# BadgerTechnologies/navigation

Measured on AMD Instinct MI355X. Metric: scored trajectories/sec (whole node) + costmap inflation cells/sec, 400x400 map, higher is better.
Workload: dtype f64

## Files before the change

### navigation_amd/csrc/costmap_kernels.hip

```cpp
#include "navgpu_device.h"

namespace navgpu {

__global__ void k_fill_u8(uint8_t* dst, uint8_t v, size_t n) {
  size_t i = (size_t)blockIdx.x * blockDim.x + threadIdx.x;
  size_t stride = (size_t)gridDim.x * blockDim.x;
  uint32_t w = v * 0x01010101u;
  uint4 q = make_uint4(w, w, w, w);
  size_t n16 = n / 16;
  for (size_t k = i; k < n16; k += stride) reinterpret_cast<uint4*>(dst)[k] = q;
  for (size_t k = n16 * 16 + i; k < n; k += stride) dst[k] = v;
}
__global__ void k_fill_u32(uint32_t* dst, uint32_t v, size_t n) {
  size_t i = (size_t)blockIdx.x * blockDim.x + threadIdx.x;
  size_t stride = (size_t)gridDim.x * blockDim.x;
  for (size_t k = i; k < n; k += stride) dst[k] = v;
}
void launch_fill_u8(uint8_t* dst, uint8_t v, size_t n, hipStream_t s) {
  if (!n) return;
  size_t blocks = (n / 16 + 255) / 256;
  if (blocks < 1) blocks = 1;
  if (blocks > 4096) blocks = 4096;
  hipLaunchKernelGGL(k_fill_u8, dim3((unsigned)blocks), dim3(256), 0, s, dst, v, n);
}
// ... 301 lines not shown
            double full = hyp2(dx, dy);
            double scale = fmin(1.0, obs.raytrace_range / full);
            b.touch(ox + dx * scale, oy + dy * scale);
          }
        } else {
          if (obs.n_points == 0) continue;
          const double ox = obs.ox, oy = obs.oy, oz = obs.oz;
          if (ox < g.ox || oy < g.oy || oz < cm.origin_z) continue;
          const double sensor_x = (ox - g.ox) / g.res, sensor_y = (oy - g.oy) / g.res, sensor_z = (oz - cm.origin_z) / cm.z_resolution;
          if (!(sensor_x < g.nx && sensor_y < g.ny && sensor_z < size_z)) continue;
          const double map_end_x = g.ox + (g.nx - 1 + 0.5) * g.res;
          const double map_end_y = g.oy + (g.ny - 1 + 0.5) * g.res;
          const uint32_t cell_range = cellDistance(obs.raytrace_range, g.res);
          for (uint32_t p = tid; p < obs.n_points; p += blockDim.x) {
            double wpx = pts[3 * p], wpy = pts[3 * p + 1], wpz = pts[3 * p + 2];
            double distance = sqrt((ox - wpx) * (ox - wpx) + (oy - wpy) * (oy - wpy) + (oz - wpz) * (oz - wpz));
            double scaling_fact = fmax(fmin(1.0, (distance - 2 * g.res) / distance), 0.0);
            wpx = scaling_fact * (wpx - ox) + ox;
            wpy = scaling_fact * (wpy - oy) + oy;
            wpz = scaling_fact * (wpz - oz) + oz;
            double a = wpx - ox, bb = wpy - oy, c = wpz - oz, t = 1.0;
            if (wpz > cm.max_obstacle_height)
              t = fmax(0.0, fmin(t, (cm.max_obstacle_height - 0.01 - oz) / c));
            else if (wpz < cm.origin_z)
              t = fmin(t, (cm.origin_z - oz) / c);
            if (wpx < g.ox) t = fmin(t, (g.ox - ox) / a);
            if (wpy < g.oy) t = fmin(t, (g.oy - oy) / bb);
            if (wpx > map_end_x) t = fmin(t, (map_end_x - ox) / a);
            if (wpy > map_end_y) t = fmin(t, (map_end_y - oy) / bb);
            wpx = ox + a * t;
            wpy = oy + bb * t;
            wpz = oz + c * t;
            if (wpx < g.ox || wpy < g.oy || wpz < cm.origin_z) continue;
            double px = (wpx - g.ox) / g.res, py = (wpy - g.oy) / g.res, pz = (wpz - cm.origin_z) / cm.z_resolution;
            if (!(px < g.nx && py < g.ny && pz < size_z)) continue;
            if (pass == 0) {
              raytrace3d(g.nx, sensor_x, sensor_y, sensor_z, px, py, pz, cell_range,
                         [&](uint32_t off, uint32_t zm) { atomicAnd(&vox[off], ~zm); });
              double dx = wpx - ox, dy = wpy - oy;
              double full = hyp2(dx, dy);
              double scale = fmin(1.0, obs.raytrace_range / full);
              b.touch(ox + dx * scale, oy + dy * scale);
            } else {
              raytrace3d(g.nx, sensor_x, sensor_y, sensor_z, px, py, pz, cell_range, [&](uint32_t off, uint32_t) {
                uint32_t col = vox[off];
                uint32_t unknown_bits = (uint16_t)(col >> 16) ^ (uint16_t)col;
                uint32_t marked_bits = col >> 16;
                if (bitsBelowThreshold(marked_bits, mark_thr))
                  layer[off] = bitsBelowThreshold(unknown_bits, unknown_thr) ? kFree : kNoInfo;
              });
            }
          }
        }
      }
      __syncthreads();
    }
    if (VOXEL && mark_thr > 0) {
      uint2* seq = cm.mark_seq + (size_t)inst * cm.max_points;
      uint32_t n_seq = 0;
      for (uint32_t o = ob; o < oe; ++o) n_seq = max(n_seq, cm.obs[o].first_point + cm.obs[o].n_points);
      for (uint32_t s = tid; s < n_seq; s += blockDim.x) seq[s] = make_uint2(0u, 0u);
      __syncthreads();
      for (uint32_t o = ob; o < oe; ++o) {
        const ObsCsr obs = cm.obs[o];
        if (!(obs.flags & NAVGPU_OBS_MARKING)) continue;
        const float* pts = inst_points + (size_t)obs.first_point * 3;
        const double sq_obstacle_range = obs.obstacle_range * obs.obstacle_range;
        for (uint32_t p = tid; p < obs.n_points; p += blockDim.x) {
          const float fx = pts[3 * p], fy = pts[3 * p + 1], fz = pts[3 * p + 2];
          double px = fx, py = fy, pz = fz;
          if (pz > cm.max_obstacle_height) continue;
          double sq_dist = (px - obs.ox) * (px - obs.ox) + (py - obs.oy) * (py - obs.oy) + (pz - obs.oz) * (pz - obs.oz);
          if (sq_dist >= sq_obstacle_range) continue;
          double wz = (pz < cm.origin_z) ? cm.origin_z : pz;
          if (px < g.ox || py < g.oy || wz < cm.origin_z) continue;
          double fxm = (px - g.ox) / g.res, fym = (py - g.oy) / g.res, fzm = (wz - cm.origin_z) / cm.z_resolution;
          if (!(fxm < 2147483648.0) || !(fym < 2147483648.0) || !(fzm < 2147483648.0)) continue;
          uint32_t mx = (uint32_t)(int)fxm, my = (uint32_t)(int)fym, mz = (uint32_t)(int)fzm;
          if (!(mx < g.nx && my < g.ny && mz < (uint32_t)cm.z_voxels)) continue;
          if (mz >= size_z) continue;
          const uint32_t cell = my * g.nx + mx;
          seq[obs.first_point + p] = make_uint2(cell, 0x80000000u | ((vox[cell] >> 16) << 8) | mz);
        }
      }
      __syncthreads();
      for (uint32_t s = tid; s < n_seq; s += blockDim.x) {
        const uint2 e = seq[s];
        if (!(e.y & 0x80000000u)) continue;
        const uint32_t mz = e.y & 0xFFu;
        uint32_t acc = ((e.y >> 8) & 0xFFFFu) | (1u << mz);
        for (uint32_t q = 0; q < s; ++q) {
          const uint2 f = seq[q];
          if ((f.y & 0x80000000u) && f.x == e.x) acc |= 1u << (f.y & 0xFFu);
        }
        atomicOr(&vox[e.x], ((uint32_t)1 << mz << 16) | (1u << mz));
        if (!bitsBelowThreshold(acc, mark_thr)) {
          layer[e.x] = kLethal;
          const float* pt = inst_points + (size_t)s * 3;
          b.touch((double)pt[0], (double)pt[1]);
        }
      }
    } else
    for (uint32_t o = ob; o < oe; ++o) {
      const ObsCsr obs = cm.obs[o];
      if (!(obs.flags & NAVGPU_OBS_MARKING)) continue;
      const float* pts = inst_points + (size_t)obs.first_point * 3;
      const double sq_obstacle_range = obs.obstacle_range * obs.obstacle_range;
      for (uint32_t p = tid; p < obs.n_points; p += blockDim.x) {
        const float fx = pts[3 * p], fy = pts[3 * p + 1], fz = pts[3 * p + 2];
        double px = fx, py = fy, pz = fz;
        if (pz > cm.max_obstacle_height) continue;
        double sq_dist = (px - obs.ox) * (px - obs.ox) + (py - obs.oy) * (py - obs.oy) + (pz - obs.oz) * (pz - obs.oz);
        if (sq_dist >= sq_obstacle_range) continue;
        if (!VOXEL) {
          uint32_t mx, my;
          if (!worldToMap(g, px, py, mx, my)) continue;
          layer[my * g.nx + mx] = kLethal;
          b.touch(px, py);
        } else {
          double wz = (pz < cm.origin_z) ? cm.origin_z : pz;
          if (px < g.ox || py < g.oy || wz < cm.origin_z) continue;
          double fxm = (px - g.ox) / g.res, fym = (py - g.oy) / g.res, fzm = (wz - cm.origin_z) / cm.z_resolution;
          if (!(fxm < 2147483648.0) || !(fym < 2147483648.0) || !(fzm < 2147483648.0)) continue;
          uint32_t mx = (uint32_t)(int)fxm, my = (uint32_t)(int)fym, mz = (uint32_t)(int)fzm;
          if (!(mx < g.nx && my < g.ny && mz < (uint32_t)cm.z_voxels)) continue;
          if (mz >= size_z) continue;
          uint32_t full_mask = ((uint32_t)1 << mz << 16) | (1u << mz);
          uint32_t old = atomicOr(&vox[my * g.nx + mx], full_mask);
          uint32_t marked_bits = (old | full_mask) >> 16;
          if (!bitsBelowThreshold(marked_bits, mark_thr)) {
            layer[my * g.nx + mx] = kLethal;
            b.touch(px, py);
          }
        }
      }
    }
    if (cm.footprint_clearing) {
      uint32_t nfp = cm.fp_n[inst];
      if (tid < nfp) b.touch(cm.fp_world[((size_t)inst * kMaxFootprint + tid) * 2], cm.fp_world[((size_t)inst * kMaxFootprint + tid) * 2 + 1]);
    }
  }

  for (int off = 32; off > 0; off >>= 1) {
    double o0 = __shfl_down(b.min_x, off), o1 = __shfl_down(b.min_y, off), o2 = __shfl_down(b.max_x, off), o3 = __shfl_down(b.max_y, off);
    b.min_x = (o0 < b.min_x) ? o0 : b.min_x;
    b.min_y = (o1 < b.min_y) ? o1 : b.min_y;
    b.max_x = (b.max_x < o2) ? o2 : b.max_x;
    b.max_y = (b.max_y < o3) ? o3 : b.max_y;
  }
  if ((tid & 63) == 0) {
    red[tid >> 6][0] = b.min_x;
    red[tid >> 6][1] = b.min_y;
    red[tid >> 6][2] = b.max_x;
    red[tid >> 6][3] = b.max_y;
  }
  __syncthreads();
  if (tid == 0) {
    for (int w = 1; w < 4; ++w) {
      b.min_x = (red[w][0] < b.min_x) ? red[w][0] : b.min_x;
      b.min_y = (red[w][1] < b.min_y) ? red[w][1] : b.min_y;
      b.max_x = (b.max_x < red[w][2]) ? red[w][2] : b.max_x;
      b.max_y = (b.max_y < red[w][3]) ? red[w][3] : b.max_y;
    }
    if (only_bounds) {
      bounds_io_out[4 * blockIdx.x + 0] = b.min_x;
      bounds_io_out[4 * blockIdx.x + 1] = b.min_y;
      bounds_io_out[4 * blockIdx.x + 2] = b.max_x;
      bounds_io_out[4 * blockIdx.x + 3] = b.max_y;
      s_box_valid = 1;
    } else {
      if (cm.layers & NAVGPU_LAYER_INFLATION) {
        if (st->need_reinflation) {
          st->last_min_x = b.min_x;
          st->last_min_y = b.min_y;
          st->last_max_x = b.max_x;
          st->last_max_y = b.max_y;
          b.min_x = -3.4028234663852886e38;
          b.min_y = -3.4028234663852886e38;
          b.max_x = 3.4028234663852886e38;
          b.max_y = 3.4028234663852886e38;
          st->need_reinflation = 0;
        } else {
          double tminx = st->last_min_x, tminy = st->last_min_y, tmaxx = st->last_max_x, tmaxy = st->last_max_y;
          st->last_min_x = b.min_x;
          st->last_min_y = b.min_y;
          st->last_max_x = b.max_x;
          st->last_max_y = b.max_y;
          b.min_x = ((b.min_x < tminx) ? b.min_x : tminx) - cm.inflation_radius;
          b.min_y = ((b.min_y < tminy) ? b.min_y : tminy) - cm.inflation_radius;
          b.max_x = ((tmaxx < b.max_x) ? b.max_x : tmaxx) + cm.inflation_radius;
          b.max_y = ((tmaxy < b.max_y) ? b.max_y : tmaxy) + cm.inflation_radius;
        }
      }
      st->bounds[0] = b.min_x;
      st->bounds[1] = b.min_y;
      st->bounds[2] = b.max_x;
      st->bounds[3] = b.max_y;
      int x0, xn, y0, yn;
      enforceBounds(g, b.min_x, b.min_y, x0, y0);
      enforceBounds(g, b.max_x, b.max_y, xn, yn);
      x0 = x0 > 0 ? x0 : 0;
      xn = ((int)g.nx < xn + 1) ? (int)g.nx : xn + 1;
      y0 = y0 > 0 ? y0 : 0;
      yn = ((int)g.ny < yn + 1) ? (int)g.ny : yn + 1;
      st->box[0] = x0;
      st->box[1] = xn;
      st->box[2] = y0;
      st->box[3] = yn;
      st->box_valid = !(xn < x0 || yn < y0);
      s_box_valid = st->box_valid;
    }
  }
  __syncthreads();

  if (has_obs_layer && cm.footprint_clearing && s_box_valid) {
    const uint32_t nfp = cm.fp_n[inst];
    if (tid == 0) s_poly_ok = nfp >= 3;
    __syncthreads();
    if (tid < nfp) {
      uint32_t mx, my;
      bool ok = worldToMap(g, cm.fp_world[((size_t)inst * kMaxFootprint + tid) * 2], cm.fp_world[((size_t)inst * kMaxFootprint + tid) * 2 + 1], mx, my);
      s_vx[tid] = mx;
      s_vy[tid] = my;
      if (!ok) atomicAnd(&s_poly_ok, 0);
    }
    __syncthreads();
    if (s_poly_ok) {
      uint32_t minx = 0xFFFFFFFFu, maxx = 0;
      for (uint32_t i = 0; i < nfp; ++i) {
        minx = s_vx[i] < minx ? s_vx[i] : minx;
        maxx = s_vx[i] > maxx ? s_vx[i] : maxx;
      }
      const uint32_t span = maxx - minx + 1;
      if (span <= 1024) {
        for (uint32_t c = tid; c < span; c += blockDim.x) {
          colmin[c] = 0xFFFFFFFFu;
          colmax[c] = 0;
        }
        __syncthreads();
        if (tid < nfp) {
          uint32_t e1 = (tid + 1 == nfp) ? 0 : tid + 1;
          raytrace2d(g.nx, s_vx[tid], s_vy[tid], s_vx[e1], s_vy[e1], 0xFFFFFFFFu, [&](uint32_t off) {
            uint32_t y = off / g.nx, x = off - y * g.nx;
            atomicMin(&colmin[x - minx], y);
            atomicMax(&colmax[x - minx], y);
          });
        }
        __syncthreads();
        for (uint32_t c = tid >> 4; c < span; c += blockDim.x >> 4) {
          uint32_t lo = colmin[c], hi = colmax[c];
          if (lo == 0xFFFFFFFFu) continue;
          for (uint32_t y = lo + (tid & 15); y <= hi; y += 16) layer[y * g.nx + minx + c] = kFree;
        }
      }
    }
  }
}

__global__ __launch_bounds__(256) void k_reset_bounding_box(CostmapDev cm, uint32_t first, const double* boxes_world) {
  const uint32_t inst = first + blockIdx.x;
  const Geom g{cm.origin[2 * inst], cm.origin[2 * inst + 1], cm.res, cm.nx, cm.ny};
  const double* bw = boxes_world + 4 * blockIdx.x;
  int x0, y0, xn, yn;
  enforceBounds(g, bw[0], bw[1], x0, y0);
  enforceBounds(g, bw[2], bw[3], xn, yn);
  uint8_t* layer = cm.obst + (size_t)inst * cm.cells_padded;
  if (xn > x0 && yn > y0) {
    const uint32_t w = (uint32_t)(xn - x0), n = w * (uint32_t)(yn - y0);
    for (uint32_t i = threadIdx.x; i < n; i += blockDim.x) layer[(uint32_t)(y0 + i / w) * g.nx + (uint32_t)x0 + i % w] = cm.obstacle_default;
  }
  if (threadIdx.x == 0) {
    InstCostmapState* st = cm.state + inst;
    if (!st->has_extra_bounds) {
      st->extra[0] = st->extra[1] = 1e6;
      st->extra[2] = st->extra[3] = -1e6;
    }
    st->extra[0] = (bw[0] < st->extra[0]) ? bw[0] : st->extra[0];
    st->extra[1] = (bw[1] < st->extra[1]) ? bw[1] : st->extra[1];
    st->extra[2] = (st->extra[2] < bw[2]) ? bw[2] : st->extra[2];
    st->extra[3] = (st->extra[3] < bw[3]) ? bw[3] : st->extra[3];
    st->has_extra_bounds = 1;
  }
}
__global__ __launch_bounds__(256) void k_reset_window(uint8_t* grid, size_t stride, uint32_t nx, uint32_t x0, uint32_t y0, uint32_t xn, uint32_t yn, uint8_t value) {
  uint8_t* gp = grid + (size_t)blockIdx.x * stride;
  const uint32_t w = xn - x0, n = w * (yn - y0);
  for (uint32_t i = threadIdx.x; i < n; i += blockDim.x) gp[(y0 + i / w) * nx + x0 + i % w] = value;
}
void launch_reset_window(uint8_t* grid, size_t stride, uint32_t count, uint32_t nx, uint32_t x0, uint32_t y0, uint32_t xn, uint32_t yn, uint8_t value, hipStream_t s) {
  hipLaunchKernelGGL(k_reset_window, dim3(count), dim3(256), 0, s, grid, stride, nx, x0, y0, xn, yn, value);
}
void launch_reset_bounding_box(const CostmapDev& cm, uint32_t first, uint32_t count, const double* boxes_world, hipStream_t s) {
  hipLaunchKernelGGL(k_reset_bounding_box, dim3(count), dim3(256), 0, s, cm, first, boxes_world);
}

void launch_obstacle(const CostmapDev& cm, uint32_t first, uint32_t count, const double* bounds_in, int only_bounds, hipStream_t s) {
  double* bounds_out = const_cast<double*>(bounds_in);
  if (cm.layers & NAVGPU_LAYER_VOXEL)
    hipLaunchKernelGGL(k_obstacle<true>, dim3(count), dim3(256), 0, s, cm, first, bounds_in, bounds_out, only_bounds);
  else
    hipLaunchKernelGGL(k_obstacle<false>, dim3(count), dim3(256), 0, s, cm, first, bounds_in, bounds_out, only_bounds);
}

__global__ __launch_bounds__(256) void k_merge(CostmapDev cm, uint32_t first, const int32_t* boxes, int static_received, int layer_only) {
  const uint32_t inst = first + blockIdx.y;
  int x0, xn, y0, yn;
  if (boxes) {
    x0 = boxes[4 * blockIdx.y + 0];
    y0 = boxes[4 * blockIdx.y + 1];
    xn = boxes[4 * blockIdx.y + 2];
    yn = boxes[4 * blockIdx.y + 3];
  } else {
    const InstCostmapState* st = cm.state + inst;
    if (!st->box_valid) return;
    x0 = st->box[0];
    xn = st->box[1];
    y0 = st->box[2];
    yn = st->box[3];
  }
  const uint32_t q = blockIdx.x * blockDim.x + threadIdx.x;
  const uint32_t base = q * 16;
  if (base >= cm.cells) return;
  const int row_first = base / cm.nx, row_last = (min(base + 15, cm.cells - 1)) / cm.nx;
  if (row_last < y0 || row_first >= yn) return;
  bool inside = false;
  if (row_first == row_last) {
    const int gx = base - row_first * cm.nx;
    if (gx + 15 < x0 || gx >= xn) return;
    inside = gx >= x0 && gx + 15 < xn && base + 15 < cm.cells && !layer_only;
  }
  const size_t off = (size_t)inst * cm.cells_padded + base;
  uint4 mv = make_uint4(0, 0, 0, 0);
  if (!inside) mv = *reinterpret_cast<const uint4*>(cm.master + off);
  const bool has_static = (cm.layers & NAVGPU_LAYER_STATIC) && static_received && !layer_only && !cm.stat_roll && cm.stat;
  const bool roll_static = cm.stat_roll != nullptr && !layer_only;
  double tfm[8] = {1, 0, 0, 0, 0, 1, 0, 0};
  double m_ox = 0, m_oy = 0;
  if (roll_static) {
    const double* T = cm.stat_tf + (size_t)inst * 12;
    tfm[0] = T[0]; tfm[1] = T[1]; tfm[2] = T[2]; tfm[3] = T[9];
    tfm[4] = T[3]; tfm[5] = T[4]; tfm[6] = T[5]; tfm[7] = T[10];
    m_ox = cm.origin[2 * inst];
    m_oy = cm.origin[2 * inst + 1];
  }
  const bool has_obst = (cm.layers & (NAVGPU_LAYER_OBSTACLE | NAVGPU_LAYER_VOXEL)) && cm.obs_enabled;
  uint4 sv = has_static ? *reinterpret_cast<const uint4*>(cm.stat + off) : make_uint4(0, 0, 0, 0);
  uint4 lv = has_obst ? *reinterpret_cast<const uint4*>(cm.obst + off) : make_uint4(0, 0, 0, 0);
  uint32_t mw[4] = {mv.x, mv.y, mv.z, mv.w}, sw[4] = {sv.x, sv.y, sv.z, sv.w}, lw[4] = {lv.x, lv.y, lv.z, lv.w};
  int y = row_first;
  int x = base - row_first * cm.nx;
  bool changed = false;
#pragma unroll
  for (int k = 0; k < 16; ++k) {
    if (base + k < cm.cells && x >= x0 && x < xn && y >= y0 && y < yn) {
      const int sh = (k & 3) * 8;
      uint8_t m = layer_only ? (uint8_t)((mw[k >> 2] >> sh) & 0xFF) : cm.master_default;
      if (has_static) {
        uint8_t sc = (sw[k >> 2] >> sh) & 0xFF;
        if (!cm.static_use_maximum)
          m = sc;
        else if (sc != kNoInfo && (m == kNoInfo || m < sc))
          m = sc;
      }
      if (roll_static) {
        const double wx = m_ox + (x + 0.5) * cm.res, wy = m_oy + (y + 0.5) * cm.res;
        const double px = tfm[0] * wx + tfm[1] * wy + tfm[2] * 0.0 + tfm[3];
        const double py = tfm[4] * wx + tfm[5] * wy + tfm[6] * 0.0 + tfm[7];
        if (!(px < cm.stat_ox || py < cm.stat_oy)) {
          const uint32_t smx = (uint32_t)(int)((px - cm.stat_ox) / cm.stat_res), smy = (uint32_t)(int)((py - cm.stat_oy) / cm.stat_res);
          if (smx < cm.stat_nx && smy < cm.stat_ny) {
            const uint8_t sc = cm.stat_roll[(size_t)smy * cm.stat_nx + smx];
            m = cm.static_use_maximum ? (sc > m ? sc : m) : sc;
          }
        }
      }
      if (has_obst) {
        uint8_t lc = (lw[k >> 2] >> sh) & 0xFF;
        if (lc != kNoInfo) {
          if (cm.combination_method == 0)
            m = lc;
          else if (cm.combination_method == 1 && (m == kNoInfo || m < lc))
            m = lc;
        }
      }
      mw[k >> 2] = (mw[k >> 2] & ~(0xFFu << sh)) | ((uint32_t)m << sh);
      changed = true;
    }
    if (++x == (int)cm.nx) {
      x = 0;
      ++y;
    }
  }
  if (changed) *reinterpret_cast<uint4*>(cm.master + off) = make_uint4(mw[0], mw[1], mw[2], mw[3]);
}

void launch_merge(const CostmapDev& cm, uint32_t first, uint32_t count, const int32_t* boxes, hipStream_t s, bool layer_only) {
  uint32_t groups = (cm.cells + 15) / 16;
  dim3 grid((groups + 255) / 256, count);
  hipLaunchKernelGGL(k_merge, grid, dim3(256), 0, s, cm, first, boxes, cm.static_received, layer_only ? 1 : 0);
}

constexpr int kTile = 64;
__global__ __launch_bounds__(256) void k_inflate(CostmapDev cm, uint32_t first, const int32_t* boxes) {
  extern __shared__ __align__(16) uint8_t lds[];
  const uint32_t inst = first + blockIdx.z;
  const int R = (int)cm.R;
  int min_i, min_j, max_i, max_j;
  if (boxes) {
    min_i = boxes[4 * blockIdx.z + 0];
    min_j = boxes[4 * blockIdx.z + 1];
    max_i = boxes[4 * blockIdx.z + 2];
    max_j = boxes[4 * blockIdx.z + 3];
  } else {
    const InstCostmapState* st = cm.state + inst;
    if (!st->box_valid) return;
    min_i = st->box[0];
    max_i = st->box[1];
    min_j = st->box[2];
    max_j = st->box[3];
  }
  min_i = max(0, min_i - R);
  min_j = max(0, min_j - R);
  max_i = min((int)cm.nx, max_i + R);
  max_j = min((int)cm.ny, max_j + R);
  const int tx0 = blockIdx.x * kTile, ty0 = blockIdx.y * kTile;
  if (tx0 - R >= max_i || tx0 + kTile + R <= min_i || ty0 - R >= max_j || ty0 + kTile + R <= min_j) return;

  const int W = kTile + 2 * R;
  const int WS = (W + 3) & ~3;
  uint8_t* seed = lds;
  uint8_t* hd = seed + W * WS;
  uint8_t* lut = hd + W * kTile;
  __shared__ int s_any;
  const uint32_t tid = threadIdx.x;
  uint8_t* master = cm.master + (size_t)inst * cm.cells_padded;
  if (tid == 0) s_any = 0;
  for (int i = tid; i < (R + 2) * (R + 2); i += blockDim.x) lut[i] = cm.lut[i];
  __syncthreads();
  int any = 0;
  for (int i = tid; i < W * W; i += blockDim.x) {
    int ly = i / W, lx = i - ly * W;
    int gx = tx0 - R + lx, gy = ty0 - R + ly;
    uint8_t f = 0;
    if (gx >= min_i && gx < max_i && gy >= min_j && gy < max_j) f = master[gy * cm.nx + gx] == kLethal;
    seed[ly * WS + lx] = f;
    any |= f;
  }
  if (any) s_any = 1;
  __syncthreads();
  if (!s_any) return;
  for (int i = tid; i < W * kTile; i += blockDim.x) {
    int ly = i / kTile, c = i - ly * kTile;
    const uint8_t* row = seed + ly * WS + c + R;
    uint8_t best = 255;
    for (int d = 0; d <= R; ++d) {
      if (row[d] | row[-d]) {
        best = (uint8_t)d;
        break;
      }
    }
    hd[i] = best;
  }
  __syncthreads();
  const int n = R + 2;
  for (int i = tid; i < kTile * kTile; i += blockDim.x) {
    int ry = i / kTile, c = i - ry * kTile;
    int gx = tx0 + c, gy = ty0 + ry;
    if (gx >= (int)cm.nx || gy >= (int)cm.ny) continue;
    uint8_t cost = 0;
    for (int dy = -R; dy <= R; ++dy) {
      uint8_t h = hd[(ry + R + dy) * kTile + c];
      if (h != 255) {
        int ady = dy < 0 ? -dy : dy;
        uint8_t cc = lut[h * n + ady];
        cost = cc > cost ? cc : cost;
      }
    }
    if (cost == 0) continue;
    uint8_t old = master[gy * cm.nx + gx];
    uint8_t nv = (old == kNoInfo && cost >= kInscribed) ? cost : (old > cost ? old : cost);
    if (nv != old) master[gy * cm.nx + gx] = nv;
  }
}

constexpr int kBX = 64, kBY = 32;
template <int RT>
__global__ __launch_bounds__(256) void k_inflate_bits(CostmapDev cm, uint32_t first, uint32_t count, const int32_t* boxes) {
  const uint32_t tbx = blockIdx.x >> 3, tby = blockIdx.y, rz = blockIdx.z * 8u + (blockIdx.x & 7u);
  if (rz >= count) return;
  const uint32_t inst = first + rz;
  const int R = RT > 0 ? RT : (int)cm.R;
  int min_i, min_j, max_i, max_j;
  if (boxes) {
    min_i = boxes[4 * rz + 0];
    min_j = boxes[4 * rz + 1];
    max_i = boxes[4 * rz + 2];
    max_j = boxes[4 * rz + 3];
  } else {
    const InstCostmapState* st = cm.state + inst;
    if (!st->box_valid) return;
    min_i = st->box[0];
    max_i = st->box[1];
    min_j = st->box[2];
    max_j = st->box[3];
  }
  min_i = max(0, min_i - R);
  min_j = max(0, min_j - R);
  max_i = min((int)cm.nx, max_i + R);
  max_j = min((int)cm.ny, max_j + R);
  const int tx0 = (int)tbx * kBX, ty0 = (int)tby * kBY;
  if (tx0 - R >= max_i || tx0 + kBX + R <= min_i || ty0 - R >= max_j || ty0 + kBY + R <= min_j) return;

  constexpr int kMaxHR = kBY + 2 * 14;
  constexpr int kOct = (kMaxHR + 7) / 8;
  __shared__ uint32_t s_rows[kMaxHR][4];
  __shared__ uint32_t s_hd[kOct + 1][kBX];
  __shared__ uint8_t s_lut2[256];
  __shared__ int s_any;
  __shared__ uint32_t s_rowany[2];
  const uint32_t tid = threadIdx.x, lane = tid & 63, wave = tid >> 6;
  const int HR = kBY + 2 * R;
  uint8_t* master = cm.master + (size_t)inst * cm.cells_padded;
  if (tid == 0) s_any = 0;
  if (tid < 2) s_rowany[tid] = 0;
  s_lut2[tid] = cm.lut2[tid];
  __syncthreads();
  int any = 0;
  uint32_t rows_lo = 0, rows_hi = 0;
  constexpr int kSeedIt = (kMaxHR + 3) / 4;
  uint8_t cell[kSeedIt][2];
  const int gxa = tx0 - 32 + (int)lane, gxb = gxa + 64;
  const int lo_x = max(min_i, tx0 - R), lo_y = max(min_j, ty0 - R);
  const int hi_x = max(lo_x, min(max_i, tx0 + kBX + R) - 1), hi_y = max(lo_y, min(max_j, ty0 + kBY + R) - 1);
  const int cxa = min(min(max(gxa, lo_x), hi_x), (int)cm.nx - 1), cxb = min(min(max(gxb, lo_x), hi_x), (int)cm.nx - 1);
  const bool xa_ok = gxa >= min_i && gxa < max_i && gxa >= tx0 - R && gxa < tx0 + kBX + R;
  const bool xb_ok = gxb >= min_i && gxb < max_i && gxb >= tx0 - R && gxb < tx0 + kBX + R;
#pragma unroll
  for (int it = 0; it < kSeedIt; ++it) {
    const int gy = ty0 - R + (int)wave + 4 * it;
    const int cy = min(min(max(gy, lo_y), hi_y), (int)cm.ny - 1);
    cell[it][0] = master[cy * cm.nx + cxa];
    cell[it][1] = master[cy * cm.nx + cxb];
  }
#pragma unroll
  for (int it = 0; it < kSeedIt; ++it) {
    const int r = (int)wave + 4 * it, gy = ty0 - R + r;
    if (r < HR) {
      const bool row_ok = gy >= min_j && gy < max_j;
#pragma unroll
      for (int half = 0; half < 2; ++half) {
        const unsigned long long m = __ballot(row_ok && (half ? xb_ok : xa_ok) && cell[it][half] == kLethal);
        if (lane == 0) {
          s_rows[r][2 * half] = (uint32_t)m;
          s_rows[r][2 * half + 1] = (uint32_t)(m >> 32);
        }
        any |= m != 0ull;
        if (m != 0ull) {
          if (r < 32)
            rows_lo |= 1u << r;
          else
            rows_hi |= 1u << (r - 32);
        }
      }
    }
  }
  if (any && lane == 0) {
    s_any = 1;
    if (rows_lo) atomicOr(&s_rowany[0], rows_lo);
    if (rows_hi) atomicOr(&s_rowany[1], rows_hi);
  }
  __syncthreads();
  if (!s_any) return;
  const uint32_t lowmask = (1u << R) - 1u;
  for (int o = wave; o * 8 < HR; o += 4) {
    uint32_t packed = 0;
#pragma unroll
    for (int k = 0; k < 8; ++k) {
      const int r = o * 8 + k;
      uint32_t h = 15;
      if (r < HR && (s_rows[r][0] | s_rows[r][1] | s_rows[r][2] | s_rows[r][3]) != 0u) {
        const uint32_t sft = 32u + lane - (uint32_t)R;
        const uint32_t wi = sft >> 5, bs = sft & 31u;
        const unsigned long long two = ((unsigned long long)s_rows[r][wi + 1 < 4 ? wi + 1 : 3] << 32) | s_rows[r][wi];
        const uint32_t q = (uint32_t)(two >> bs);
        const uint32_t qr = q >> R;
        const uint32_t ql = q & lowmask;
        uint32_t dr = 15, dl = 15;
        if (qr & ((2u << R) - 1u)) dr = (uint32_t)__builtin_ctz(qr & ((2u << R) - 1u));
        if (ql) dl = (uint32_t)R - (31u - (uint32_t)__builtin_clz(ql));
        h = dr < dl ? dr : dl;
      }
      packed |= h << (4 * k);
    }
    s_hd[o][lane] = packed;
  }
  __syncthreads();
  uint32_t hw[5];
#pragma unroll
  for (int k = 0; k < 5; ++k) hw[k] = (wave + k) * 8 < (uint32_t)HR ? s_hd[wave + k][lane] : 0xFFFFFFFFu;
  if (__ballot((hw[0] & hw[1] & hw[2] & hw[3] & hw[4]) != 0xFFFFFFFFu) == 0ull) return;
  const int gx = tx0 + (int)lane;
  const int R2 = R * R;
  uint32_t bestr[8] = {0xFFFFu, 0xFFFFu, 0xFFFFu, 0xFFFFu, 0xFFFFu, 0xFFFFu, 0xFFFFu, 0xFFFFu};
  if (RT > 0) {
    const unsigned long long rowany = (((unsigned long long)s_rowany[1] << 32) | s_rowany[0]) >> (8u * wave);
    const uint32_t ra_lo = __builtin_amdgcn_readfirstlane((uint32_t)rowany), ra_hi = __builtin_amdgcn_readfirstlane((uint32_t)(rowany >> 32));
#pragma unroll
    for (int p = 0; p < 8 + 2 * RT; ++p) {
      if (((p < 32 ? ra_lo >> (p & 31) : ra_hi >> (p & 31)) & 1u) != 0u) {
        const uint32_t h = (hw[p >> 3] >> (4 * (p & 7))) & 15u;
        const uint32_t hh = h * h;
#pragma unroll
        for (int j = 0; j < 8; ++j) {
          const int dy = p - RT - j;
          if (dy >= -RT && dy <= RT) {
            const uint32_t d2 = hh + (uint32_t)(dy * dy);
            bestr[j] = d2 < bestr[j] ? d2 : bestr[j];
          }
        }
      }
    }
  }
#pragma unroll
  for (int j = 0; j < 8; ++j) {
    const int gy = ty0 + (int)wave * 8 + j;
    uint32_t best = bestr[j];
    if (RT == 0) {
      for (int dy = -R; dy <= R; ++dy) {
        const int p = j + R + dy;
        const uint32_t wsel = p >> 3;
        const uint32_t word = wsel == 0 ? hw[0] : (wsel == 1 ? hw[1] : (wsel == 2 ? hw[2] : (wsel == 3 ? hw[3] : hw[4])));
        const uint32_t h = (word >> (4 * (p & 7))) & 15u;
        const uint32_t d2 = h * h + (uint32_t)(dy * dy);
        best = d2 < best ? d2 : best;
      }
    }
    if (best > (uint32_t)R2 || gx >= (int)cm.nx || gy >= (int)cm.ny) continue;
    const uint8_t cost = s_lut2[best];
    if (cost == 0) continue;
    const uint8_t old = master[gy * cm.nx + gx];
    const uint8_t nv = (old == kNoInfo && cost >= kInscribed) ? cost : (old > cost ? old : cost);
    if (nv != old) master[gy * cm.nx + gx] = nv;
  }
}

constexpr uint32_t kPqSeenWords = 5120, kPqWinBytes = 65536;
constexpr size_t kPqLdsBytes = 150 * 1024;
constexpr uint32_t kPqTabEntries = 66 * 66;
__global__ __launch_bounds__(64) void k_inflate_pq(CostmapDev cm, uint32_t first, const int32_t* boxes) {
  extern __shared__ __align__(16) uint8_t pq_sm[];
  const uint32_t inst = first + blockIdx.x;
  const uint32_t tid = threadIdx.x;
  int min_i, min_j, max_i, max_j;
  if (boxes) {
    min_i = boxes[4 * blockIdx.x + 0];
    min_j = boxes[4 * blockIdx.x + 1];
    max_i = boxes[4 * blockIdx.x + 2];
    max_j = boxes[4 * blockIdx.x + 3];
  } else {
    const InstCostmapState* st = cm.state + inst;
    if (!st->box_valid) return;
    min_i = st->box[0];
    max_i = st->box[1];
    min_j = st->box[2];
    max_j = st->box[3];
  }
  uint8_t* master = cm.master + (size_t)inst * cm.cells_padded;
  uint8_t* seen_g = cm.pq_seen + (size_t)inst * cm.cells_padded;
  PqCell* heap_g = cm.pq_heap + (size_t)inst * cm.pq_cap;
  const uint32_t size_x = cm.nx, size_y = cm.ny;
  const int R = (int)cm.R;
  const uint32_t n = cm.R + 2;
  min_i = max(0, min_i - R);
  min_j = max(0, min_j - R);
  max_i = min((int)size_x, max_i + R);
  max_j = min((int)size_y, max_j + R);
  if (max_i <= min_i || max_j <= min_j) return;
  const int wx0 = max(0, min_i - R - 1), wy0 = max(0, min_j - R - 1), wx1 = min((int)size_x, max_i + R + 1), wy1 = min((int)size_y, max_j + R + 1);
  const uint32_t ww = (uint32_t)(wx1 - wx0), wh = (uint32_t)(wy1 - wy0), wcells = ww * wh;
  const bool seen_lds = wcells <= kPqSeenWords * 32u, win_lds = wcells <= kPqWinBytes;
  uint16_t* rank = reinterpret_cast<uint16_t*>(pq_sm);
  uint8_t* lut_l = pq_sm + kPqTabEntries * 2;
  const uint32_t seen_off = (kPqTabEntries * 3 + 15u) & ~15u;
  uint32_t* seen_l = reinterpret_cast<uint32_t*>(pq_sm + seen_off);
  const uint32_t win_off = seen_off + (seen_lds ? (((wcells + 31) / 32 * 4 + 15u) & ~15u) : 0u);
  uint8_t* win_l = pq_sm + win_off;
  const uint32_t heap_off = win_off + (win_lds ? ((wcells + 15u) & ~15u) : 0u);
  PqCell* heap_l = reinterpret_cast<PqCell*>(pq_sm + heap_off);
  const long heap_lds = (long)((kPqLdsBytes - heap_off) / sizeof(PqCell));
  for (uint32_t i = tid; i < n * n; i += 64) {
    rank[i] = reinterpret_cast<const uint16_t*>(cm.dist_lut)[i];
    lut_l[i] = cm.lut[i];
  }
  if (seen_lds) {
    for (uint32_t i = tid; i < (wcells + 31) / 32; i += 64) seen_l[i] = 0;
  } else {
    for (uint32_t i = tid * 16; i < cm.cells_padded; i += 64 * 16) *reinterpret_cast<uint4*>(seen_g + i) = make_uint4(0, 0, 0, 0);
  }
  if (win_lds)
    for (uint32_t i = tid; i < wcells; i += 64) {
      const uint32_t y = i / ww, x = i - y * ww;
      win_l[i] = master[(uint32_t)(wy0 + (int)y) * size_x + (uint32_t)(wx0 + (int)x)];
    }
  __syncthreads();
  if (tid == 0) {
    long len = 0;
    auto hget = [&](long i) -> PqCell { return i < heap_lds ? heap_l[i] : heap_g[i]; };
    auto hset = [&](long i, const PqCell& v) {
      if (i < heap_lds)
        heap_l[i] = v;
      else
        heap_g[i] = v;
    };
    auto widx = [&](uint32_t mx, uint32_t my) { return (my - (uint32_t)wy0) * ww + (mx - (uint32_t)wx0); };
    auto seenGet = [&](uint32_t index, uint32_t mx, uint32_t my) -> bool {
      if (seen_lds) {
        const uint32_t w = widx(mx, my);
        return (seen_l[w >> 5] >> (w & 31)) & 1u;
      }
      return seen_g[index] != 0;
    };
    auto seenSet = [&](uint32_t index, uint32_t mx, uint32_t my) {
      if (seen_lds) {
        const uint32_t w = widx(mx, my);
        seen_l[w >> 5] |= 1u << (w & 31);
      } else {
        seen_g[index] = 1;
      }
    };
    auto pushHeap = [&](long hole, const PqCell& value) {
      long parent = (hole - 1) / 2;
      while (hole > 0) {
        const PqCell pv = hget(parent);
        if (!(pv.rank > value.rank)) break;
        hset(hole, pv);
        hole = parent;
        parent = (hole - 1) / 2;
      }
      hset(hole, value);
    };
    auto probe = [&](bool in_map, uint32_t index, uint32_t mx, uint32_t my, uint32_t sx, uint32_t sy) -> uint32_t {
      if (!in_map) return 0xFFFFu;
      const uint32_t dx = mx > sx ? mx - sx : sx - mx, dy = my > sy ? my - sy : sy - my;
      const uint32_t r = rank[dx * n + dy];
      return seenGet(index, mx, my) ? 0xFFFFu : r;
    };
    auto push = [&](uint32_t r, uint32_t index, uint32_t mx, uint32_t my, uint32_t sx, uint32_t sy) {
      if (r == 0xFFFFu) return;
      if ((uint64_t)len >= cm.pq_cap) return;
      PqCell c;
      c.index = index;
      c.rank = (uint16_t)r;
      c.sdx = (int8_t)((int)sx - (int)mx);
      c.sdy = (int8_t)((int)sy - (int)my);
      pushHeap(len++, c);
    };
    auto enqueue = [&](uint32_t index, uint32_t mx, uint32_t my, uint32_t sx, uint32_t sy) { push(probe(true, index, mx, my, sx, sy), index, mx, my, sx, sy); };
    for (int j = min_j; j < max_j; j++)
      for (int i = min_i; i < max_i; i++) {
        const uint32_t index = (uint32_t)j * size_x + (uint32_t)i;
        const uint8_t c0 = win_lds ? win_l[widx((uint32_t)i, (uint32_t)j)] : master[index];
        if (c0 == kLethal) enqueue(index, i, j, i, j);
      }
    while (len > 0) {
      const PqCell cur = hget(0);
      if (len > 1) {
        const PqCell value = hget(len - 1);
        const long l = len - 1;
        long hole = 0, child = 0;
        while (child < (l - 1) / 2) {
          child = 2 * (child + 1);
          const PqCell a = hget(child), b = hget(child - 1);
          if (a.rank > b.rank) {
            child--;
            hset(hole, b);
          } else {
            hset(hole, a);
          }
          hole = child;
        }
        if ((l & 1) == 0 && child == (l - 2) / 2) {
          child = 2 * (child + 1);
          hset(hole, hget(child - 1));
          hole = child - 1;
        }
        pushHeap(hole, value);
      }
      --len;
      const uint32_t index = cur.index;
      const uint32_t my = index / size_x, mx = index - my * size_x;
      if (seenGet(index, mx, my)) continue;
      seenSet(index, mx, my);
      const uint32_t sx = (uint32_t)((int)mx + cur.sdx), sy = (uint32_t)((int)my + cur.sdy);
      const uint32_t dx = mx > sx ? mx - sx : sx - mx, dy = my > sy ? my - sy : sy - my;
      const uint8_t cost = lut_l[dx * n + dy];
      uint8_t* cellp = win_lds ? &win_l[widx(mx, my)] : &master[index];
      const uint8_t old_cost = *cellp;
      if (old_cost == kNoInfo && cost >= kInscribed)
        *cellp = cost;
      else
        *cellp = old_cost > cost ? old_cost : cost;
      const uint32_t r0 = probe(mx > 0, index - 1, mx - 1, my, sx, sy), r1 = probe(my > 0, index - size_x, mx, my - 1, sx, sy),
                     r2 = probe(mx < size_x - 1, index + 1, mx + 1, my, sx, sy), r3 = probe(my < size_y - 1, index + size_x, mx, my + 1, sx, sy);
      push(r0, index - 1, mx - 1, my, sx, sy);
      push(r1, index - size_x, mx, my - 1, sx, sy);
      push(r2, index + 1, mx + 1, my, sx, sy);
      push(r3, index + size_x, mx, my + 1, sx, sy);
    }
  }
  __syncthreads();
  if (win_lds)
    for (uint32_t i = tid; i < wcells; i += 64) {
      const uint32_t y = i / ww, x = i - y * ww;
      master[(uint32_t)(wy0 + (int)y) * size_x + (uint32_t)(wx0 + (int)x)] = win_l[i];
    }
}

void launch_inflate(const CostmapDev& cm, uint32_t first, uint32_t count, const int32_t* boxes, hipStream_t s) {
  if (!cm.infl_enabled) return;
  const int R = (int)cm.R;
  if (cm.infl_pq) {
    if (!cm.pq_heap || !cm.pq_seen || !cm.dist_lut) return;
    hipFuncSetAttribute((const void*)k_inflate_pq, hipFuncAttributeMaxDynamicSharedMemorySize, (int)kPqLdsBytes);
    hipLaunchKernelGGL(k_inflate_pq, dim3(count), dim3(64), kPqLdsBytes, s, cm, first, boxes);
    return;
  }
  if (cm.lut2_ok && R >= 1 && R <= 14) {
    dim3 grid(8u * ((cm.nx + kBX - 1) / kBX), (cm.ny + kBY - 1) / kBY, (count + 7u) / 8u);
    if (R == 11)
      hipLaunchKernelGGL(k_inflate_bits<11>, grid, dim3(256), 0, s, cm, first, count, boxes);
    else
      hipLaunchKernelGGL(k_inflate_bits<0>, grid, dim3(256), 0, s, cm, first, count, boxes);
    return;
  }
  const int W = kTile + 2 * R, WS = (W + 3) & ~3;
  size_t lds = (size_t)W * WS + (size_t)W * kTile + (size_t)(R + 2) * (R + 2);
  dim3 grid((cm.nx + kTile - 1) / kTile, (cm.ny + kTile - 1) / kTile, count);
  hipLaunchKernelGGL(k_inflate, grid, dim3(256), lds, s, cm, first, boxes);
}

}
```

### navigation_amd/csrc/navgpu_device.h

```cpp
#pragma once
#include <hip/hip_runtime.h>
#include <stdint.h>

#include "../../include/navgpu.h"

namespace navgpu {

constexpr uint8_t kNoInfo = 255, kLethal = 254, kInscribed = 253, kFree = 0;
constexpr int kMaxFootprint = 32;
constexpr int kCareRows = 128, kCareWords = 4;
#ifndef NAVGPU_SCORE_TAB_THREADS
#define NAVGPU_SCORE_TAB_THREADS 256
#endif
#ifndef NAVGPU_SCORE_TAB_LDS_KB
#define NAVGPU_SCORE_TAB_LDS_KB 14
#endif
#ifndef NAVGPU_SCORE_PREP_THREADS
#define NAVGPU_SCORE_PREP_THREADS 256
#endif
#ifndef NAVGPU_SCORE_THREADS
#define NAVGPU_SCORE_THREADS 256
#endif
#ifdef NAVGPU_DEBUG_SWITCHES
#define NAVGPU_DEBUG_ENV(name) getenv(name)
#else
#define NAVGPU_DEBUG_ENV(name) ((const char*)nullptr)
#endif
constexpr int kScoreThreads = NAVGPU_SCORE_THREADS;

struct InstCostmapState {
  double last_min_x, last_min_y, last_max_x, last_max_y;
  int32_t need_reinflation;
  int32_t static_has_updated_data;
  int32_t box[4];
  int32_t box_valid;
  int32_t pad;
  double bounds[4];
  double extra[4];
  int32_t has_extra_bounds, pad2;
};

struct ObsCsr {
  uint32_t first_point, n_points, flags, pad;
  double ox, oy, oz;
  double obstacle_range, raytrace_range;
};

struct PqCell {
  uint32_t index;
  uint16_t rank;
  int8_t sdx, sdy;
};
static_assert(sizeof(PqCell) == 8, "heap entry");
struct CostmapDev {
  uint32_t nx, ny, cells, cells_padded;
  double res;
  int32_t layers, track_unknown;
  uint8_t master_default, obstacle_default;
  int32_t obs_enabled, footprint_clearing, combination_method, static_use_maximum, static_received;
  double max_obstacle_height;
  int32_t z_voxels, unknown_threshold, mark_threshold;
  double origin_z, z_resolution;
  int32_t infl_enabled;
  uint32_t R;
  double inflation_radius;
  double* origin;
  uint8_t *master, *stat, *obst;
  uint32_t* voxel;
  uint8_t* lut;
  uint8_t* lut2;
  int32_t lut2_ok;
  int32_t infl_pq;
  double* dist_lut;
  uint8_t* pq_seen;
  PqCell* pq_heap;
  uint64_t pq_cap;
  uint8_t* stat_roll;
  uint32_t stat_nx, stat_ny;
  double stat_res, stat_ox, stat_oy;
  double* stat_tf;
  InstCostmapState* state;
  double* pose;
  double* fp_world;
  uint32_t* fp_n;
  ObsCsr* obs;
  uint32_t* obs_count;
  float* points;
  uint32_t max_obs, max_points;
  int32_t* shift;
  uint8_t *master_alt, *obst_alt;
  uint32_t* voxel_alt;
  uint2* mark_seq;
};

struct PlannerDev {
  uint32_t nx, ny, cells;
  double res, inv_res;
  double* origin;
  const uint8_t* master;
  uint32_t cells_padded;
  navgpu_dwa_config cfg;
  double scale_path, scale_goal, scale_obstacle;
  uint32_t max_plan, max_sim_steps, max_axis;
  uint32_t max_samples, score_blocks;
  navgpu_robot_state* state;
  double* plan;
  uint32_t* plan_count;
  double* front_last;
  int32_t* align_on;
  double* fp_spec;
  uint32_t* fp_n;
  float* axis_samples;
  int32_t* axis_count;
  uint32_t *path, *goal, *goal_front;
  uint32_t* bfs_scratch;
  int32_t* bfs_box;
  uint32_t* bfs_care;
  uint32_t* bfs_reach;
  uint32_t bfs_bounded;
  unsigned long long* bfs_trace;
  uint32_t* bfs_next_item;
  uint32_t* bfs_free;
  uint32_t* bfs_levels;
  uint32_t* bfs_order;
  uint32_t bfs_grids;
  uint32_t* within;
  uint32_t win;
  uint32_t fp_rcells;
  uint8_t fp_halfw[32];
  uint32_t fp_chunk;
  uint32_t use_tables, tab_steps, tab_nfp, tab_nth;
  int32_t mg_agg[4];
  double mg_yshift[4];
  int32_t mg_generic;
  uint32_t tab_rows;
  uint32_t tab_bytes;
  double tab_dt;
  uint8_t* prep;
  uint32_t prep_stride, prep_bytes;
  double* sample_cost;
  int32_t* sample_status;
  double* part_cost;
  int32_t* part_index;
  int32_t* counters;
  uint32_t* osc_flags;
  float* osc_prev;
  navgpu_plan_result* result;
  double* traj;
};

struct TpOut {
  double cost;
  double ex, ey, eth;
  double ahead;
  int32_t n_points;
  int32_t ahead_ok;
};
struct TpDev {
  navgpu_tp_config cfg;
  uint32_t max_samples;
  double* samples;
  uint32_t* n_samples;
  double* start;
  TpOut* out;
  int32_t* winner;
  double* points;
  uint32_t* within_cells;
  uint32_t* within_count;
  uint32_t max_within;
  uint32_t* within_bits;
};
void launch_tp_within(const PlannerDev& pl, const TpDev& tp, uint32_t first, uint32_t count, hipStream_t s);
void launch_tp_rollout(const PlannerDev& pl, const TpDev& tp, uint32_t first, uint32_t count, int store_points, hipStream_t s);

void launch_obstacle(const CostmapDev& cm, uint32_t first, uint32_t count, const double* bounds_in, int only_bounds,
                     hipStream_t s);
void launch_reset_window(uint8_t* grid, size_t stride, uint32_t count, uint32_t nx, uint32_t x0, uint32_t y0, uint32_t xn, uint32_t yn, uint8_t value, hipStream_t s);
void launch_reset_bounding_box(const CostmapDev& cm, uint32_t first, uint32_t count, const double* boxes_world, hipStream_t s);
void launch_merge(const CostmapDev& cm, uint32_t first, uint32_t count, const int32_t* boxes, hipStream_t s, bool layer_only = false);
void launch_inflate(const CostmapDev& cm, uint32_t first, uint32_t count, const int32_t* boxes, hipStream_t s);
void launch_static_interpret(uint8_t* dst, const int8_t* occ, uint32_t cells, uint32_t cells_padded, uint32_t count,
                             int track_unknown_space, int trinary, int lethal_threshold, int unknown_cost_value, hipStream_t s);
void launch_export_window(const uint8_t* master, uint32_t nx, uint32_t x0, uint32_t y0, uint32_t w, uint32_t h, int8_t* out, hipStream_t s);
void launch_fill_u8(uint8_t* dst, uint8_t v, size_t n, hipStream_t s);
void launch_fill_u32(uint32_t* dst, uint32_t v, size_t n, hipStream_t s);
void launch_shift_u8(const uint8_t* src, uint8_t* dst, const CostmapDev& cm, uint32_t first, uint32_t count, uint8_t fill, hipStream_t s);
void launch_shift_u32(const uint32_t* src, uint32_t* dst, const CostmapDev& cm, uint32_t first, uint32_t count, uint32_t fill, hipStream_t s);

void launch_cell_costs(const PlannerDev& pl, uint32_t inst, float4* out, hipStream_t s);
void launch_samples(const PlannerDev& pl, uint32_t first, uint32_t count, hipStream_t s);
void launch_bfs(const PlannerDev& pl, uint32_t first, uint32_t count, hipStream_t s, const uint32_t* order = nullptr, bool free_ready = false);
uint32_t launch_score(const PlannerDev& pl, uint32_t first, uint32_t count, const float* explicit_sample, hipStream_t s);
void launch_select(const PlannerDev& pl, uint32_t first, uint32_t count, uint32_t n_blocks, hipStream_t s);
constexpr uint32_t kPoseChunk = 64;
struct PoseChunk {
  navgpu_robot_state* state;
  double* front_last;
  int32_t* align_on;
  uint32_t* bfs_reach;
  uint32_t first, count;
  navgpu_robot_state st[kPoseChunk];
  double front[2 * kPoseChunk];
  int32_t align[kPoseChunk];
  uint32_t reach[kPoseChunk];
};
static_assert(sizeof(PoseChunk) <= 4096, "kernel arguments are limited to 4 KB");
void launch_stage_poses(const PoseChunk& c, hipStream_t s);
void launch_sincos(const double* th, uint32_t n, double* sn, double* cs, hipStream_t s);
size_t score_table_bytes(const PlannerDev& pl);
size_t score_window_bytes(uint32_t win);
size_t score_prep_bytes(const PlannerDev& pl);
size_t score_prep_slot_bytes(const PlannerDev& pl);
size_t bfs_scratch_words(uint32_t nx, uint32_t ny);
uint32_t score_table_rows(const PlannerDev& pl, uint32_t win);

struct Geom {
  double ox, oy, res;
  uint32_t nx, ny;
};

__device__ __forceinline__ bool worldToMap(const Geom& g, double wx, double wy, uint32_t& mx, uint32_t& my) {
  if (wx < g.ox || wy < g.oy) return false;
  double fx = (wx - g.ox) / g.res;
  double fy = (wy - g.oy) / g.res;
  if (!(fx < 2147483648.0) || !(fy < 2147483648.0)) return false;
  mx = (uint32_t)(int)fx;
  my = (uint32_t)(int)fy;
  return mx < g.nx && my < g.ny;
}

__device__ __forceinline__ double hyp2(double x, double y) {
  double a = x * x, b = y * y;
  double s = a + b;
  double h = sqrt(s);
  if (h == 0.0) return 0.0;
  double bb = s - a;
  double e = (a - (s - bb)) + (b - bb);
  double r = __builtin_fma(-h, h, s);
  return h + (r + e) / (2.0 * h);
}

struct NavfnDev {
  int nx, ny, ns;
  uint32_t ns_padded, path_cap;
  uint8_t *costarr, *pending;
  float *potarr, *gradx, *grady;
  int* pb;
  float* path;
  navgpu_navfn_result* results;
  float* potalt;
  uint32_t* wf_act;
  uint32_t *wf_nchg, *wf_min;
  struct NavfnWfStatus* wf_status;
  int wf_tiles_x, wf_tiles_y, wf_max_rounds;
};
struct NavfnWfStatus {
  int32_t done, final_array, rounds, pad;
};
struct NavfnWfRule {
  int32_t global_planner, quadratic, outline, allow_unknown;
  int32_t lethal_cost, neutral_cost;
  float cost_factor;
  int32_t max_sweeps;
};
void launch_navfn_wf_init(const NavfnDev& nv, uint32_t first, uint32_t count, const NavfnWfRule& rule, const int32_t* seed_cells, const float* seed_vals,
                          hipStream_t s);
void launch_navfn_wf_round(const NavfnDev& nv, uint32_t first, uint32_t count, const NavfnWfRule& rule, const int32_t* stop_cells, int at_start, int round,
                           hipStream_t s);
void launch_gp_wf_finish(const NavfnDev& nv, uint32_t first, uint32_t count, const navgpu_global_planner_params& gp, const double* starts,
                         const double* goals, const int32_t* goal_cells, hipStream_t s);
void launch_navfn_wf_path(const NavfnDev& nv, uint32_t first, uint32_t count, const int32_t* goals, const int32_t* starts, hipStream_t s);
void launch_navfn_costmap(const NavfnDev& nv, uint32_t first, uint32_t count, const uint8_t* cmap, size_t stride, int cost_mode, int allow_unknown,
                          hipStream_t s);
void launch_gp_plan(const NavfnDev& nv, uint32_t first, uint32_t count, const navgpu_global_planner_params& gp, const double* starts,
                    const double* goals, const int32_t* goal_cells, void* heaps, hipStream_t s);
void launch_navfn_plan(const NavfnDev& nv, uint32_t first, uint32_t count, const int32_t* goals, const int32_t* starts, int astar, int at_start,
                       hipStream_t s);

}
```

### navigation_amd/csrc/navgpu_fleet.h

```cpp
#pragma once
#include <algorithm>
#include <cfloat>
#include <cmath>
#include <cstdio>
#include <cstdlib>
#include <cstring>
#include <ctime>
#include <mutex>
#include <string>
#include <vector>

#include "navgpu_device.h"

using namespace navgpu;

namespace navgpu {
extern thread_local std::string g_last_error;

#define HIP_TRY(expr)                                                                              \
  do {                                                                                             \
    hipError_t e_ = (expr);                                                                        \
    if (e_ != hipSuccess) {                                                                        \
      g_last_error = std::string(#expr) + ": " + hipGetErrorString(e_);                            \
      return NAVGPU_ERR_HIP;                                                                       \
    }                                                                                              \
  } while (0)

inline hipError_t waitStream(hipStream_t s) { return hipStreamSynchronize(s); }

struct EventPair {
  int kernel;
  hipEvent_t a, b;
};
int ensureCompleteGrids(navgpu_fleet* f, uint32_t first, uint32_t count);
}

struct navgpu_fleet {
  navgpu_fleet_desc desc{};
  std::recursive_mutex mu;
  hipStream_t stream = nullptr;
  CostmapDev cm{};
  PlannerDev pl{};
  bool planner_configured = false, inflation_configured = false, planner_staged = false;
  bool shift_pending = false;
  uint32_t shift_first = 0, shift_count = 0;
  std::vector<void*> allocs;
  std::vector<double> h_origin;
  std::vector<double> h_fp_spec;
  std::vector<uint32_t> h_fp_n;
  navgpu_inflation_params infl{};
  navgpu_obstacle_params obsp{};
  double fp_radius = 0.0;
  std::vector<void*> pinned;
  ObsCsr* hp_obs = nullptr;
  uint32_t *hp_cnt = nullptr, *hp_used = nullptr, *hp_plan_cnt = nullptr;
  float* hp_pts = nullptr;
  double *hp_fpw = nullptr, *hp_pose = nullptr, *hp_plan = nullptr, *hp_front = nullptr;
  int32_t *hp_shift = nullptr, *hp_align = nullptr;
  uint32_t *hp_reach = nullptr, *hp_fpn = nullptr;
  uint8_t *cm_stage_dev = nullptr, *cm_stage_host = nullptr, *pl_stage_dev = nullptr, *pl_stage_host = nullptr;
  size_t cm_stage_bytes = 0, pl_stage_bytes = 0;
  bool bounded_grids = true;
  std::vector<uint8_t> grid_partial;
  std::vector<int32_t> h_box;
  std::vector<uint64_t> inputs_gen, cycle_gen;
  void touchInputs(uint32_t first, uint32_t count) {
    for (uint32_t i = first; i < first + count && i < inputs_gen.size(); ++i) ++inputs_gen[i];
  }
  navgpu_robot_state* hp_state = nullptr;
  navgpu_plan_result* hp_result = nullptr;
  bool hp_dma_pending = false;
  int cycles_in_flight = 1;
  int res_slot = 0;
  hipEvent_t ev_cycle[2] = {nullptr, nullptr}, ev_cm_h2d = nullptr, ev_pl_h2d = nullptr;
  bool ev_cycle_set[2] = {false, false}, ev_cm_set = false, ev_pl_set = false;
  hipError_t waitMirrors(hipEvent_t ev, bool set) {
    if (cycles_in_flight < 2) return navgpu::waitStream(stream);
    return set ? hipEventSynchronize(ev) : hipSuccess;
  }
  struct LocalPlannerState {
    std::vector<double> plan;
    double T[3] = {0, 0, 0};
    bool has_T = false, have_plan = false;
    bool xy_tolerance_latch = false, rotating_to_goal = false;
  };
  std::vector<LocalPlannerState> lp;
  navgpu_local_limits lp_limits{};
  bool lp_configured = false;
  struct TpHost {
    std::vector<double> plan;
    double final_goal_x = 0, final_goal_y = 0;
    bool final_goal_position_valid = false;
    navgpu_tp_state st{};
    std::vector<navgpu_tp_sample> made;
    int n_points = 0;
  };
  TpDev tp{};
  bool tp_configured = false;
  std::vector<TpHost> tph;
  std::vector<double> tp_h_samples, tp_h_start;
  std::vector<TpOut> tp_h_out;
  std::vector<uint32_t> tp_h_nsamples, tp_h_within, tp_h_within_count;
  std::vector<int32_t> tp_h_winner;
  double* d_bounds_tmp = nullptr;
  int32_t* d_boxes_tmp = nullptr;
  float* d_explicit = nullptr;
  int8_t* d_occ = nullptr;
  float4* d_cell_costs = nullptr;
  size_t alloc_limit = 0;
  bool profiling = false;
  uint32_t prof_mask = ~0u;
  std::vector<EventPair> events;
  std::vector<EventPair> free_events;
  double prof_ms[NAVGPU_K_COUNT] = {0};
  uint64_t prof_n[NAVGPU_K_COUNT] = {0};

  template <class T>
  int alloc(T** p, size_t count) {
    void* q = nullptr;
    size_t bytes = std::max<size_t>(count * sizeof(T), 16);
    if (alloc_limit && bytes > alloc_limit) {
      g_last_error = "hipMalloc: refused by navgpu_fleet_set_alloc_limit";
      return NAVGPU_ERR_HIP;
    }
    hipError_t e = hipMalloc(&q, bytes);
    if (e != hipSuccess) {
      g_last_error = std::string("hipMalloc: ") + hipGetErrorString(e);
      return NAVGPU_ERR_HIP;
    }
    e = hipMemsetAsync(q, 0, bytes, stream);
    if (e != hipSuccess) {
      g_last_error = std::string("hipMemsetAsync: ") + hipGetErrorString(e);
      return NAVGPU_ERR_HIP;
    }
    allocs.push_back(q);
    *p = static_cast<T*>(q);
    return NAVGPU_OK;
  }
  template <class T>
  int allocPinned(T** p, size_t count) {
    void* q = nullptr;
    hipError_t e = hipHostMalloc(&q, std::max<size_t>(count * sizeof(T), 16), hipHostMallocDefault);
    if (e != hipSuccess) {
      g_last_error = std::string("hipHostMalloc: ") + hipGetErrorString(e);
      return NAVGPU_ERR_HIP;
    }
    memset(q, 0, std::max<size_t>(count * sizeof(T), 16));
    pinned.push_back(q);
    *p = static_cast<T*>(q);
    return NAVGPU_OK;
  }
  void release(void* q) {
    if (!q) return;
    auto it = std::find(allocs.begin(), allocs.end(), q);
    if (it != allocs.end()) allocs.erase(it);
    hipFree(q);
  }
  bool rangeOk(uint32_t first, uint32_t count) const { return count > 0 && first < desc.n_instances && count <= desc.n_instances - first; }

  int beginKernel(int k, EventPair* ep) {
    if (!profiling || !((prof_mask >> k) & 1u)) return NAVGPU_OK;
    if (free_events.empty()) {
      EventPair n{};
      HIP_TRY(hipEventCreate(&n.a));
      HIP_TRY(hipEventCreate(&n.b));
      free_events.push_back(n);
    }
    *ep = free_events.back();
    free_events.pop_back();
    ep->kernel = k;
    HIP_TRY(hipEventRecord(ep->a, stream));
    return NAVGPU_OK;
  }
  int endKernel(EventPair* ep) {
    if (!profiling || !ep->a) return NAVGPU_OK;
    HIP_TRY(hipEventRecord(ep->b, stream));
    events.push_back(*ep);
    if (events.size() > 8192) return foldEvents();
    return NAVGPU_OK;
  }
  int foldEvents() {
    if (events.empty()) return NAVGPU_OK;
    HIP_TRY(waitStream(stream));
    for (auto& e : events) {
      float ms = 0;
      HIP_TRY(hipEventElapsedTime(&ms, e.a, e.b));
      prof_ms[e.kernel] += ms;
      prof_n[e.kernel] += 1;
      free_events.push_back(e);
    }
    events.clear();
    return NAVGPU_OK;
  }
};

#ifndef NAVGPU_TEST_NO_FLEET_LOCK
struct FleetGuard {
  std::lock_guard<std::recursive_mutex> lk;
  explicit FleetGuard(navgpu_fleet* f) : lk(f->mu) { (void)hipSetDevice(f->desc.device); }
};
#else
struct FleetGuard {
  explicit FleetGuard(navgpu_fleet* f) { (void)hipSetDevice(f->desc.device); }
};
#endif

#define PROFILED(fleet, kid, launch_expr)            \
  do {                                               \
    EventPair ep_{};                                 \
    int rc_ = (fleet)->beginKernel((kid), &ep_);     \
    if (rc_) return rc_;                             \
    launch_expr;                                     \
    rc_ = (fleet)->endKernel(&ep_);                  \
    if (rc_) return rc_;                             \
  } while (0)

inline int checkLaunch() {
  hipError_t e = hipGetLastError();
  if (e != hipSuccess) {
    g_last_error = std::string("kernel launch: ") + hipGetErrorString(e);
    return NAVGPU_ERR_HIP;
  }
  return NAVGPU_OK;
}
```

### navigation_amd/csrc/navgpu_host.cpp

```cpp
#include "navgpu_fleet.h"

namespace navgpu {
thread_local std::string g_last_error;
}

extern "C" {

const char* navgpu_version(void) { return "navgpu 0.1 (gfx950)"; }
const char* navgpu_strerror(int status) {
  switch (status) {
    case NAVGPU_OK: return "ok";
    case NAVGPU_ERR_INVALID: return "invalid argument";
    case NAVGPU_ERR_NO_DEVICE: return "no usable HIP device (this library has no CPU fallback)";
    case NAVGPU_ERR_HIP: return "HIP runtime error";
    case NAVGPU_ERR_CAPACITY: return "input exceeds a capacity given at fleet creation";
    case NAVGPU_ERR_STATE: return "call sequence violated";
    default: return "unknown status";
  }
}
const char* navgpu_last_error(void) { return g_last_error.c_str(); }
int navgpu_device_count(void) {
  int n = 0;
  if (hipGetDeviceCount(&n) != hipSuccess) return 0;
  return n;
}
const char* navgpu_kernel_name(int32_t k) {
  static const char* names[NAVGPU_K_COUNT] = {"k_obstacle", "k_merge", "k_inflate", "k_bfs", "k_score", "k_select"};
  return (k >= 0 && k < NAVGPU_K_COUNT) ? names[k] : "?";
}

int navgpu_fleet_create(const navgpu_fleet_desc* d, navgpu_fleet** out) {
  if (!d || !out || d->n_instances == 0 || d->size_x == 0 || d->size_y == 0 || !(d->resolution > 0)) return NAVGPU_ERR_INVALID;
  if ((uint64_t)((d->size_x + 127) / 128) * ((d->size_y + 15) / 16) > 8192) {
    g_last_error = "navgpu_fleet_create: costmap larger than 16.7 M cells";
    return NAVGPU_ERR_CAPACITY;
  }
  if (d->max_footprint > (uint32_t)kMaxFootprint) return NAVGPU_ERR_CAPACITY;
  if ((uint64_t)d->size_x * d->size_y > (1ull << 30) || d->size_x > 65535 || d->size_y > 65535) return NAVGPU_ERR_CAPACITY;
  int ndev = 0;
  if (hipGetDeviceCount(&ndev) != hipSuccess || ndev <= 0 || d->device < 0 || d->device >= ndev) {
    g_last_error = "no HIP device";
    return NAVGPU_ERR_NO_DEVICE;
  }
  HIP_TRY(hipSetDevice(d->device));
  auto* f = new navgpu_fleet();
  f->desc = *d;
  if (f->desc.max_observations == 0) f->desc.max_observations = 1;
  if (f->desc.max_points == 0) f->desc.max_points = 1;
  if (f->desc.max_plan == 0) f->desc.max_plan = 1;
  if (f->desc.max_sim_steps == 0) f->desc.max_sim_steps = 64;
  const uint32_t n = d->n_instances;
  if (hipStreamCreateWithFlags(&f->stream, hipStreamNonBlocking) != hipSuccess) {
    g_last_error = "hipStreamCreate failed";
    delete f;
    return NAVGPU_ERR_NO_DEVICE;
  }
  CostmapDev& cm = f->cm;
  cm.nx = d->size_x;
  cm.ny = d->size_y;
  cm.cells = d->size_x * d->size_y;
  cm.cells_padded = (cm.cells + 63) & ~63u;
  cm.res = d->resolution;
  cm.layers = d->layers;
  cm.track_unknown = d->track_unknown;
  cm.master_default = d->track_unknown ? kNoInfo : kFree;
  cm.obstacle_default = d->track_unknown ? kNoInfo : kFree;
  cm.obs_enabled = 1;
  cm.footprint_clearing = 1;
  cm.combination_method = 1;
  cm.max_obstacle_height = 2.0;
  cm.z_voxels = 10;
  cm.unknown_threshold = 15;
  cm.mark_threshold = 0;
  cm.origin_z = 0.0;
  cm.z_resolution = 0.2;
  cm.max_obs = f->desc.max_observations;
  cm.max_points = f->desc.max_points;
  int rc = 0;
#define A(ptr, cnt)                        \
  if ((rc = f->alloc(&(ptr), (cnt))) != 0) { \
    navgpu_fleet_destroy(f);               \
    return rc;                             \
  }
  A(cm.origin, (size_t)n * 2);
  A(cm.master, (size_t)n * cm.cells_padded);
  if ((d->layers & NAVGPU_LAYER_STATIC) && !d->rolling_window) A(cm.stat, (size_t)n * cm.cells_padded);
  if (d->layers & (NAVGPU_LAYER_OBSTACLE | NAVGPU_LAYER_VOXEL)) A(cm.obst, (size_t)n * cm.cells_padded);
  if (d->layers & NAVGPU_LAYER_VOXEL) A(cm.voxel, (size_t)n * cm.cells_padded);
  A(cm.lut, 66 * 66);
  A(cm.lut2, 256);
  A(cm.state, n);
  A(cm.shift, (size_t)n * 2);
  {
    size_t off = 0;
    auto take = [&](size_t bytes) {
      const size_t at = off;
      off = (off + bytes + 255) & ~(size_t)255;
      return at;
    };
    const size_t o_pose = take(sizeof(double) * 3 * n), o_fpw = take(sizeof(double) * 2 * kMaxFootprint * n), o_fpn = take(sizeof(uint32_t) * n),
                 o_obs = take(sizeof(ObsCsr) * (size_t)n * cm.max_obs), o_cnt = take(sizeof(uint32_t) * n),
                 o_pts = take(sizeof(float) * 3 * (size_t)n * cm.max_points);
    f->cm_stage_bytes = off;
    uint8_t *d = nullptr, *h = nullptr;
    A(d, off);
    if ((rc = f->allocPinned(&h, off)) != 0) {
      navgpu_fleet_destroy(f);
      return rc;
    }
    f->cm_stage_dev = d;
    f->cm_stage_host = h;
    cm.pose = reinterpret_cast<double*>(d + o_pose);
    cm.fp_world = reinterpret_cast<double*>(d + o_fpw);
    cm.fp_n = reinterpret_cast<uint32_t*>(d + o_fpn);
    cm.obs = reinterpret_cast<ObsCsr*>(d + o_obs);
    cm.obs_count = reinterpret_cast<uint32_t*>(d + o_cnt);
    cm.points = reinterpret_cast<float*>(d + o_pts);
    f->hp_pose = reinterpret_cast<double*>(h + o_pose);
    f->hp_fpw = reinterpret_cast<double*>(h + o_fpw);
    f->hp_fpn = reinterpret_cast<uint32_t*>(h + o_fpn);
    f->hp_obs = reinterpret_cast<ObsCsr*>(h + o_obs);
    f->hp_cnt = reinterpret_cast<uint32_t*>(h + o_cnt);
    f->hp_pts = reinterpret_cast<float*>(h + o_pts);
  }
  if (d->rolling_window) {
    if (d->layers & NAVGPU_LAYER_STATIC) {
      A(cm.stat_tf, (size_t)n * 12);
      std::vector<double> ident((size_t)n * 12, 0.0);
      for (uint32_t i = 0; i < n; ++i) ident[(size_t)i * 12 + 0] = ident[(size_t)i * 12 + 4] = ident[(size_t)i * 12 + 8] = 1.0;
      if (hipMemcpy(cm.stat_tf, ident.data(), sizeof(double) * ident.size(), hipMemcpyHostToDevice) != hipSuccess) {
        navgpu_fleet_destroy(f);
        return NAVGPU_ERR_HIP;
      }
    }
    A(cm.master_alt, (size_t)n * cm.cells_padded);
    if (cm.obst) A(cm.obst_alt, (size_t)n * cm.cells_padded);
    if (cm.voxel) A(cm.voxel_alt, (size_t)n * cm.cells_padded);
  }
  if (cm.voxel) A(cm.mark_seq, (size_t)n * cm.max_points);
#define AP(ptr, cnt)                              \
  if ((rc = f->allocPinned(&(ptr), (cnt))) != 0) { \
    navgpu_fleet_destroy(f);                       \
    return rc;                                     \
  }
  AP(f->hp_used, n);
  AP(f->hp_shift, (size_t)n * 2);
  AP(f->hp_result, (size_t)n * 2);
  f->pl.result = f->hp_result;
#undef AP
  A(f->d_bounds_tmp, (size_t)n * 4);
  A(f->d_boxes_tmp, (size_t)n * 4);
  A(f->d_explicit, 4);
  PlannerDev& pl = f->pl;
  pl.nx = cm.nx;
  pl.ny = cm.ny;
  pl.cells = cm.cells;
  pl.cells_padded = cm.cells_padded;
  pl.res = cm.res;
  pl.inv_res = 1.0 / cm.res;
  pl.origin = cm.origin;
  pl.master = cm.master;
  pl.max_plan = f->desc.max_plan;
  pl.max_sim_steps = f->desc.max_sim_steps;
  {
    size_t off = 0;
    auto take = [&](size_t bytes) {
      const size_t at = off;
      off = (off + bytes + 255) & ~(size_t)255;
      return at;
    };
    const size_t o_state = take(sizeof(navgpu_robot_state) * n), o_front = take(sizeof(double) * 2 * n), o_align = take(sizeof(int32_t) * n),
                 o_reach = take(sizeof(uint32_t) * n), o_pcnt = take(sizeof(uint32_t) * n), o_plan = take(sizeof(double) * 2 * (size_t)n * pl.max_plan);
    f->pl_stage_bytes = off;
    uint8_t *d = nullptr, *h = nullptr;
    A(d, off);
    if ((rc = f->allocPinned(&h, off)) != 0) {
      navgpu_fleet_destroy(f);
      return rc;
    }
    f->pl_stage_dev = d;
    f->pl_stage_host = h;
    pl.state = reinterpret_cast<navgpu_robot_state*>(d + o_state);
    pl.front_last = reinterpret_cast<double*>(d + o_front);
    pl.align_on = reinterpret_cast<int32_t*>(d + o_align);
    pl.bfs_reach = reinterpret_cast<uint32_t*>(d + o_reach);
    pl.plan_count = reinterpret_cast<uint32_t*>(d + o_pcnt);
    pl.plan = reinterpret_cast<double*>(d + o_plan);
    f->hp_state = reinterpret_cast<navgpu_robot_state*>(h + o_state);
    f->hp_front = reinterpret_cast<double*>(h + o_front);
    f->hp_align = reinterpret_cast<int32_t*>(h + o_align);
    f->hp_reach = reinterpret_cast<uint32_t*>(h + o_reach);
    f->hp_plan_cnt = reinterpret_cast<uint32_t*>(h + o_pcnt);
    f->hp_plan = reinterpret_cast<double*>(h + o_plan);
  }
  A(pl.fp_spec, (size_t)n * kMaxFootprint * 2);
  A(pl.fp_n, n);
  A(pl.axis_count, (size_t)n * 4);
  A(pl.path, (size_t)n * pl.cells);
  A(pl.goal, (size_t)n * pl.cells);
  A(pl.goal_front, (size_t)n * pl.cells);
  if (bfs_scratch_words(cm.nx, cm.ny)) A(pl.bfs_scratch, (size_t)n * bfs_scratch_words(cm.nx, cm.ny));
  pl.bfs_grids = 3;
  pl.within = nullptr;
  A(pl.bfs_box, (size_t)n * 8);
  A(pl.bfs_care, (size_t)n * kCareRows * kCareWords);
  A(pl.bfs_next_item, 4);
  A(pl.bfs_free, (size_t)n * cm.ny * ((cm.nx + 31) / 32));
  A(pl.bfs_levels, (size_t)n * 3);
  A(pl.bfs_order, (size_t)n * 3);
  pl.bfs_bounded = 0;
  A(pl.counters, (size_t)n * 2);
  A(pl.osc_flags, n);
  A(pl.osc_prev, (size_t)n * 3);
  A(pl.traj, (size_t)n * pl.max_sim_steps * 3);
#undef A
  f->h_origin.assign((size_t)n * 2, 0.0);
  f->h_fp_spec.assign((size_t)n * kMaxFootprint * 2, 0.0);
  f->h_fp_n.assign(n, 0);
  f->grid_partial.assign(n, 0);
  f->bounded_grids = true;
  f->h_box.assign((size_t)n * 4, 0);
  f->inputs_gen.assign(n, 0);
  f->cycle_gen.assign(n, 0);
  launch_fill_u8(cm.master, cm.master_default, (size_t)n * cm.cells_padded, f->stream);
  if (cm.obst) launch_fill_u8(cm.obst, cm.obstacle_default, (size_t)n * cm.cells_padded, f->stream);
  if (cm.voxel) launch_fill_u32(cm.voxel, 0x0000FFFFu, (size_t)n * cm.cells_padded, f->stream);
  std::vector<InstCostmapState> st(n);
  for (auto& s : st) {
    memset(&s, 0, sizeof(s));
    s.last_min_x = -FLT_MAX;
    s.last_min_y = -FLT_MAX;
    s.last_max_x = FLT_MAX;
    s.last_max_y = FLT_MAX;
  }
  hipError_t e = hipMemcpyAsync(cm.state, st.data(), sizeof(InstCostmapState) * n, hipMemcpyHostToDevice, f->stream);
  if (e == hipSuccess) e = hipMemsetAsync(pl.bfs_reach, 0, sizeof(uint32_t) * n, f->stream);
  if (e == hipSuccess) e = hipMemsetAsync(pl.bfs_levels, 0, sizeof(uint32_t) * 3 * n, f->stream);
  if (e == hipSuccess) e = waitStream(f->stream);
  if (e != hipSuccess || checkLaunch() != NAVGPU_OK) {
    if (e != hipSuccess) g_last_error = std::string("fleet init: ") + hipGetErrorString(e);
    navgpu_fleet_destroy(f);
    return NAVGPU_ERR_NO_DEVICE;
  }
  *out = f;
  return NAVGPU_OK;
}

int navgpu_fleet_destroy(navgpu_fleet* f) {
  if (!f) return NAVGPU_ERR_INVALID;
  if (f->stream) waitStream(f->stream);
  for (auto& e : f->events) {
    hipEventDestroy(e.a);
    hipEventDestroy(e.b);
  }
  for (auto& e : f->free_events) {
    hipEventDestroy(e.a);
    hipEventDestroy(e.b);
  }
  for (hipEvent_t e : {f->ev_cycle[0], f->ev_cycle[1], f->ev_cm_h2d, f->ev_pl_h2d})
    if (e) hipEventDestroy(e);
  for (void* p : f->allocs) hipFree(p);
  for (void* p : f->pinned) hipHostFree(p);
  if (f->stream) hipStreamDestroy(f->stream);
  delete f;
  return NAVGPU_OK;
}
int navgpu_sync(navgpu_fleet* f) {
  if (!f) return NAVGPU_ERR_INVALID;
  FleetGuard guard_(f);
  HIP_TRY(waitStream(f->stream));
  return NAVGPU_OK;
}
void* navgpu_stream(navgpu_fleet* f) { return f ? (void*)f->stream : nullptr; }
int navgpu_fleet_set_alloc_limit(navgpu_fleet* f, uint64_t max_bytes) {
  if (!f) return NAVGPU_ERR_INVALID;
  FleetGuard guard_(f);
  f->alloc_limit = (size_t)max_bytes;
  return NAVGPU_OK;
}

int navgpu_fleet_set_origin(navgpu_fleet* f, uint32_t first, uint32_t count, const double* xy) {
  if (!f || !xy || !f->rangeOk(first, count)) return NAVGPU_ERR_INVALID;
  FleetGuard guard_(f);
  f->touchInputs(first, count);
  memcpy(&f->h_origin[(size_t)first * 2], xy, sizeof(double) * 2 * count);
  HIP_TRY(hipMemcpyAsync(f->cm.origin + (size_t)first * 2, xy, sizeof(double) * 2 * count, hipMemcpyHostToDevice, f->stream));
  HIP_TRY(waitStream(f->stream));
  return NAVGPU_OK;
}

int navgpu_fleet_get_origin(navgpu_fleet* f, uint32_t first, uint32_t count, double* xy) {
  if (!f || !xy || !f->rangeOk(first, count)) return NAVGPU_ERR_INVALID;
  FleetGuard guard_(f);
  memcpy(xy, &f->h_origin[(size_t)first * 2], sizeof(double) * 2 * count);
  return NAVGPU_OK;
}

static int gridInfo(navgpu_fleet* f, int grid, void** base, size_t* elem, size_t* stride_elems, size_t* used_elems) {
  CostmapDev& cm = f->cm;
  PlannerDev& pl = f->pl;
  switch (grid) {
    case NAVGPU_GRID_MASTER: *base = cm.master; *elem = 1; *stride_elems = cm.cells_padded; break;
    case NAVGPU_GRID_STATIC: *base = cm.stat; *elem = 1; *stride_elems = cm.cells_padded; break;
    case NAVGPU_GRID_OBSTACLE: *base = cm.obst; *elem = 1; *stride_elems = cm.cells_padded; break;
    case NAVGPU_GRID_VOXEL: *base = cm.voxel; *elem = 4; *stride_elems = cm.cells_padded; break;
    case NAVGPU_GRID_PATH: *base = pl.path; *elem = 4; *stride_elems = pl.cells; break;
    case NAVGPU_GRID_GOAL: *base = pl.goal; *elem = 4; *stride_elems = pl.cells; break;
    case NAVGPU_GRID_GOAL_FRONT: *base = pl.goal_front; *elem = 4; *stride_elems = pl.cells; break;
    default: return NAVGPU_ERR_INVALID;
  }
  *used_elems = cm.cells;
  if (!*base) return NAVGPU_ERR_STATE;
  return NAVGPU_OK;
}
int navgpu_grid_upload(navgpu_fleet* f, int grid, uint32_t first, uint32_t count, const void* host) {
  if (!f || !host || !f->rangeOk(first, count)) return NAVGPU_ERR_INVALID;
  FleetGuard guard_(f);
  f->touchInputs(first, count);
  void* base;
  size_t elem, stride, used;
  int rc = gridInfo(f, grid, &base, &elem, &stride, &used);
  if (rc) return rc;
  if (grid >= NAVGPU_GRID_PATH)
    for (uint32_t i = first; i < first + count; ++i) f->grid_partial[i] = 0;
  HIP_TRY(hipMemcpy2DAsync((char*)base + (size_t)first * stride * elem, stride * elem, host, used * elem, used * elem, count,
                           hipMemcpyHostToDevice, f->stream));
  HIP_TRY(waitStream(f->stream));
  return NAVGPU_OK;
}
int navgpu_grid_download(navgpu_fleet* f, int grid, uint32_t first, uint32_t count, void* host) {
  if (!f || !host || !f->rangeOk(first, count)) return NAVGPU_ERR_INVALID;
  FleetGuard guard_(f);
  void* base;
  size_t elem, stride, used;
  int rc = gridInfo(f, grid, &base, &elem, &stride, &used);
  if (rc) return rc;
  if (grid >= NAVGPU_GRID_PATH && (rc = ensureCompleteGrids(f, first, count))) return rc;
  HIP_TRY(hipMemcpy2DAsync(host, used * elem, (char*)base + (size_t)first * stride * elem, stride * elem, used * elem, count,
                           hipMemcpyDeviceToHost, f->stream));
  HIP_TRY(waitStream(f->stream));
  return NAVGPU_OK;
}
int navgpu_grid_device(navgpu_fleet* f, int grid, void** ptr, size_t* stride_bytes) {
  if (!f || !ptr) return NAVGPU_ERR_INVALID;
  FleetGuard guard_(f);
  void* base;
  size_t elem, stride, used;
  int rc = gridInfo(f, grid, &base, &elem, &stride, &used);
  if (rc) return rc;
  if (grid >= NAVGPU_GRID_PATH && (rc = ensureCompleteGrids(f, 0, f->desc.n_instances))) return rc;
  *ptr = base;
  if (stride_bytes) *stride_bytes = stride * elem;
  return NAVGPU_OK;
}
int navgpu_grid_reset(navgpu_fleet* f, int grid, uint32_t first, uint32_t count) {
  if (!f || !f->rangeOk(first, count)) return NAVGPU_ERR_INVALID;
  FleetGuard guard_(f);
  f->touchInputs(first, count);
  CostmapDev& cm = f->cm;
  switch (grid) {
    case NAVGPU_GRID_MASTER: launch_fill_u8(cm.master + (size_t)first * cm.cells_padded, cm.master_default, (size_t)count * cm.cells_padded, f->stream); break;
    case NAVGPU_GRID_OBSTACLE:
      if (!cm.obst) return NAVGPU_ERR_STATE;
      launch_fill_u8(cm.obst + (size_t)first * cm.cells_padded, cm.obstacle_default, (size_t)count * cm.cells_padded, f->stream);
      if (cm.voxel) launch_fill_u32(cm.voxel + (size_t)first * cm.cells_padded, 0x0000FFFFu, (size_t)count * cm.cells_padded, f->stream);
      break;
    case NAVGPU_GRID_VOXEL:
      if (!cm.voxel) return NAVGPU_ERR_STATE;
      launch_fill_u32(cm.voxel + (size_t)first * cm.cells_padded, 0x0000FFFFu, (size_t)count * cm.cells_padded, f->stream);
      break;
    default: return NAVGPU_ERR_INVALID;
  }
  return checkLaunch();
}

static int applyPendingShift(navgpu_fleet* f, uint32_t first, uint32_t count);
int navgpu_grid_reset_window(navgpu_fleet* f, int grid, uint32_t first, uint32_t count, uint32_t x0, uint32_t y0, uint32_t xn, uint32_t yn) {
  if (!f || !f->rangeOk(first, count)) return NAVGPU_ERR_INVALID;
  FleetGuard guard_(f);
  CostmapDev& cm = f->cm;
  if (xn > cm.nx || yn > cm.ny || x0 > xn || y0 > yn) return NAVGPU_ERR_INVALID;
  uint8_t* base = nullptr;
  uint8_t value = 0;
  switch (grid) {
    case NAVGPU_GRID_MASTER: base = cm.master; value = cm.master_default; break;
    case NAVGPU_GRID_OBSTACLE: base = cm.obst; value = cm.obstacle_default; break;
    default: return NAVGPU_ERR_INVALID;
  }
  if (!base) return NAVGPU_ERR_STATE;
  f->touchInputs(first, count);
  if (xn > x0 && yn > y0) launch_reset_window(base + (size_t)first * cm.cells_padded, cm.cells_padded, count, cm.nx, x0, y0, xn, yn, value, f->stream);
  return checkLaunch();
}
int navgpu_layer_reset_bounding_box(navgpu_fleet* f, uint32_t first, uint32_t count, const double* boxes) {
  if (!f || !boxes || !f->rangeOk(first, count)) return NAVGPU_ERR_INVALID;
  FleetGuard guard_(f);
  CostmapDev& cm = f->cm;
  if (!cm.obst) return NAVGPU_ERR_STATE;
  for (uint32_t i = 0; i < count; ++i)
    if (!(boxes[4 * i] <= boxes[4 * i + 2]) || !(boxes[4 * i + 1] <= boxes[4 * i + 3])) return NAVGPU_ERR_INVALID;
  {
    int rc = applyPendingShift(f, first, count);
    if (rc) return rc;
  }
  f->touchInputs(first, count);
  HIP_TRY(hipMemcpyAsync(f->d_bounds_tmp, boxes, sizeof(double) * 4 * count, hipMemcpyHostToDevice, f->stream));
  launch_reset_bounding_box(cm, first, count, f->d_bounds_tmp, f->stream);
  HIP_TRY(waitStream(f->stream));
  return checkLaunch();
}

static double fpDistance(double x0, double y0, double x1, double y1) { return hypot(x1 - x0, y1 - y0); }
static double fpDistanceToLine(double pX, double pY, double x0, double y0, double x1, double y1) {
  const double A = pX - x0, B = pY - y0, C = x1 - x0, D = y1 - y0;
  const double dot = A * C + B * D, len_sq = C * C + D * D;
  const double param = dot / len_sq;
  double xx, yy;
  if (param < 0) {
    xx = x0;
    yy = y0;
  } else if (param > 1) {
    xx = x1;
    yy = y1;
  } else {
    xx = x0 + param * C;
    yy = y0 + param * D;
  }
  return fpDistance(pX, pY, xx, yy);
}
int navgpu_footprint_radii(const double* xy, uint32_t n, double* inscribed, double* circumscribed) {
  if ((n && !xy) || !inscribed || !circumscribed) return NAVGPU_ERR_INVALID;
  double min_dist = DBL_MAX, max_dist = 0.0;
  if (n > 2) {
    for (uint32_t i = 0; i < n; ++i) {
      const uint32_t j = (i + 1 == n) ? 0 : i + 1;
      const double vertex_dist = fpDistance(0.0, 0.0, xy[2 * i], xy[2 * i + 1]);
      const double edge_dist = fpDistanceToLine(0.0, 0.0, xy[2 * i], xy[2 * i + 1], xy[2 * j], xy[2 * j + 1]);
      min_dist = std::min(min_dist, std::min(vertex_dist, edge_dist));
      max_dist = std::max(max_dist, std::max(vertex_dist, edge_dist));
    }
  }
  *inscribed = min_dist;
  *circumscribed = max_dist;
  return NAVGPU_OK;
}
int navgpu_footprint_pad(double* xy, uint32_t n, double padding) {
  if (n && !xy) return NAVGPU_ERR_INVALID;
  auto sign0 = [](double x) { return x < 0.0 ? -1.0 : (x > 0.0 ? 1.0 : 0.0); };
  for (uint32_t i = 0; i < 2 * n; ++i) xy[i] += sign0(xy[i]) * padding;
  return NAVGPU_OK;
}
int navgpu_footprint_from_radius(double radius, double* xy16) {
  if (!xy16) return NAVGPU_ERR_INVALID;
  const int N = 16;
  for (int i = 0; i < N; ++i) {
    const double angle = i * 2 * M_PI / N;
    xy16[2 * i] = cos(angle) * radius;
    xy16[2 * i + 1] = sin(angle) * radius;
  }
  return NAVGPU_OK;
}

int navgpu_device_sincos(int32_t device, const double* theta, uint32_t n, double* sin_out, double* cos_out) {
  if (!theta || !sin_out || !cos_out) return NAVGPU_ERR_INVALID;
  if (n == 0) return NAVGPU_OK;
  HIP_TRY(hipSetDevice(device));
  double* d = nullptr;
  HIP_TRY(hipMalloc(&d, (size_t)3 * n * sizeof(double)));
  int rc = NAVGPU_OK;
  if (hipMemcpy(d, theta, (size_t)n * sizeof(double), hipMemcpyHostToDevice) != hipSuccess) rc = NAVGPU_ERR_HIP;
  if (rc == NAVGPU_OK) {
    launch_sincos(d, n, d + n, d + 2 * (size_t)n, nullptr);
    if (hipMemcpy(sin_out, d + n, (size_t)n * sizeof(double), hipMemcpyDeviceToHost) != hipSuccess ||
        hipMemcpy(cos_out, d + 2 * (size_t)n, (size_t)n * sizeof(double), hipMemcpyDeviceToHost) != hipSuccess)
      rc = NAVGPU_ERR_HIP;
  }
  hipFree(d);
  return rc;
}

int navgpu_costmap_export(navgpu_fleet* f, uint32_t instance, uint32_t x0, uint32_t y0, uint32_t xn, uint32_t yn, int8_t* out) {
  if (!f || !out || instance >= f->desc.n_instances) return NAVGPU_ERR_INVALID;
  FleetGuard guard_(f);
  const CostmapDev& cm = f->cm;
  if (x0 >= xn || y0 >= yn || xn > cm.nx || yn > cm.ny) return NAVGPU_ERR_INVALID;
  if (!f->d_occ) {
    int rc = f->alloc(&f->d_occ, cm.cells);
    if (rc) return rc;
  }
  const uint32_t w = xn - x0, h = yn - y0;
  launch_export_window(cm.master + (size_t)instance * cm.cells_padded, cm.nx, x0, y0, w, h, f->d_occ, f->stream);
  HIP_TRY(hipMemcpyAsync(out, f->d_occ, (size_t)w * h, hipMemcpyDeviceToHost, f->stream));
  HIP_TRY(waitStream(f->stream));
  return checkLaunch();
}

int navgpu_static_set_map(navgpu_fleet* f, uint32_t first, uint32_t count, const int8_t* occ, int32_t track_unknown_space,
                          int32_t use_maximum, int32_t trinary, int32_t lethal_cost_threshold, int32_t unknown_cost_value) {
  if (!f || !occ || !f->rangeOk(first, count)) return NAVGPU_ERR_INVALID;
  FleetGuard guard_(f);
  CostmapDev& cm = f->cm;
  if (!cm.stat) return NAVGPU_ERR_STATE;
  if (!f->d_occ) {
    int rc = f->alloc(&f->d_occ, cm.cells);
    if (rc) return rc;
  }
  HIP_TRY(hipMemcpyAsync(f->d_occ, occ, cm.cells, hipMemcpyHostToDevice, f->stream));
  int lethal = std::max(std::min(lethal_cost_threshold, 100), 0);
  launch_static_interpret(cm.stat + (size_t)first * cm.cells_padded, f->d_occ, cm.cells, cm.cells_padded, count, track_unknown_space,
                          trinary, lethal, unknown_cost_value, f->stream);
  cm.static_use_maximum = use_maximum;
  cm.static_received = 1;
  std::vector<InstCostmapState> st(count);
  HIP_TRY(hipMemcpyAsync(st.data(), cm.state + first, sizeof(InstCostmapState) * count, hipMemcpyDeviceToHost, f->stream));
  HIP_TRY(waitStream(f->stream));
  for (auto& s : st) s.static_has_updated_data = 1;
  HIP_TRY(hipMemcpyAsync(cm.state + first, st.data(), sizeof(InstCostmapState) * count, hipMemcpyHostToDevice, f->stream));
  HIP_TRY(waitStream(f->stream));
  return checkLaunch();
}

int navgpu_static_set_rolling_map(navgpu_fleet* f, const int8_t* occ, uint32_t size_x, uint32_t size_y, double resolution, double origin_x,
                                  double origin_y, int32_t track_unknown_space, int32_t use_maximum, int32_t trinary, int32_t lethal_cost_threshold,
                                  int32_t unknown_cost_value) {
  if (!f || !occ || size_x == 0 || size_y == 0 || !(resolution > 0)) return NAVGPU_ERR_INVALID;
  FleetGuard guard_(f);
  CostmapDev& cm = f->cm;
  if (!f->desc.rolling_window || !(cm.layers & NAVGPU_LAYER_STATIC) || !cm.stat_tf) {
    g_last_error = "navgpu_static_set_rolling_map needs a rolling_window fleet with NAVGPU_LAYER_STATIC (else: navgpu_static_set_map)";
    return NAVGPU_ERR_STATE;
  }
  const size_t cells = (size_t)size_x * size_y;
  if (cells > 0xFFFFFFFFull) return NAVGPU_ERR_CAPACITY;
  HIP_TRY(waitStream(f->stream));
  int8_t* d_in = nullptr;
  uint8_t* d_map = nullptr;
  int rc = f->alloc(&d_in, cells);
  if (rc) return rc;
  if ((rc = f->alloc(&d_map, cells))) {
    f->release(d_in);
    return rc;
  }
  const int lethal = std::max(std::min(lethal_cost_threshold, 100), 0);
  hipError_t e = hipMemcpyAsync(d_in, occ, cells, hipMemcpyHostToDevice, f->stream);
  if (e == hipSuccess) {
    launch_static_interpret(d_map, d_in, (uint32_t)cells, (uint32_t)cells, 1, track_unknown_space, trinary, lethal, unknown_cost_value, f->stream);
    e = waitStream(f->stream);
  }
  f->release(d_in);
  if (e != hipSuccess) {
    f->release(d_map);
    g_last_error = std::string("navgpu_static_set_rolling_map: ") + hipGetErrorString(e);
    return NAVGPU_ERR_HIP;
  }
  if (cm.stat_roll) f->release(cm.stat_roll);
  cm.stat_roll = d_map;
  cm.stat_nx = size_x;
  cm.stat_ny = size_y;
  cm.stat_res = resolution;
  cm.stat_ox = origin_x;
  cm.stat_oy = origin_y;
  cm.static_use_maximum = use_maximum;
  cm.static_received = 1;
  f->touchInputs(0, f->desc.n_instances);
  return checkLaunch();
}

int navgpu_static_set_transform(navgpu_fleet* f, uint32_t first, uint32_t count, const double* m) {
  if (!f || !m || !f->rangeOk(first, count)) return NAVGPU_ERR_INVALID;
  FleetGuard guard_(f);
  if (!f->cm.stat_tf) return NAVGPU_ERR_STATE;
  HIP_TRY(hipMemcpyAsync(f->cm.stat_tf + (size_t)first * 12, m, sizeof(double) * 12 * count, hipMemcpyHostToDevice, f->stream));
  HIP_TRY(waitStream(f->stream));
  f->touchInputs(first, count);
  return NAVGPU_OK;
}

int navgpu_obstacle_configure(navgpu_fleet* f, const navgpu_obstacle_params* p) {
  if (!f || !p) return NAVGPU_ERR_INVALID;
  FleetGuard guard_(f);
  if (p->z_voxels < 0 || p->z_voxels > 16) return NAVGPU_ERR_INVALID;
  CostmapDev& cm = f->cm;
  f->obsp = *p;
  cm.obs_enabled = p->enabled;
  cm.footprint_clearing = p->footprint_clearing_enabled;
  cm.combination_method = p->combination_method;
  cm.max_obstacle_height = p->max_obstacle_height;
  if (cm.layers & NAVGPU_LAYER_VOXEL) {
    cm.z_voxels = p->z_voxels;
    cm.origin_z = p->origin_z;
    cm.z_resolution = p->z_resolution;
    cm.unknown_threshold = p->unknown_threshold;
    cm.mark_threshold = p->mark_threshold;
  }
  return NAVGPU_OK;
}

int navgpu_inflation_configure(navgpu_fleet* f, const navgpu_inflation_params* p) {
  if (!f || !p) return NAVGPU_ERR_INVALID;
  FleetGuard guard_(f);
  CostmapDev& cm = f->cm;
  if (p->cost_scaling_factor < 0) {
    g_last_error = "cost_scaling_factor < 0 is not supported";
    return NAVGPU_ERR_INVALID;
  }
  double cells_dist = std::max(0.0, ceil(p->inflation_radius / cm.res));
  if (cells_dist > 64) return NAVGPU_ERR_CAPACITY;
  const uint32_t R = (uint32_t)cells_dist;
  const uint32_t n = R + 2;
  std::vector<uint8_t> lut((size_t)n * n);
  for (uint32_t i = 0; i < n; ++i)
    for (uint32_t j = 0; j < n; ++j) {
      double distance = hypot(i, j);
      uint8_t cost = 0;
      if (distance == 0)
        cost = kLethal;
      else if (distance * cm.res <= p->inscribed_radius)
        cost = kInscribed;
      else {
        double euclidean_distance = distance * cm.res;
        double factor = exp(-1.0 * p->cost_scaling_factor * (euclidean_distance - p->inscribed_radius));
        cost = (uint8_t)((kInscribed - 1) * factor);
      }
      if (distance > R) cost = 0;
      lut[(size_t)i * n + j] = cost;
    }
  std::vector<uint16_t> dist_lut((size_t)n * n);
  const int want_pq = p->priority_queue_order ? 1 : 0;
  if (want_pq) {
    std::vector<double> d((size_t)n * n);
    for (uint32_t i = 0; i < n; ++i)
      for (uint32_t j = 0; j < n; ++j) d[(size_t)i * n + j] = hypot(i, j);
    std::vector<double> uniq(d);
    std::sort(uniq.begin(), uniq.end());
    uniq.erase(std::unique(uniq.begin(), uniq.end()), uniq.end());
    for (size_t k = 0; k < d.size(); ++k)
      dist_lut[k] = d[k] > (double)R ? (uint16_t)0xFFFFu : (uint16_t)(std::lower_bound(uniq.begin(), uniq.end(), d[k]) - uniq.begin());
    if (cm.nx > 65535 || cm.ny > 65535) return NAVGPU_ERR_CAPACITY;
    int rc;
    if (!cm.dist_lut && (rc = f->alloc(&cm.dist_lut, (size_t)66 * 66))) return rc;
    if (!cm.pq_seen && (rc = f->alloc(&cm.pq_seen, (size_t)f->desc.n_instances * cm.cells_padded))) return rc;
    if (!cm.pq_heap) {
      const uint64_t cap = (uint64_t)5 * cm.cells;
      if ((rc = f->alloc(&cm.pq_heap, (size_t)f->desc.n_instances * cap))) return rc;
      cm.pq_cap = cap;
    }
  }
  std::vector<uint8_t> lut2(256, 0);
  bool lut2_ok = R <= 14;
  if (lut2_ok) {
    for (uint32_t i = 0; i <= R; ++i)
      for (uint32_t j = 0; j <= R; ++j) {
        const uint32_t d2 = i * i + j * j;
        if (d2 < 256) lut2[d2] = std::max(lut2[d2], lut[(size_t)i * n + j]);
      }
    uint8_t prev = 255;
    for (uint32_t d2 = 0; d2 <= R * R; ++d2) {
      bool reachable = false;
      for (uint32_t i = 0; i * i <= d2 && !reachable; ++i) {
        const uint32_t rem = d2 - i * i, j = (uint32_t)llround(sqrt((double)rem));
        reachable = j * j == rem;
      }
      if (!reachable) continue;
      if (lut2[d2] > prev) lut2_ok = false;
      prev = lut2[d2];
    }
  }
  HIP_TRY(waitStream(f->stream));
  HIP_TRY(hipMemcpyAsync(cm.lut, lut.data(), lut.size(), hipMemcpyHostToDevice, f->stream));
  HIP_TRY(hipMemcpyAsync(cm.lut2, lut2.data(), lut2.size(), hipMemcpyHostToDevice, f->stream));
  if (want_pq) HIP_TRY(hipMemcpyAsync(cm.dist_lut, dist_lut.data(), sizeof(uint16_t) * dist_lut.size(), hipMemcpyHostToDevice, f->stream));
  HIP_TRY(waitStream(f->stream));
  cm.infl_pq = want_pq;
  cm.lut2_ok = lut2_ok ? 1 : 0;
  const bool changed = !f->inflation_configured || f->infl.inflation_radius != p->inflation_radius ||
                       f->infl.cost_scaling_factor != p->cost_scaling_factor || f->infl.inscribed_radius != p->inscribed_radius ||
                       f->infl.enabled != p->enabled || f->infl.priority_queue_order != p->priority_queue_order;
  f->infl = *p;
  f->inflation_configured = true;
  cm.R = R;
  cm.inflation_radius = p->inflation_radius;
  cm.infl_enabled = p->enabled;
  if (changed) {
    const uint32_t nI = f->desc.n_instances;
    std::vector<InstCostmapState> st(nI);
    HIP_TRY(hipMemcpyAsync(st.data(), cm.state, sizeof(InstCostmapState) * nI, hipMemcpyDeviceToHost, f->stream));
    HIP_TRY(waitStream(f->stream));
    for (auto& s : st) s.need_reinflation = 1;
    HIP_TRY(hipMemcpyAsync(cm.state, st.data(), sizeof(InstCostmapState) * nI, hipMemcpyHostToDevice, f->stream));
    HIP_TRY(waitStream(f->stream));
  }
  return NAVGPU_OK;
}

static void planWindow(const navgpu_fleet* f, PlannerDev& pl, const std::vector<uint32_t>& fp_n, const std::vector<double>& fp_spec, double fp_radius) {
  const navgpu_dwa_config& c = pl.cfg;
  double vmax;
  if (c.max_trans_vel >= 0)
    vmax = c.max_trans_vel + 1e-4;
  else
    vmax = hypot(std::max(fabs(c.min_vel_x), fabs(c.max_vel_x)), std::max(fabs(c.min_vel_y), fabs(c.max_vel_y)));
  double reach = vmax * c.sim_time + std::max(fp_radius, fabs(c.forward_point_distance));
  double cells = ceil(reach / pl.res) + 2;
  uint32_t win = (uint32_t)std::min(cells * 2 + 1, 240.0);
  pl.win = win;
  pl.fp_rcells = (uint32_t)ceil(fp_radius / pl.res) + 1;
  {
    const double rho = fp_radius / pl.res + 1.803 + 0.01;
    for (uint32_t d = 0; d < 32; ++d) {
      pl.fp_halfw[d] = 0xFF;
      if (d <= pl.fp_rcells && (double)d <= rho) pl.fp_halfw[d] = (uint8_t)std::min<double>(pl.fp_rcells, floor(sqrt(rho * rho - (double)d * d)));
    }
  }
  {
    double max_edge = 0.0;
    for (uint32_t i = 0; i < f->desc.n_instances; ++i) {
      const uint32_t nv = fp_n[i];
      const double* q = &fp_spec[(size_t)i * kMaxFootprint * 2];
      for (uint32_t a = 0; a < nv; ++a) {
        const uint32_t b = (a + 1) % nv;
        max_edge = std::max(max_edge, std::max(fabs(q[2 * a] - q[2 * b]), fabs(q[2 * a + 1] - q[2 * b + 1])));
        max_edge = std::max(max_edge, hypot(q[2 * a] - q[2 * b], q[2 * a + 1] - q[2 * b + 1]));
      }
    }
    pl.fp_chunk = (uint32_t)ceil(max_edge / pl.res) + 1;
  }
  uint32_t max_nfp = 0;
  for (uint32_t v : fp_n) max_nfp = std::max(max_nfp, v);
  pl.use_tables = 0;
  if (c.use_dwa && c.discretize_by_time && max_nfp <= 8) {
    pl.tab_steps = (uint32_t)ceil(c.sim_time / c.sim_granularity);
    pl.tab_dt = c.sim_time / (int)pl.tab_steps;
    pl.tab_nfp = max_nfp;
    pl.tab_nth = (uint32_t)std::max(c.vth_samples, 2) + 1;
    pl.tab_rows = pl.tab_steps >= 1 && pl.tab_steps <= pl.max_sim_steps && pl.tab_steps <= 127 ? score_table_rows(pl, win) : 0;
    if (pl.tab_rows >= 1) pl.use_tables = 1;
  }
}

static int allocPrep(navgpu_fleet* f, const PlannerDev& pl, uint8_t** fresh, uint32_t* stride) {
  PlannerDev tmp = pl;
  tmp.use_tables = 1;
  const size_t need = (score_prep_slot_bytes(tmp) + 255) & ~(size_t)255;
  *fresh = nullptr;
  *stride = f->pl.prep_stride;
  if (f->pl.prep && need <= f->pl.prep_stride) return NAVGPU_OK;
  int rc = f->alloc(fresh, (size_t)f->desc.n_instances * need);
  if (rc != NAVGPU_OK) return rc;
  *stride = (uint32_t)need;
  return NAVGPU_OK;
}

int navgpu_set_footprint(navgpu_fleet* f, uint32_t first, uint32_t count, const double* xy, uint32_t nv) {
  if (!f || !f->rangeOk(first, count) || (nv && !xy)) return NAVGPU_ERR_INVALID;
  FleetGuard guard_(f);
  if (nv > f->desc.max_footprint || nv > (uint32_t)kMaxFootprint) return NAVGPU_ERR_CAPACITY;
  std::vector<uint32_t> fp_n = f->h_fp_n;
  std::vector<double> fp_spec = f->h_fp_spec;
  double fp_radius = f->fp_radius;
  for (uint32_t i = first; i < first + count; ++i) {
    fp_n[i] = nv;
    for (uint32_t k = 0; k < nv * 2; ++k) fp_spec[(size_t)i * kMaxFootprint * 2 + k] = xy[k];
  }
  for (uint32_t k = 0; k < nv; ++k) fp_radius = std::max(fp_radius, hypot(xy[2 * k], xy[2 * k + 1]));
  if (fp_radius / f->cm.res > 500) return NAVGPU_ERR_CAPACITY;
  PlannerDev np = f->pl;
  uint8_t* fresh_prep = nullptr;
  uint32_t stride = f->pl.prep_stride;
  if (f->planner_configured) {
    planWindow(f, np, fp_n, fp_spec, fp_radius);
    int rc = allocPrep(f, np, &fresh_prep, &stride);
    if (rc != NAVGPU_OK) return rc;
  }
  hipError_t e = waitStream(f->stream);
  if (e == hipSuccess)
    e = hipMemcpyAsync(f->pl.fp_spec + (size_t)first * kMaxFootprint * 2, &fp_spec[(size_t)first * kMaxFootprint * 2], sizeof(double) * kMaxFootprint * 2 * count,
                       hipMemcpyHostToDevice, f->stream);
  if (e == hipSuccess) e = hipMemcpyAsync(f->pl.fp_n + first, &fp_n[first], sizeof(uint32_t) * count, hipMemcpyHostToDevice, f->stream);
  if (e == hipSuccess) e = waitStream(f->stream);
  if (e != hipSuccess) {
    if (fresh_prep) f->release(fresh_prep);
    g_last_error = std::string("navgpu_set_footprint: ") + hipGetErrorString(e);
    return NAVGPU_ERR_HIP;
  }
  f->h_fp_n.swap(fp_n);
  f->h_fp_spec.swap(fp_spec);
  f->fp_radius = fp_radius;
  if (f->planner_configured) {
    uint8_t* keep = fresh_prep ? fresh_prep : f->pl.prep;
    if (fresh_prep) f->release(f->pl.prep);
    f->pl = np;
    f->pl.prep = keep;
    f->pl.prep_stride = stride;
  }
  return NAVGPU_OK;
}

int navgpu_costmap_stage(navgpu_fleet* f, uint32_t first, uint32_t count, const double* poses, const navgpu_observation* obs,
                         uint32_t n_obs, const float* points, uint32_t n_points_total) {
  if (!f || !poses || !f->rangeOk(first, count) || (n_obs && (!obs || (!points && n_points_total)))) return NAVGPU_ERR_INVALID;
  FleetGuard guard_(f);
  CostmapDev& cm = f->cm;
  if (f->desc.rolling_window && f->shift_pending) return NAVGPU_ERR_STATE;
  if (f->desc.rolling_window) f->touchInputs(first, count);
  HIP_TRY(f->waitMirrors(f->ev_cm_h2d, f->ev_cm_set));
  for (uint32_t li = 0; li < count; ++li) f->hp_cnt[first + li] = f->hp_used[first + li] = 0;
  for (uint32_t k = 0; k < n_obs; ++k) {
    const navgpu_observation& o = obs[k];
    if (o.instance < first || o.instance >= first + count) return NAVGPU_ERR_INVALID;
    const uint32_t i = o.instance;
    if (f->hp_cnt[i] >= cm.max_obs || f->hp_used[i] + o.n_points > cm.max_points) return NAVGPU_ERR_CAPACITY;
    if ((uint64_t)o.first_point + o.n_points > n_points_total) return NAVGPU_ERR_INVALID;
    ObsCsr& d = f->hp_obs[(size_t)i * cm.max_obs + f->hp_cnt[i]++];
    d.first_point = f->hp_used[i];
    d.n_points = o.n_points;
    d.flags = o.flags;
    d.pad = 0;
    d.ox = o.origin_x;
    d.oy = o.origin_y;
    d.oz = o.origin_z;
    d.obstacle_range = o.obstacle_range;
    d.raytrace_range = o.raytrace_range;
    if (o.n_points)
      memcpy(&f->hp_pts[((size_t)i * cm.max_points + f->hp_used[i]) * 3], points + (size_t)o.first_point * 3, sizeof(float) * 3 * o.n_points);
    f->hp_used[i] += o.n_points;
  }
  if (f->desc.rolling_window) {
    const double size_m_x = (cm.nx - 1 + 0.5) * cm.res, size_m_y = (cm.ny - 1 + 0.5) * cm.res;
    for (uint32_t li = 0; li < count; ++li) {
      double& ox = f->h_origin[(size_t)(first + li) * 2];
      double& oy = f->h_origin[(size_t)(first + li) * 2 + 1];
      const double new_origin_x = poses[3 * li] - size_m_x / 2, new_origin_y = poses[3 * li + 1] - size_m_y / 2;
      const int cell_ox = int((new_origin_x - ox) / cm.res), cell_oy = int((new_origin_y - oy) / cm.res);
      ox = ox + cell_ox * cm.res;
      oy = oy + cell_oy * cm.res;
      f->hp_shift[2 * (first + li)] = cell_ox;
      f->hp_shift[2 * (first + li) + 1] = cell_oy;
    }
    HIP_TRY(hipMemcpyAsync(cm.shift + (size_t)first * 2, f->hp_shift + (size_t)first * 2, sizeof(int32_t) * 2 * count, hipMemcpyHostToDevice, f->stream));
    HIP_TRY(hipMemcpyAsync(cm.origin + (size_t)first * 2, &f->h_origin[(size_t)first * 2], sizeof(double) * 2 * count, hipMemcpyHostToDevice, f->stream));
    f->shift_pending = true;
    f->shift_first = first;
    f->shift_count = count;
  }
  for (uint32_t li = 0; li < count; ++li) {
    const uint32_t i = first + li;
    const double x = poses[3 * li], y = poses[3 * li + 1], th = poses[3 * li + 2];
    f->hp_pose[3 * i] = x;
    f->hp_pose[3 * i + 1] = y;
    f->hp_pose[3 * i + 2] = th;
    const double cos_th = cos(th), sin_th = sin(th);
    for (uint32_t v = 0; v < f->h_fp_n[i]; ++v) {
      const double sx = f->h_fp_spec[((size_t)i * kMaxFootprint + v) * 2], sy = f->h_fp_spec[((size_t)i * kMaxFootprint + v) * 2 + 1];
      f->hp_fpw[((size_t)i * kMaxFootprint + v) * 2] = x + (sx * cos_th - sy * sin_th);
      f->hp_fpw[((size_t)i * kMaxFootprint + v) * 2 + 1] = y + (sx * sin_th + sy * cos_th);
    }
  }
  memcpy(f->hp_fpn + first, &f->h_fp_n[first], sizeof(uint32_t) * count);
  if (first == 0 && count == f->desc.n_instances) {
    HIP_TRY(hipMemcpyAsync(f->cm_stage_dev, f->cm_stage_host, f->cm_stage_bytes, hipMemcpyHostToDevice, f->stream));
  } else {
    HIP_TRY(hipMemcpyAsync(cm.pose + (size_t)first * 3, f->hp_pose + (size_t)first * 3, sizeof(double) * 3 * count, hipMemcpyHostToDevice, f->stream));
    HIP_TRY(hipMemcpyAsync(cm.obs + (size_t)first * cm.max_obs, f->hp_obs + (size_t)first * cm.max_obs, sizeof(ObsCsr) * (size_t)count * cm.max_obs, hipMemcpyHostToDevice, f->stream));
    HIP_TRY(hipMemcpyAsync(cm.obs_count + first, f->hp_cnt + first, sizeof(uint32_t) * count, hipMemcpyHostToDevice, f->stream));
    HIP_TRY(hipMemcpyAsync(cm.points + (size_t)first * cm.max_points * 3, f->hp_pts + (size_t)first * cm.max_points * 3, sizeof(float) * 3 * (size_t)count * cm.max_points, hipMemcpyHostToDevice, f->stream));
    HIP_TRY(hipMemcpyAsync(cm.fp_world + (size_t)first * kMaxFootprint * 2, f->hp_fpw + (size_t)first * kMaxFootprint * 2, sizeof(double) * 2 * kMaxFootprint * (size_t)count, hipMemcpyHostToDevice, f->stream));
    HIP_TRY(hipMemcpyAsync(cm.fp_n + first, f->hp_fpn + first, sizeof(uint32_t) * count, hipMemcpyHostToDevice, f->stream));
  }
  if (f->cycles_in_flight > 1) {
    HIP_TRY(hipEventRecord(f->ev_cm_h2d, f->stream));
    f->ev_cm_set = true;
  }
  return NAVGPU_OK;
}

static int applyPendingShift(navgpu_fleet* f, uint32_t first, uint32_t count) {
  CostmapDev& cm = f->cm;
  if (!(f->desc.rolling_window && f->shift_pending)) return NAVGPU_OK;
  if (first != f->shift_first || count != f->shift_count) return NAVGPU_ERR_STATE;
  if (first != 0 || count != f->desc.n_instances) return NAVGPU_ERR_INVALID;
  launch_shift_u8(cm.master, cm.master_alt, cm, first, count, cm.master_default, f->stream);
  std::swap(cm.master, cm.master_alt);
  f->pl.master = cm.master;
  if (cm.obst) {
    launch_shift_u8(cm.obst, cm.obst_alt, cm, first, count, cm.obstacle_default, f->stream);
    std::swap(cm.obst, cm.obst_alt);
  }
  if (cm.voxel) {
    launch_shift_u32(cm.voxel, cm.voxel_alt, cm, first, count, 0x0000FFFFu, f->stream);
    std::swap(cm.voxel, cm.voxel_alt);
  }
  f->shift_pending = false;
  return NAVGPU_OK;
}

int navgpu_costmap_update(navgpu_fleet* f, uint32_t first, uint32_t count) {
  if (!f || !f->rangeOk(first, count)) return NAVGPU_ERR_INVALID;
  FleetGuard guard_(f);
  f->touchInputs(first, count);
  CostmapDev& cm = f->cm;
  if ((cm.layers & NAVGPU_LAYER_INFLATION) && !f->inflation_configured) return NAVGPU_ERR_STATE;
  {
    int rc = applyPendingShift(f, first, count);
    if (rc) return rc;
  }
  PROFILED(f, NAVGPU_K_OBSTACLE, launch_obstacle(cm, first, count, nullptr, 0, f->stream));
  PROFILED(f, NAVGPU_K_MERGE, launch_merge(cm, first, count, nullptr, f->stream));
  if (cm.layers & NAVGPU_LAYER_INFLATION) PROFILED(f, NAVGPU_K_INFLATE, launch_inflate(cm, first, count, nullptr, f->stream));
  return checkLaunch();
}

int navgpu_costmap_bounds(navgpu_fleet* f, uint32_t first, uint32_t count, int32_t* boxes) {
  if (!f || !boxes || !f->rangeOk(first, count)) return NAVGPU_ERR_INVALID;
  FleetGuard guard_(f);
  std::vector<InstCostmapState> st(count);
  HIP_TRY(hipMemcpyAsync(st.data(), f->cm.state + first, sizeof(InstCostmapState) * count, hipMemcpyDeviceToHost, f->stream));
  HIP_TRY(waitStream(f->stream));
  for (uint32_t i = 0; i < count; ++i)
    for (int k = 0; k < 4; ++k) boxes[4 * i + k] = st[i].box[k];
  return NAVGPU_OK;
}

int navgpu_inflate(navgpu_fleet* f, uint32_t first, uint32_t count, const int32_t* boxes) {
  if (!f || !f->rangeOk(first, count)) return NAVGPU_ERR_INVALID;
  FleetGuard guard_(f);
  f->touchInputs(first, count);
  if (!f->inflation_configured) return NAVGPU_ERR_STATE;
  const int32_t* d_boxes = nullptr;
  if (boxes) {
    HIP_TRY(hipMemcpyAsync(f->d_boxes_tmp, boxes, sizeof(int32_t) * 4 * count, hipMemcpyHostToDevice, f->stream));
    d_boxes = f->d_boxes_tmp;
  }
  PROFILED(f, NAVGPU_K_INFLATE, launch_inflate(f->cm, first, count, d_boxes, f->stream));
  if (boxes) HIP_TRY(waitStream(f->stream));
  return checkLaunch();
}

int navgpu_obstacle_update_bounds(navgpu_fleet* f, uint32_t first, uint32_t count, double* bounds) {
  if (!f || !bounds || !f->rangeOk(first, count)) return NAVGPU_ERR_INVALID;
  FleetGuard guard_(f);
  if (!f->cm.obst) return NAVGPU_ERR_STATE;
  {
    int rc = applyPendingShift(f, first, count);
    if (rc) return rc;
  }
  HIP_TRY(hipMemcpyAsync(f->d_bounds_tmp, bounds, sizeof(double) * 4 * count, hipMemcpyHostToDevice, f->stream));
  PROFILED(f, NAVGPU_K_OBSTACLE, launch_obstacle(f->cm, first, count, f->d_bounds_tmp, 1, f->stream));
  HIP_TRY(hipMemcpyAsync(bounds, f->d_bounds_tmp, sizeof(double) * 4 * count, hipMemcpyDeviceToHost, f->stream));
  HIP_TRY(waitStream(f->stream));
  return checkLaunch();
}

int navgpu_obstacle_update_costs(navgpu_fleet* f, uint32_t first, uint32_t count, const int32_t* boxes) {
  if (!f || !f->rangeOk(first, count)) return NAVGPU_ERR_INVALID;
  FleetGuard guard_(f);
  f->touchInputs(first, count);
  const int32_t* d_boxes = nullptr;
  if (boxes) {
    HIP_TRY(hipMemcpyAsync(f->d_boxes_tmp, boxes, sizeof(int32_t) * 4 * count, hipMemcpyHostToDevice, f->stream));
    d_boxes = f->d_boxes_tmp;
  }
  PROFILED(f, NAVGPU_K_MERGE, launch_merge(f->cm, first, count, d_boxes, f->stream, true));
  if (boxes) HIP_TRY(waitStream(f->stream));
  return checkLaunch();
}


static const int kBoxMarginCells = 4;
static double reachMetres(const navgpu_dwa_config& c, const float vel[3], const float* sample) {
  auto axis = [&](double lo, double hi, int a) {
    double b = std::max(std::max(fabs(lo), fabs(hi)), fabs((double)vel[a]));
    if (sample) b = std::max(fabs((double)sample[a]), fabs((double)vel[a]));
    return b;
  };
  const double bx = axis(c.min_vel_x, c.max_vel_x, 0), by = axis(c.min_vel_y, c.max_vel_y, 1);
  return hypot(bx, by) * c.sim_time * 1.001 + fabs(c.forward_point_distance);
}
static uint32_t bfsReachCells(const navgpu_fleet* f, const navgpu_robot_state& s, double goal_x, double goal_y) {
  if (!f->bounded_grids) return 0;
  if (f->pl.mg_generic) return 0;
  const double reach = reachMetres(f->pl.cfg, s.vel, nullptr);
  const double cells = ceil(reach / f->pl.res) + kBoxMarginCells;
  if (!(cells < 32768.0)) return 0;
  if (!(hypot(goal_x - s.pos[0], goal_y - s.pos[1]) > 2.0 * reach)) return 0;
  return (uint32_t)cells;
}
static bool robotBox(const navgpu_fleet* f, uint32_t i, const float pos[3], uint32_t reach, int32_t box[4]) {
  const double ox = f->h_origin[2 * i], oy = f->h_origin[2 * i + 1], res = f->pl.res;
  const double wx = pos[0], wy = pos[1];
  if (!reach || !(wx >= ox) || !(wy >= oy)) return false;
  const double fx = (wx - ox) / res, fy = (wy - oy) / res;
  if (!(fx < 2147483648.0) || !(fy < 2147483648.0)) return false;
  const int64_t mx = (int)fx, my = (int)fy;
  if (mx >= (int64_t)f->pl.nx || my >= (int64_t)f->pl.ny) return false;
  box[0] = (int32_t)std::max<int64_t>(mx - reach, 0);
  box[1] = (int32_t)std::min<int64_t>(mx + reach, f->pl.nx - 1);
  box[2] = (int32_t)std::max<int64_t>(my - reach, 0);
  box[3] = (int32_t)std::min<int64_t>(my + reach, f->pl.ny - 1);
  return true;
}
extern "C++" int navgpu::ensureCompleteGrids(navgpu_fleet* f, uint32_t first, uint32_t count) {
  if (NAVGPU_DEBUG_ENV("NAVGPU_DEBUG_RAW_GRIDS")) return NAVGPU_OK;
  for (uint32_t i = first; i < first + count; ++i)
    if (f->grid_partial[i] && f->cycle_gen[i] != f->inputs_gen[i]) {
      g_last_error = "MapGrids of instance " + std::to_string(i) + " were searched inside the robot's box only and the costmap / plan they came from has changed; "
                     "read them before the next update or call navgpu_planner_set_bounded_map_grids(f, 0)";
      return NAVGPU_ERR_STATE;
    }
  PlannerDev pl = f->pl;
  pl.bfs_bounded = 0;
  for (uint32_t i = first; i < first + count;) {
    if (!f->grid_partial[i]) {
      ++i;
      continue;
    }
    uint32_t j = i;
    while (j < first + count && f->grid_partial[j]) f->grid_partial[j++] = 0;
    launch_bfs(pl, i, j - i, f->stream);
    i = j;
  }
  return checkLaunch();
}

static int restageReach(navgpu_fleet* f) {
  if (!f->planner_staged) return NAVGPU_OK;
  PlannerDev& pl = f->pl;
  HIP_TRY(waitStream(f->stream));
  const uint32_t n = f->desc.n_instances;
  for (uint32_t i = 0; i < n; ++i) {
    const uint32_t np = f->hp_plan_cnt[i];
    if (!np) {
      f->hp_reach[i] = 0;
      continue;
    }
    const double* last = &f->hp_plan[((size_t)i * pl.max_plan + np - 1) * 2];
    f->hp_reach[i] = bfsReachCells(f, f->hp_state[i], last[0], last[1]);
  }
  HIP_TRY(hipMemcpyAsync(pl.bfs_reach, f->hp_reach, sizeof(uint32_t) * n, hipMemcpyHostToDevice, f->stream));
  f->hp_dma_pending = true;
  if (f->cycles_in_flight > 1) {
    HIP_TRY(hipEventRecord(f->ev_pl_h2d, f->stream));
    f->ev_pl_set = true;
  }
  return NAVGPU_OK;
}

int navgpu_planner_set_bounded_map_grids(navgpu_fleet* f, int32_t enable) {
  if (!f) return NAVGPU_ERR_INVALID;
  FleetGuard guard_(f);
  f->bounded_grids = enable != 0;
  return restageReach(f);
}
int navgpu_planner_set_map_grid_options(navgpu_fleet* f, int32_t critic, int32_t aggregation, double yshift) {
  if (!f || critic < 0 || critic > 3 || aggregation < 0 || aggregation > 2 || !std::isfinite(yshift)) return NAVGPU_ERR_INVALID;
  FleetGuard guard_(f);
  PlannerDev& pl = f->pl;
  pl.mg_agg[critic] = aggregation;
  pl.mg_yshift[critic] = yshift;
  pl.mg_generic = 0;
  for (int k = 0; k < 4; ++k)
    if (pl.mg_agg[k] != 0 || pl.mg_yshift[k] != 0.0) pl.mg_generic = 1;
  return restageReach(f);
}
int navgpu_planner_wavefront_levels(navgpu_fleet* f, uint32_t first, uint32_t count, uint32_t* levels) {
  if (!f || !levels || !f->rangeOk(first, count)) return NAVGPU_ERR_INVALID;
  FleetGuard guard_(f);
  HIP_TRY(hipMemcpyAsync(levels, f->pl.bfs_levels + (size_t)first * 3, sizeof(uint32_t) * 3 * count, hipMemcpyDeviceToHost, f->stream));
  HIP_TRY(waitStream(f->stream));
  return NAVGPU_OK;
}

int navgpu_planner_configure(navgpu_fleet* f, const navgpu_dwa_config* c) {
  if (!f || !c) return NAVGPU_ERR_INVALID;
  FleetGuard guard_(f);
  if (!(c->sim_time > 0) || !(c->sim_granularity > 0) || !(c->angular_sim_granularity > 0)) return NAVGPU_ERR_INVALID;
  PlannerDev& pl = f->pl;
  navgpu_dwa_config cfg = *c;
  if (cfg.vx_samples <= 0) cfg.vx_samples = 1;
  if (cfg.vy_samples <= 0) cfg.vy_samples = 1;
  if (cfg.vth_samples <= 0) cfg.vth_samples = 1;
  if (cfg.rollout_trig != 0 && cfg.rollout_trig != 1) return NAVGPU_ERR_INVALID;
  const uint32_t max_axis = (uint32_t)std::max(std::max(cfg.vx_samples, cfg.vy_samples), std::max(cfg.vth_samples, 2)) + 1;
  if (max_axis > 128) return NAVGPU_ERR_CAPACITY;
  double steps;
  if (cfg.discretize_by_time)
    steps = ceil(cfg.sim_time / cfg.sim_granularity);
  else {
    double vmax = cfg.max_trans_vel >= 0 ? cfg.max_trans_vel + 1e-4
                                         : hypot(std::max(fabs(cfg.min_vel_x), fabs(cfg.max_vel_x)), std::max(fabs(cfg.min_vel_y), fabs(cfg.max_vel_y)));
    steps = ceil(std::max(vmax * cfg.sim_time / cfg.sim_granularity, fabs(cfg.max_rot_vel) * cfg.sim_time / cfg.angular_sim_granularity)) + 1;
  }
  if (steps > pl.max_sim_steps) {
    g_last_error = "max_sim_steps too small for this sim_time / granularity";
    return NAVGPU_ERR_CAPACITY;
  }
  const uint32_t nI = f->desc.n_instances;
  const uint32_t ax = (uint32_t)(std::max(cfg.vx_samples, 2) + 1), ay = (uint32_t)(std::max(cfg.vy_samples, 2) + 1),
                 at = (uint32_t)(std::max(cfg.vth_samples, 2) + 1);
  const uint32_t max_samples = ax * ay * at;
  const uint32_t score_blocks = 2 * ((max_samples + std::min(kScoreThreads, NAVGPU_SCORE_TAB_THREADS) - 1) / std::min(kScoreThreads, NAVGPU_SCORE_TAB_THREADS)) + at + 2;
  PlannerDev np = pl;
  np.cfg = cfg;
  np.scale_path = pl.res * cfg.path_distance_bias * 0.5;
  np.scale_goal = pl.res * cfg.goal_distance_bias * 0.5;
  np.scale_obstacle = pl.res * cfg.occdist_scale;
  const bool resize = max_axis != pl.max_axis || max_samples != pl.max_samples;
  float* n_axis = nullptr;
  double* n_part_cost = nullptr;
  int32_t* n_part_index = nullptr;
  double* n_sample_cost = nullptr;
  int32_t* n_sample_status = nullptr;
  uint8_t* n_prep = nullptr;
  uint32_t n_stride = pl.prep_stride;
  auto dropNew = [&] {
    f->release(n_axis);
    f->release(n_part_cost);
    f->release(n_part_index);
    f->release(n_sample_cost);
    f->release(n_sample_status);
    f->release(n_prep);
  };
  int rc = NAVGPU_OK;
  if (resize) {
    np.max_axis = max_axis;
    np.max_samples = max_samples;
    np.score_blocks = score_blocks;
    if (!rc) rc = f->alloc(&n_axis, (size_t)nI * 3 * max_axis);
    if (!rc) rc = f->alloc(&n_part_cost, (size_t)nI * score_blocks);
    if (!rc) rc = f->alloc(&n_part_index, (size_t)nI * score_blocks);
    if (!rc && f->desc.keep_sample_costs) rc = f->alloc(&n_sample_cost, (size_t)nI * max_samples);
    if (!rc && f->desc.keep_sample_costs) rc = f->alloc(&n_sample_status, (size_t)nI * max_samples);
  }
  if (!rc) {
    planWindow(f, np, f->h_fp_n, f->h_fp_spec, f->fp_radius);
    rc = allocPrep(f, np, &n_prep, &n_stride);
  }
  if (!rc && waitStream(f->stream) != hipSuccess) rc = NAVGPU_ERR_HIP;
  if (rc) {
    dropNew();
    return rc;
  }
  if (resize) {
    f->release(pl.axis_samples);
    f->release(pl.part_cost);
    f->release(pl.part_index);
    f->release(pl.sample_cost);
    f->release(pl.sample_status);
    np.axis_samples = n_axis;
    np.part_cost = n_part_cost;
    np.part_index = n_part_index;
    np.sample_cost = n_sample_cost;
    np.sample_status = n_sample_status;
  }
  if (n_prep) {
    f->release(pl.prep);
    np.prep = n_prep;
    np.prep_stride = n_stride;
  }
  pl = np;
  f->planner_configured = true;
  f->touchInputs(0, nI);
  if ((rc = restageReach(f)) != NAVGPU_OK) return rc;
  HIP_TRY(waitStream(f->stream));
  return NAVGPU_OK;
}

int navgpu_planner_set_plan(navgpu_fleet* f, uint32_t first, uint32_t count) {
  if (!f || !f->rangeOk(first, count)) return NAVGPU_ERR_INVALID;
  FleetGuard guard_(f);
  HIP_TRY(hipMemsetAsync(f->pl.osc_flags + first, 0, sizeof(uint32_t) * count, f->stream));
  return NAVGPU_OK;
}

int navgpu_planner_stage(navgpu_fleet* f, uint32_t first, uint32_t count, const navgpu_robot_state* states, const double* plan_xy,
                         uint32_t n_plan_total) {
  if (!f || !states || !plan_xy || !f->rangeOk(first, count)) return NAVGPU_ERR_INVALID;
  FleetGuard guard_(f);
  if (!f->planner_configured) return NAVGPU_ERR_STATE;
  PlannerDev& pl = f->pl;
  const navgpu_dwa_config& c = pl.cfg;
  for (uint32_t li = 0; li < count; ++li) {
    const navgpu_robot_state& s = states[li];
    if (s.plan_count == 0) return NAVGPU_ERR_INVALID;
    if (s.plan_count > pl.max_plan) return NAVGPU_ERR_CAPACITY;
    if ((uint64_t)s.plan_first + s.plan_count > n_plan_total) return NAVGPU_ERR_INVALID;
  }
  HIP_TRY(f->waitMirrors(f->ev_pl_h2d, f->ev_pl_set));
  for (uint32_t li = 0; li < count; ++li) {
    const uint32_t i = first + li;
    const navgpu_robot_state& s = states[li];
    f->hp_state[i] = s;
    memcpy(&f->hp_plan[(size_t)i * pl.max_plan * 2], plan_xy + (size_t)s.plan_first * 2, sizeof(double) * 2 * s.plan_count);
    f->hp_plan_cnt[i] = s.plan_count;
    const double gx = plan_xy[((size_t)s.plan_first + s.plan_count - 1) * 2], gy = plan_xy[((size_t)s.plan_first + s.plan_count - 1) * 2 + 1];
    const double sq_dist = (s.pos[0] - gx) * (s.pos[0] - gx) + (s.pos[1] - gy) * (s.pos[1] - gy);
    const double angle_to_goal = atan2(gy - s.pos[1], gx - s.pos[0]);
    f->hp_front[2 * i] = gx + c.forward_point_distance * cos(angle_to_goal);
    f->hp_front[2 * i + 1] = gy + c.forward_point_distance * sin(angle_to_goal);
    f->hp_align[i] = sq_dist > c.forward_point_distance * c.forward_point_distance * c.cheat_factor ? 1 : 0;
    f->hp_reach[i] = bfsReachCells(f, s, gx, gy);
  }
  f->touchInputs(first, count);
  if (first == 0 && count == f->desc.n_instances) {
    HIP_TRY(hipMemcpyAsync(f->pl_stage_dev, f->pl_stage_host, f->pl_stage_bytes, hipMemcpyHostToDevice, f->stream));
  } else {
    HIP_TRY(hipMemcpyAsync(pl.state + first, f->hp_state + first, sizeof(navgpu_robot_state) * count, hipMemcpyHostToDevice, f->stream));
    HIP_TRY(hipMemcpyAsync(pl.plan + (size_t)first * pl.max_plan * 2, f->hp_plan + (size_t)first * pl.max_plan * 2, sizeof(double) * 2 * (size_t)count * pl.max_plan, hipMemcpyHostToDevice, f->stream));
    HIP_TRY(hipMemcpyAsync(pl.plan_count + first, f->hp_plan_cnt + first, sizeof(uint32_t) * count, hipMemcpyHostToDevice, f->stream));
    HIP_TRY(hipMemcpyAsync(pl.front_last + (size_t)first * 2, f->hp_front + (size_t)first * 2, sizeof(double) * 2 * count, hipMemcpyHostToDevice, f->stream));
    HIP_TRY(hipMemcpyAsync(pl.align_on + first, f->hp_align + first, sizeof(int32_t) * count, hipMemcpyHostToDevice, f->stream));
    HIP_TRY(hipMemcpyAsync(pl.bfs_reach + first, f->hp_reach + first, sizeof(uint32_t) * count, hipMemcpyHostToDevice, f->stream));
  }
  if (f->cycles_in_flight > 1) {
    HIP_TRY(hipEventRecord(f->ev_pl_h2d, f->stream));
    f->ev_pl_set = true;
  }
  f->planner_staged = true;
  f->hp_dma_pending = true;
  return NAVGPU_OK;
}

int navgpu_planner_stage_poses(navgpu_fleet* f, uint32_t first, uint32_t count, const float* pos_xyth, const float* vel_xyth) {
  if (!f || !pos_xyth || !vel_xyth || !f->rangeOk(first, count)) return NAVGPU_ERR_INVALID;
  FleetGuard guard_(f);
  if (!f->planner_configured || !f->planner_staged) return NAVGPU_ERR_STATE;
  PlannerDev& pl = f->pl;
  const navgpu_dwa_config& c = pl.cfg;
  for (uint32_t i = first; i < first + count; ++i)
    if (!f->hp_plan_cnt[i]) {
      g_last_error = "navgpu_planner_stage_poses: instance " + std::to_string(i) + " has no staged plan";
      return NAVGPU_ERR_STATE;
    }
  if (f->hp_dma_pending) {
    HIP_TRY(f->waitMirrors(f->ev_pl_h2d, f->ev_pl_set));
    f->hp_dma_pending = false;
  }
  for (uint32_t li = 0; li < count; ++li) {
    const uint32_t i = first + li;
    navgpu_robot_state& s = f->hp_state[i];
    for (int k = 0; k < 3; ++k) {
      s.pos[k] = pos_xyth[3 * li + k];
      s.vel[k] = vel_xyth[3 * li + k];
    }
    const double* last = &f->hp_plan[((size_t)i * pl.max_plan + f->hp_plan_cnt[i] - 1) * 2];
    const double gx = last[0], gy = last[1];
    const double sq_dist = (s.pos[0] - gx) * (s.pos[0] - gx) + (s.pos[1] - gy) * (s.pos[1] - gy);
    const double angle_to_goal = atan2(gy - s.pos[1], gx - s.pos[0]);
    f->hp_front[2 * i] = gx + c.forward_point_distance * cos(angle_to_goal);
    f->hp_front[2 * i + 1] = gy + c.forward_point_distance * sin(angle_to_goal);
    f->hp_align[i] = sq_dist > c.forward_point_distance * c.forward_point_distance * c.cheat_factor ? 1 : 0;
    f->hp_reach[i] = bfsReachCells(f, s, gx, gy);
  }
  f->touchInputs(first, count);
  PoseChunk ch;
  ch.state = pl.state;
  ch.front_last = pl.front_last;
  ch.align_on = pl.align_on;
  ch.bfs_reach = pl.bfs_reach;
  for (uint32_t at = 0; at < count; at += kPoseChunk) {
    ch.first = first + at;
    ch.count = std::min(kPoseChunk, count - at);
    memcpy(ch.st, f->hp_state + ch.first, sizeof(navgpu_robot_state) * ch.count);
    memcpy(ch.front, f->hp_front + (size_t)ch.first * 2, sizeof(double) * 2 * ch.count);
    memcpy(ch.align, f->hp_align + ch.first, sizeof(int32_t) * ch.count);
    memcpy(ch.reach, f->hp_reach + ch.first, sizeof(uint32_t) * ch.count);
    launch_stage_poses(ch, f->stream);
  }
  return checkLaunch();
}

int navgpu_planner_wavefront_boxes(navgpu_fleet* f, uint32_t first, uint32_t count, int32_t* boxes) {
  if (!f || !boxes || !f->rangeOk(first, count)) return NAVGPU_ERR_INVALID;
  FleetGuard guard_(f);
  for (uint32_t li = 0; li < count; ++li) {
    const uint32_t i = first + li;
    if (f->grid_partial[i])
      memcpy(boxes + 4 * li, &f->h_box[(size_t)4 * i], sizeof(int32_t) * 4);
    else {
      boxes[4 * li] = 0;
      boxes[4 * li + 1] = (int32_t)f->pl.nx - 1;
      boxes[4 * li + 2] = 0;
      boxes[4 * li + 3] = (int32_t)f->pl.ny - 1;
    }
  }
  return NAVGPU_OK;
}

#ifdef NAVGPU_DEBUG_SWITCHES
extern "C" int navgpu_debug_prep_image(navgpu_fleet* f, uint32_t inst, uint8_t* out, uint32_t cap, uint32_t* win, uint32_t* bytes) {
  waitStream(f->stream);
  const uint32_t n = std::min<uint32_t>(cap, f->pl.prep_stride);
  hipMemcpy(out, f->pl.prep + (size_t)inst * f->pl.prep_stride, n, hipMemcpyDeviceToHost);
  *win = f->pl.win;
  *bytes = n;
  return 0;
}
#endif
int navgpu_planner_cycle(navgpu_fleet* f, uint32_t first, uint32_t count) {
  if (!f || !f->rangeOk(first, count)) return NAVGPU_ERR_INVALID;
  FleetGuard guard_(f);
  if (!f->planner_configured || !f->planner_staged) return NAVGPU_ERR_STATE;
  PlannerDev& pl = f->pl;
  const int prev_slot = f->res_slot;
  if (f->cycles_in_flight > 1) {
    if (first != 0 || count != f->desc.n_instances) return NAVGPU_ERR_STATE;
    pl.result = f->hp_result + (size_t)(prev_slot ^ 1) * f->desc.n_instances;
  }
  pl.bfs_bounded = 1;
  for (uint32_t i = first; i < first + count; ++i) {
    f->grid_partial[i] = robotBox(f, i, f->hp_state[i].pos, f->hp_reach[i], &f->h_box[(size_t)4 * i]) ? 1 : 0;
    f->cycle_gen[i] = f->inputs_gen[i];
  }
  launch_samples(pl, first, count, f->stream);
#ifdef NAVGPU_DEBUG_SWITCHES
  if (getenv("NAVGPU_DEBUG_BFS_TRACE") && !pl.bfs_trace) f->alloc(&pl.bfs_trace, (size_t)f->desc.n_instances * 3 * 8);
#endif
  PROFILED(f, NAVGPU_K_BFS, launch_bfs(pl, first, count, f->stream, pl.bfs_order + (size_t)first * 3, true));
#ifdef NAVGPU_DEBUG_SWITCHES
  if (pl.bfs_trace) {
    std::vector<unsigned long long> h((size_t)count * 24);
    hipMemcpyAsync(h.data(), pl.bfs_trace, h.size() * 8, hipMemcpyDeviceToHost, f->stream);
    waitStream(f->stream);
    if (FILE* fp = fopen(getenv("NAVGPU_DEBUG_BFS_TRACE"), "w")) {
      for (size_t i = 0; i < (size_t)count * 3; ++i)
        fprintf(fp, "%zu %llu %llu %llu %llu %llu %llu %llu %llu\n", i, h[8 * i], h[8 * i + 1] & 0xFFFFFFFFFFFFull, h[8 * i + 1] >> 48, h[8 * i + 2], h[8 * i + 3], h[8 * i + 4], h[8 * i + 5], h[8 * i + 6]);
      fclose(fp);
    }
  }
#endif
  uint32_t n_blocks = 0;
  PROFILED(f, NAVGPU_K_SCORE, n_blocks = launch_score(pl, first, count, nullptr, f->stream));
  PROFILED(f, NAVGPU_K_SELECT, launch_select(pl, first, count, n_blocks, f->stream));
  int rc = checkLaunch();
  if (f->cycles_in_flight > 1) {
    const int slot = prev_slot ^ 1;
    if (rc == NAVGPU_OK && hipEventRecord(f->ev_cycle[slot], f->stream) != hipSuccess) rc = NAVGPU_ERR_HIP;
    if (rc == NAVGPU_OK) {
      f->res_slot = slot;
      f->ev_cycle_set[slot] = true;
    } else {
      pl.result = f->hp_result + (size_t)prev_slot * f->desc.n_instances;
    }
  }
  return rc;
}

int navgpu_planner_set_cycles_in_flight(navgpu_fleet* f, int32_t cycles) {
  if (!f || cycles < 1 || cycles > 2) return NAVGPU_ERR_INVALID;
  FleetGuard guard_(f);
  HIP_TRY(waitStream(f->stream));
  if (cycles > 1)
    for (hipEvent_t* e : {&f->ev_cycle[0], &f->ev_cycle[1], &f->ev_cm_h2d, &f->ev_pl_h2d})
      if (!*e) HIP_TRY(hipEventCreateWithFlags(e, hipEventDisableTiming));
  if (cycles == 1 && f->res_slot) {
    memcpy(f->hp_result, f->hp_result + f->desc.n_instances, sizeof(navgpu_plan_result) * f->desc.n_instances);
    f->res_slot = 0;
    f->pl.result = f->hp_result;
  }
  f->ev_cycle_set[0] = f->ev_cycle_set[1] = f->ev_cm_set = f->ev_pl_set = false;
  f->cycles_in_flight = cycles;
  return NAVGPU_OK;
}

int navgpu_planner_results_previous(navgpu_fleet* f, uint32_t first, uint32_t count, navgpu_plan_result* results) {
  if (!f || !results || !f->rangeOk(first, count)) return NAVGPU_ERR_INVALID;
  FleetGuard guard_(f);
  const int slot = f->res_slot ^ 1;
  if (f->cycles_in_flight < 2 || !f->ev_cycle_set[slot]) return NAVGPU_ERR_STATE;
  HIP_TRY(hipEventSynchronize(f->ev_cycle[slot]));
  memcpy(results, f->hp_result + (size_t)slot * f->desc.n_instances + first, sizeof(navgpu_plan_result) * count);
  return NAVGPU_OK;
}

int navgpu_planner_results(navgpu_fleet* f, uint32_t first, uint32_t count, navgpu_plan_result* results) {
  if (!f || !results || !f->rangeOk(first, count)) return NAVGPU_ERR_INVALID;
  FleetGuard guard_(f);
  HIP_TRY(waitStream(f->stream));
  memcpy(results, f->hp_result + (size_t)f->res_slot * f->desc.n_instances + first, sizeof(navgpu_plan_result) * count);
  return NAVGPU_OK;
}

int navgpu_planner_trajectory(navgpu_fleet* f, uint32_t instance, double* xyth, uint32_t cap) {
  if (!f || !xyth || instance >= f->desc.n_instances) return NAVGPU_ERR_INVALID;
  FleetGuard guard_(f);
  HIP_TRY(waitStream(f->stream));
  const navgpu_plan_result r = f->hp_result[(size_t)f->res_slot * f->desc.n_instances + instance];
  uint32_t n = std::min<uint32_t>(r.n_points > 0 ? r.n_points : 0, cap);
  if (n) {
    HIP_TRY(hipMemcpyAsync(xyth, f->pl.traj + (size_t)instance * f->pl.max_sim_steps * 3, sizeof(double) * 3 * n, hipMemcpyDeviceToHost, f->stream));
    HIP_TRY(waitStream(f->stream));
  }
  return r.n_points;
}

int navgpu_planner_samples(navgpu_fleet* f, uint32_t instance, double* costs, int32_t* status, float* vel, uint32_t cap) {
  if (!f || instance >= f->desc.n_instances) return NAVGPU_ERR_INVALID;
  FleetGuard guard_(f);
  PlannerDev& pl = f->pl;
  if (!pl.sample_cost) return NAVGPU_ERR_STATE;
  int32_t cnt[4];
  HIP_TRY(hipMemcpyAsync(cnt, pl.axis_count + 4 * instance, sizeof(cnt), hipMemcpyDeviceToHost, f->stream));
  HIP_TRY(waitStream(f->stream));
  const uint32_t n = std::min<uint32_t>(cnt[3], cap);
  if (costs && n) HIP_TRY(hipMemcpyAsync(costs, pl.sample_cost + (size_t)instance * pl.max_samples, sizeof(double) * n, hipMemcpyDeviceToHost, f->stream));
  if (status && n) HIP_TRY(hipMemcpyAsync(status, pl.sample_status + (size_t)instance * pl.max_samples, sizeof(int32_t) * n, hipMemcpyDeviceToHost, f->stream));
  std::vector<float> ax((size_t)3 * pl.max_axis);
  if (vel && n) HIP_TRY(hipMemcpyAsync(ax.data(), pl.axis_samples + (size_t)instance * 3 * pl.max_axis, sizeof(float) * ax.size(), hipMemcpyDeviceToHost, f->stream));
  HIP_TRY(waitStream(f->stream));
  if (vel)
    for (uint32_t s = 0; s < n; ++s) {
      const int ix = s / (cnt[1] * cnt[2]), rem = s - ix * (cnt[1] * cnt[2]), iy = rem / cnt[2], it = rem - iy * cnt[2];
      vel[3 * s] = ax[ix];
      vel[3 * s + 1] = ax[pl.max_axis + iy];
      vel[3 * s + 2] = ax[2 * pl.max_axis + it];
    }
  return cnt[3];
}

int navgpu_planner_check_trajectory(navgpu_fleet* f, uint32_t instance, const float vs[3], int32_t* ok) {
  if (!f || !vs || !ok || instance >= f->desc.n_instances) return NAVGPU_ERR_INVALID;
  FleetGuard guard_(f);
  if (!f->planner_configured || !f->planner_staged) return NAVGPU_ERR_STATE;
  PlannerDev& pl = f->pl;
  if (f->grid_partial[instance]) {
    const navgpu_robot_state& st = f->hp_state[instance];
    const uint32_t need = (uint32_t)std::min(ceil(reachMetres(pl.cfg, st.vel, vs) / pl.res) + 3.0, 32768.0);
    int32_t nb[4];
    const int32_t* hb = &f->h_box[(size_t)4 * instance];
    const bool inside = !pl.mg_generic && robotBox(f, instance, st.pos, need, nb) && nb[0] >= hb[0] && nb[1] <= hb[1] && nb[2] >= hb[2] && nb[3] <= hb[3];
    if (!inside) {
      int rc = ensureCompleteGrids(f, instance, 1);
      if (rc) return rc;
    }
  }
  HIP_TRY(hipMemsetAsync(pl.osc_flags + instance, 0, sizeof(uint32_t), f->stream));
  HIP_TRY(hipMemcpyAsync(f->d_explicit, vs, sizeof(float) * 3, hipMemcpyHostToDevice, f->stream));
  launch_score(pl, instance, 1, f->d_explicit, f->stream);
  double cost;
  int idx;
  HIP_TRY(hipMemcpyAsync(&cost, pl.part_cost + (size_t)instance * pl.score_blocks, sizeof(double), hipMemcpyDeviceToHost, f->stream));
  HIP_TRY(hipMemcpyAsync(&idx, pl.part_index + (size_t)instance * pl.score_blocks, sizeof(int), hipMemcpyDeviceToHost, f->stream));
  HIP_TRY(waitStream(f->stream));
  *ok = (idx != 0x7FFFFFFF) ? 1 : 0;
  return checkLaunch();
}

int navgpu_planner_cost_cloud(navgpu_fleet* f, uint32_t instance, float* points, uint32_t capacity) {
  if (!f || instance >= f->desc.n_instances || (capacity && !points)) return NAVGPU_ERR_INVALID;
  FleetGuard guard_(f);
  if (!f->planner_configured) return NAVGPU_ERR_STATE;
  {
    int rc = ensureCompleteGrids(f, instance, 1);
    if (rc) return rc;
  }
  const PlannerDev& pl = f->pl;
  if (!f->d_cell_costs) {
    int rc = f->alloc(&f->d_cell_costs, (size_t)pl.cells);
    if (rc) return rc;
  }
  launch_cell_costs(pl, instance, f->d_cell_costs, f->stream);
  std::vector<float4> h(pl.cells);
  HIP_TRY(hipMemcpyAsync(h.data(), f->d_cell_costs, sizeof(float4) * pl.cells, hipMemcpyDeviceToHost, f->stream));
  HIP_TRY(waitStream(f->stream));
  int rc = checkLaunch();
  if (rc) return rc;
  const double ox = f->h_origin[2 * instance], oy = f->h_origin[2 * instance + 1], res = pl.res;
  uint32_t n = 0;
  for (uint32_t cx = 0; cx < pl.nx; ++cx)
    for (uint32_t cy = 0; cy < pl.ny; ++cy) {
      const float4& c = h[(size_t)cy * pl.nx + cx];
      if (c.w != c.w) continue;
      if (n < capacity) {
        float* p = points + (size_t)7 * n;
        p[0] = (float)(ox + (cx + 0.5) * res);
        p[1] = (float)(oy + (cy + 0.5) * res);
        p[2] = 0.0f;
        p[3] = c.x;
        p[4] = c.y;
        p[5] = c.z;
        p[6] = c.w;
      }
      ++n;
    }
  return (int)n;
}

int navgpu_planner_get_oscillation(navgpu_fleet* f, uint32_t first, uint32_t count, uint32_t* flags, float* prev) {
  if (!f || !f->rangeOk(first, count)) return NAVGPU_ERR_INVALID;
  FleetGuard guard_(f);
  if (flags) HIP_TRY(hipMemcpyAsync(flags, f->pl.osc_flags + first, sizeof(uint32_t) * count, hipMemcpyDeviceToHost, f->stream));
  if (prev) HIP_TRY(hipMemcpyAsync(prev, f->pl.osc_prev + (size_t)first * 3, sizeof(float) * 3 * count, hipMemcpyDeviceToHost, f->stream));
  HIP_TRY(waitStream(f->stream));
  return NAVGPU_OK;
}
int navgpu_planner_set_oscillation(navgpu_fleet* f, uint32_t first, uint32_t count, const uint32_t* flags, const float* prev) {
  if (!f || !f->rangeOk(first, count)) return NAVGPU_ERR_INVALID;
  FleetGuard guard_(f);
  if (flags) HIP_TRY(hipMemcpyAsync(f->pl.osc_flags + first, flags, sizeof(uint32_t) * count, hipMemcpyHostToDevice, f->stream));
  if (prev) HIP_TRY(hipMemcpyAsync(f->pl.osc_prev + (size_t)first * 3, prev, sizeof(float) * 3 * count, hipMemcpyHostToDevice, f->stream));
  HIP_TRY(waitStream(f->stream));
  return NAVGPU_OK;
}

int navgpu_profile_enable(navgpu_fleet* f, int32_t enable) {
  if (!f) return NAVGPU_ERR_INVALID;
  FleetGuard guard_(f);
  if (!enable && f->profiling) {
    int rc = f->foldEvents();
    if (rc) return rc;
  }
  f->profiling = enable != 0;
  return NAVGPU_OK;
}
int navgpu_profile_select(navgpu_fleet* f, uint32_t kernel_mask) {
  if (!f) return NAVGPU_ERR_INVALID;
  FleetGuard guard_(f);
  f->prof_mask = kernel_mask;
  return NAVGPU_OK;
}
int navgpu_profile_reset(navgpu_fleet* f) {
  if (!f) return NAVGPU_ERR_INVALID;
  FleetGuard guard_(f);
  int rc = f->foldEvents();
  if (rc) return rc;
  for (int k = 0; k < NAVGPU_K_COUNT; ++k) {
    f->prof_ms[k] = 0;
    f->prof_n[k] = 0;
  }
  return NAVGPU_OK;
}
int navgpu_profile_read(navgpu_fleet* f, int32_t k, double* total_ms, uint64_t* launches) {
  if (!f || k < 0 || k >= NAVGPU_K_COUNT) return NAVGPU_ERR_INVALID;
  FleetGuard guard_(f);
  int rc = f->foldEvents();
  if (rc) return rc;
  if (total_ms) *total_ms = f->prof_ms[k];
  if (launches) *launches = f->prof_n[k];
  return NAVGPU_OK;
}

}
```

### navigation_amd/csrc/navgpu_tp.cpp

```cpp
#include "navgpu_fleet.h"

extern "C" {

namespace {
struct TpCell {
  int x, y;
};
bool hostWorldToMap(double ox, double oy, double res, uint32_t nx, uint32_t ny, double wx, double wy, uint32_t& mx, uint32_t& my) {
  if (wx < ox || wy < oy) return false;
  const double fx = (wx - ox) / res, fy = (wy - oy) / res;
  if (!(fx < 2147483648.0) || !(fy < 2147483648.0)) return false;
  mx = (uint32_t)(int)fx;
  my = (uint32_t)(int)fy;
  return mx < nx && my < ny;
}
void tpLineCells(int x0, int x1, int y0, int y1, std::vector<TpCell>& pts) {
  int deltax = abs(x1 - x0), deltay = abs(y1 - y0);
  int x = x0, y = y0;
  int xinc1, xinc2, yinc1, yinc2, den, num, numadd, numpixels;
  xinc1 = xinc2 = (x1 >= x0) ? 1 : -1;
  yinc1 = yinc2 = (y1 >= y0) ? 1 : -1;
  if (deltax >= deltay) {
    xinc1 = 0;
    yinc2 = 0;
    den = deltax;
    num = deltax / 2;
    numadd = deltay;
    numpixels = deltax;
  } else {
    xinc2 = 0;
    yinc1 = 0;
    den = deltay;
    num = deltay / 2;
    numadd = deltax;
    numpixels = deltay;
  }
  for (int curpixel = 0; curpixel <= numpixels; curpixel++) {
    pts.push_back(TpCell{x, y});
    num += numadd;
    if (num >= den) {
      num -= den;
      x += xinc1;
      y += yinc1;
    }
    x += xinc2;
    y += yinc2;
  }
}
void tpFillCells(std::vector<TpCell>& fp) {
  unsigned int i = 0;
  while (i < fp.size() - 1) {
    if (fp[i].x > fp[i + 1].x) {
      std::swap(fp[i], fp[i + 1]);
      if (i > 0) --i;
    } else {
      ++i;
    }
  }
  i = 0;
  TpCell min_pt, max_pt;
  const unsigned int min_x = fp[0].x, max_x = fp[fp.size() - 1].x;
  for (unsigned int x = min_x; x <= max_x; ++x) {
    if (i >= fp.size() - 1) break;
    if (fp[i].y < fp[i + 1].y) {
      min_pt = fp[i];
      max_pt = fp[i + 1];
    } else {
      min_pt = fp[i + 1];
      max_pt = fp[i];
    }
    i += 2;
    while (i < fp.size() && (unsigned int)fp[i].x == x) {
      if (fp[i].y < min_pt.y)
        min_pt = fp[i];
      else if (fp[i].y > max_pt.y)
        max_pt = fp[i];
      ++i;
    }
    for (unsigned int y = min_pt.y; y < (unsigned int)max_pt.y; ++y) fp.push_back(TpCell{(int)x, (int)y});
  }
}
void tpFootprintCells(const float pos[3], const double* spec, uint32_t nfp, double ox, double oy, double res, uint32_t nx, uint32_t ny,
                      std::vector<TpCell>& cells) {
  const double x_i = pos[0], y_i = pos[1], theta_i = pos[2];
  cells.clear();
  if (nfp <= 1) {
    uint32_t mx, my;
    if (hostWorldToMap(ox, oy, res, nx, ny, x_i, y_i, mx, my)) cells.push_back(TpCell{(int)mx, (int)my});
    return;
  }
  const double cos_th = cos(theta_i), sin_th = sin(theta_i);
  uint32_t x0, y0, x1, y1;
  const uint32_t last = nfp - 1;
  auto vertex = [&](uint32_t i, uint32_t& mx, uint32_t& my) {
    const double wx = x_i + (spec[2 * i] * cos_th - spec[2 * i + 1] * sin_th);
    const double wy = y_i + (spec[2 * i] * sin_th + spec[2 * i + 1] * cos_th);
    return hostWorldToMap(ox, oy, res, nx, ny, wx, wy, mx, my);
  };
  for (uint32_t i = 0; i < last; ++i) {
    if (!vertex(i, x0, y0)) return;
    if (!vertex(i + 1, x1, y1)) return;
    tpLineCells((int)x0, (int)x1, (int)y0, (int)y1, cells);
  }
  if (!vertex(last, x0, y0)) return;
  if (!vertex(0, x1, y1)) return;
  tpLineCells((int)x0, (int)x1, (int)y0, (int)y1, cells);
  tpFillCells(cells);
}
struct TpPlanned {
  double vx, vy, vth;
  double vth_unlimited;
  int stage;
};
}

static uint32_t tpMaxSamples(const navgpu_tp_config& c) {
  return (uint32_t)(c.vx_samples * c.vtheta_samples + 2 + c.vtheta_samples + c.n_y_vels + 1);
}

int navgpu_tp_configure(navgpu_fleet* f, const navgpu_tp_config* cfg_in) {
  if (!f || !cfg_in) return NAVGPU_ERR_INVALID;
  FleetGuard guard_(f);
  navgpu_tp_config c = *cfg_in;
  if (c.n_y_vels < 0 || c.n_y_vels > 8 || !(c.sim_time > 0) || !(c.sim_granularity > 0) || !(c.angular_sim_granularity > 0))
    return NAVGPU_ERR_INVALID;
  if (c.vx_samples <= 0) c.vx_samples = 1;
  if (c.vtheta_samples <= 0) c.vtheta_samples = 1;
  double ymax = 0.1;
  for (int i = 0; i < c.n_y_vels; ++i) ymax = std::max(ymax, fabs(c.y_vels[i]));
  const double vxmax = std::max(std::max(fabs(c.max_vel_x), fabs(c.min_vel_x)), std::max(fabs(c.backup_vel), 0.1));
  const double wmax = std::max(std::max(fabs(c.max_vel_th), fabs(c.min_vel_th)), fabs(c.min_in_place_vel_th));
  const double steps = (c.heading_scoring ? c.sim_time / c.sim_granularity
                                          : std::max(hypot(vxmax, ymax) * c.sim_time / c.sim_granularity, wmax / c.angular_sim_granularity)) + 1.5;
  if (steps > (double)f->pl.max_sim_steps) {
    g_last_error = "navgpu_tp_configure: trajectories need more points than max_sim_steps";
    return NAVGPU_ERR_CAPACITY;
  }
  HIP_TRY(waitStream(f->stream));
  TpDev& tp = f->tp;
  const uint32_t n = f->desc.n_instances;
  const uint32_t ms = tpMaxSamples(c);
  if (!f->tp_configured || ms > tp.max_samples) {
    f->release(tp.samples);
    f->release(tp.out);
    tp.samples = nullptr;
    tp.out = nullptr;
    int rc = f->alloc(&tp.samples, (size_t)n * ms * 3);
    if (rc) return rc;
    rc = f->alloc(&tp.out, (size_t)n * ms);
    if (rc) return rc;
    tp.max_samples = ms;
  }
  if (!f->tp_configured) {
    const uint32_t W = (f->cm.nx + 31) / 32;
    int rc = f->alloc(&tp.n_samples, n);
    if (!rc) rc = f->alloc(&tp.start, (size_t)n * 6);
    if (!rc) rc = f->alloc(&tp.winner, n);
    if (!rc) rc = f->alloc(&tp.points, (size_t)n * f->pl.max_sim_steps * 3);
    if (!rc) rc = f->alloc(&tp.within_count, n);
    if (!rc) rc = f->alloc(&tp.within_bits, (size_t)n * f->cm.ny * W);
    if (rc) return rc;
    f->tph.assign(n, navgpu_fleet::TpHost());
  }
  tp.cfg = c;
  f->tp_h_samples.assign((size_t)n * tp.max_samples * 3, 0.0);
  f->tp_h_out.assign((size_t)n * tp.max_samples, TpOut());
  f->tp_h_start.assign((size_t)n * 6, 0.0);
  f->tp_h_nsamples.assign(n, 0);
  f->tp_h_within_count.assign(n, 0);
  f->tp_h_winner.assign(n, -1);
  f->tp_configured = true;
  HIP_TRY(waitStream(f->stream));
  return NAVGPU_OK;
}

static int tpLaunchGrids(navgpu_fleet* f, uint32_t first, uint32_t count, bool with_within) {
  PlannerDev pl = f->pl;
  pl.bfs_grids = 2;
  pl.within = with_within ? f->tp.within_bits : nullptr;
  pl.cfg.allow_unknown = f->tp.cfg.allow_unknown;
  pl.bfs_bounded = 0;
  for (uint32_t i = first; i < first + count; ++i) f->grid_partial[i] = 0;
  PROFILED(f, NAVGPU_K_BFS, launch_bfs(pl, first, count, f->stream));
  return NAVGPU_OK;
}
static int tpUploadPlans(navgpu_fleet* f, uint32_t first, uint32_t count) {
  PlannerDev& pl = f->pl;
  for (uint32_t i = first; i < first + count; ++i) {
    const std::vector<double>& p = f->tph[i].plan;
    const uint32_t np = (uint32_t)(p.size() / 2);
    if (np > pl.max_plan) return NAVGPU_ERR_CAPACITY;
    if (np) memcpy(&f->hp_plan[(size_t)i * pl.max_plan * 2], p.data(), sizeof(double) * p.size());
    f->hp_plan_cnt[i] = np;
  }
  HIP_TRY(hipMemcpyAsync(pl.plan + (size_t)first * pl.max_plan * 2, f->hp_plan + (size_t)first * pl.max_plan * 2,
                         sizeof(double) * 2 * (size_t)count * pl.max_plan, hipMemcpyHostToDevice, f->stream));
  HIP_TRY(hipMemcpyAsync(pl.plan_count + first, f->hp_plan_cnt + first, sizeof(uint32_t) * count, hipMemcpyHostToDevice, f->stream));
  return NAVGPU_OK;
}

int navgpu_tp_update_plan(navgpu_fleet* f, uint32_t instance, const double* plan_xy, uint32_t n, int32_t compute_dists) {
  if (!f || instance >= f->desc.n_instances || (n && !plan_xy)) return NAVGPU_ERR_INVALID;
  FleetGuard guard_(f);
  if (!f->tp_configured) return NAVGPU_ERR_STATE;
  if (n > f->pl.max_plan) return NAVGPU_ERR_CAPACITY;
  navgpu_fleet::TpHost& h = f->tph[instance];
  h.plan.assign(plan_xy, plan_xy + 2 * (size_t)n);
  if (n) {
    h.final_goal_x = plan_xy[2 * (size_t)(n - 1)];
    h.final_goal_y = plan_xy[2 * (size_t)(n - 1) + 1];
    h.final_goal_position_valid = true;
  } else {
    h.final_goal_position_valid = false;
  }
  if (compute_dists) {
    int rc = tpUploadPlans(f, instance, 1);
    if (rc) return rc;
    rc = tpLaunchGrids(f, instance, 1, false);
    if (rc) return rc;
    HIP_TRY(waitStream(f->stream));
    return checkLaunch();
  }
  return NAVGPU_OK;
}

static inline bool tpFlag(const navgpu_tp_state& s, uint32_t bit) { return (s.flags & bit) != 0; }
static inline void tpSet(navgpu_tp_state& s, uint32_t bit, bool v) { s.flags = v ? (s.flags | bit) : (s.flags & ~bit); }

int navgpu_tp_find_best_path(navgpu_fleet* f, uint32_t first, uint32_t count, const navgpu_robot_state* states, navgpu_tp_result* results) {
  if (!f || !states || !results || !f->rangeOk(first, count)) return NAVGPU_ERR_INVALID;
  FleetGuard guard_(f);
  if (!f->tp_configured) return NAVGPU_ERR_STATE;
  TpDev& tp = f->tp;
  const navgpu_tp_config& c = tp.cfg;
  const CostmapDev& cm = f->cm;
  const uint32_t ms = tp.max_samples;
  std::vector<std::vector<TpPlanned>> planned(count);
  std::vector<double> dvth(count, 0.0);
  std::vector<std::vector<TpCell>> cells(count);
  size_t max_cells = 0;
  for (uint32_t k = 0; k < count; ++k) {
    const uint32_t inst = first + k;
    navgpu_fleet::TpHost& h = f->tph[inst];
    if (c.simple_attractor && h.plan.empty()) {
      g_last_error = "navgpu_tp_find_best_path: simple_attractor needs a plan";
      return NAVGPU_ERR_STATE;
    }
    const float* pos = states[k].pos;
    const float* vel = states[k].vel;
    tpFootprintCells(pos, &f->h_fp_spec[(size_t)inst * kMaxFootprint * 2], f->h_fp_n[inst], f->h_origin[2 * inst],
                     f->h_origin[2 * inst + 1], cm.res, cm.nx, cm.ny, cells[k]);
    max_cells = std::max(max_cells, cells[k].size());
    const double x = pos[0], y = pos[1], vx = vel[0], vtheta = vel[2];
    const double acc_x = c.acc_lim_x, acc_theta = c.acc_lim_theta;
    double* st = &f->tp_h_start[(size_t)inst * 6];
    st[0] = x;
    st[1] = y;
    st[2] = pos[2];
    st[3] = vx;
    st[4] = vel[1];
    st[5] = vtheta;
    double max_vel_x = c.max_vel_x, max_vel_theta, min_vel_x, min_vel_theta;
    if (h.final_goal_position_valid) {
      const double final_goal_dist = hypot(h.final_goal_x - x, h.final_goal_y - y);
      max_vel_x = std::min(max_vel_x, final_goal_dist / c.sim_time);
    }
    const double horizon = c.dwa ? c.sim_period : c.sim_time;
    max_vel_x = std::max(std::min(max_vel_x, vx + acc_x * horizon), c.min_vel_x);
    min_vel_x = std::max(c.min_vel_x, vx - acc_x * horizon);
    max_vel_theta = std::min(c.max_vel_th, vtheta + acc_theta * horizon);
    min_vel_theta = std::max(c.min_vel_th, vtheta - acc_theta * horizon);
    const double dvx = (max_vel_x - min_vel_x) / (c.vx_samples - 1);
    const double dvtheta = (max_vel_theta - min_vel_theta) / (c.vtheta_samples - 1);
    dvth[k] = dvtheta;
    std::vector<TpPlanned>& P = planned[k];
    double vx_samp = min_vel_x, vtheta_samp = min_vel_theta, vy_samp = 0.0;
    if (!tpFlag(h.st, NAVGPU_TP_ESCAPING)) {
      for (int i = 0; i < c.vx_samples; ++i) {
        vtheta_samp = 0;
        P.push_back(TpPlanned{vx_samp, vy_samp, vtheta_samp, 0, 0});
        vtheta_samp = min_vel_theta;
        for (int j = 0; j < c.vtheta_samples - 1; ++j) {
          P.push_back(TpPlanned{vx_samp, vy_samp, vtheta_samp, 0, 0});
          vtheta_samp += dvtheta;
        }
        vx_samp += dvx;
      }
      if (c.holonomic_robot) {
        P.push_back(TpPlanned{0.1, 0.1, 0.0, 0, 1});
        P.push_back(TpPlanned{0.1, -0.1, 0.0, 0, 1});
      }
    }
    vtheta_samp = min_vel_theta;
    for (int i = 0; i < c.vtheta_samples; ++i) {
      const double lim = vtheta_samp > 0 ? std::max(vtheta_samp, c.min_in_place_vel_th) : std::min(vtheta_samp, -1.0 * c.min_in_place_vel_th);
      P.push_back(TpPlanned{0.0, 0.0, lim, vtheta_samp, 2});
      vtheta_samp += dvtheta;
    }
    if (c.holonomic_robot)
      for (int i = 0; i < c.n_y_vels; ++i) P.push_back(TpPlanned{0.0, c.y_vels[i], 0.0, 0, 3});
    P.push_back(TpPlanned{c.backup_vel, 0.0, 0.0, 0, 4});
    if (P.size() > ms) return NAVGPU_ERR_CAPACITY;
    f->tp_h_nsamples[inst] = (uint32_t)P.size();
    for (size_t q = 0; q < P.size(); ++q) {
      double* d = &f->tp_h_samples[((size_t)inst * ms + q) * 3];
      d[0] = P[q].vx;
      d[1] = P[q].vy;
      d[2] = P[q].vth;
    }
  }
  if (max_cells > tp.max_within || !tp.within_cells) {
    HIP_TRY(waitStream(f->stream));
    f->release(tp.within_cells);
    tp.within_cells = nullptr;
    tp.max_within = (uint32_t)std::max<size_t>(max_cells * 2, 256);
    int rc = f->alloc(&tp.within_cells, (size_t)f->desc.n_instances * tp.max_within);
    if (rc) return rc;
    f->tp_h_within.assign((size_t)f->desc.n_instances * tp.max_within, 0);
  }
  for (uint32_t k = 0; k < count; ++k) {
    const uint32_t inst = first + k;
    f->tp_h_within_count[inst] = (uint32_t)cells[k].size();
    for (size_t q = 0; q < cells[k].size(); ++q)
      f->tp_h_within[(size_t)inst * tp.max_within + q] = (uint32_t)cells[k][q].y * cm.nx + (uint32_t)cells[k][q].x;
  }
  int rc = tpUploadPlans(f, first, count);
  if (rc) return rc;
  HIP_TRY(hipMemcpyAsync(tp.within_cells + (size_t)first * tp.max_within, &f->tp_h_within[(size_t)first * tp.max_within],
                         sizeof(uint32_t) * (size_t)count * tp.max_within, hipMemcpyHostToDevice, f->stream));
  HIP_TRY(hipMemcpyAsync(tp.within_count + first, &f->tp_h_within_count[first], sizeof(uint32_t) * count, hipMemcpyHostToDevice, f->stream));
  HIP_TRY(hipMemcpyAsync(tp.samples + (size_t)first * ms * 3, &f->tp_h_samples[(size_t)first * ms * 3], sizeof(double) * 3 * (size_t)count * ms,
                         hipMemcpyHostToDevice, f->stream));
  HIP_TRY(hipMemcpyAsync(tp.n_samples + first, &f->tp_h_nsamples[first], sizeof(uint32_t) * count, hipMemcpyHostToDevice, f->stream));
  HIP_TRY(hipMemcpyAsync(tp.start + (size_t)first * 6, &f->tp_h_start[(size_t)first * 6], sizeof(double) * 6 * count, hipMemcpyHostToDevice, f->stream));
  launch_tp_within(f->pl, tp, first, count, f->stream);
  rc = tpLaunchGrids(f, first, count, true);
  if (rc) return rc;
  PROFILED(f, NAVGPU_K_SCORE, launch_tp_rollout(f->pl, tp, first, count, 0, f->stream));
  HIP_TRY(hipMemcpyAsync(&f->tp_h_out[(size_t)first * ms], tp.out + (size_t)first * ms, sizeof(TpOut) * (size_t)count * ms, hipMemcpyDeviceToHost, f->stream));
  HIP_TRY(waitStream(f->stream));
  rc = checkLaunch();
  if (rc) return rc;
  for (uint32_t k = 0; k < count; ++k) {
    const uint32_t inst = first + k;
    navgpu_fleet::TpHost& h = f->tph[inst];
    navgpu_tp_state& S = h.st;
    const std::vector<TpPlanned>& P = planned[k];
    const TpOut* O = &f->tp_h_out[(size_t)inst * ms];
    const double x = states[k].pos[0], y = states[k].pos[1], theta = states[k].pos[2];
    const double dvtheta = dvth[k];
    h.made.clear();
    int best = -1;
    int best_made = -1;
    double best_cost = -1.0, best_xv = 0, best_yv = 0, best_thv = 0;
    auto made = [&](size_t q) {
      h.made.push_back(navgpu_tp_sample{P[q].vx, P[q].vy, P[q].vth, O[q].cost, O[q].n_points, 0});
    };
    auto take = [&](size_t q) {
      best = (int)q;
      best_made = (int)h.made.size() - 1;
      best_cost = O[q].cost;
      best_xv = P[q].vx;
      best_yv = P[q].vy;
      best_thv = P[q].vth;
    };
    size_t q = 0;
    for (; q < P.size() && P[q].stage <= 1; ++q) {
      made(q);
      if (O[q].cost >= 0 && (O[q].cost < best_cost || best_cost < 0)) take(q);
    }
    double heading_dist = DBL_MAX;
    for (; q < P.size() && P[q].stage == 2; ++q) {
      made(q);
      const double vtheta_samp = P[q].vth_unlimited;
      if (O[q].cost >= 0 && (O[q].cost <= best_cost || best_cost < 0 || best_yv != 0.0) &&
          (vtheta_samp > dvtheta || vtheta_samp < -1 * dvtheta)) {
        if (O[q].ahead_ok) {
          const double ahead_gdist = O[q].ahead;
          if (ahead_gdist < heading_dist) {
            if (vtheta_samp < 0 && !tpFlag(S, NAVGPU_TP_STUCK_LEFT)) {
              take(q);
              heading_dist = ahead_gdist;
            } else if (vtheta_samp > 0 && !tpFlag(S, NAVGPU_TP_STUCK_RIGHT)) {
              take(q);
              heading_dist = ahead_gdist;
            }
          }
        }
      }
    }
    auto resetOscillationIfMoved = [&]() {
      const double dist = hypot(x - S.prev_x, y - S.prev_y);
      if (dist > c.oscillation_reset_dist)
        S.flags &= ~(NAVGPU_TP_ROTATING_LEFT | NAVGPU_TP_ROTATING_RIGHT | NAVGPU_TP_STRAFE_LEFT | NAVGPU_TP_STRAFE_RIGHT |
                     NAVGPU_TP_STUCK_LEFT | NAVGPU_TP_STUCK_RIGHT | NAVGPU_TP_STUCK_LEFT_STRAFE | NAVGPU_TP_STUCK_RIGHT_STRAFE);
    };
    auto resetEscapeIfMoved = [&]() {
      const double dist = hypot(x - S.escape_x, y - S.escape_y);
      if (dist > c.escape_reset_dist || fabs(navgpu_shortest_angular_distance(S.escape_theta, theta)) > c.escape_reset_theta)
        tpSet(S, NAVGPU_TP_ESCAPING, false);
    };
    bool finished = false;
    if (best_cost >= 0) {
      if (!(best_xv > 0)) {
        if (best_thv < 0) {
          if (tpFlag(S, NAVGPU_TP_ROTATING_RIGHT)) tpSet(S, NAVGPU_TP_STUCK_RIGHT, true);
          tpSet(S, NAVGPU_TP_ROTATING_RIGHT, true);
        } else if (best_thv > 0) {
          if (tpFlag(S, NAVGPU_TP_ROTATING_LEFT)) tpSet(S, NAVGPU_TP_STUCK_LEFT, true);
          tpSet(S, NAVGPU_TP_ROTATING_LEFT, true);
        } else if (best_yv > 0) {
          if (tpFlag(S, NAVGPU_TP_STRAFE_RIGHT)) tpSet(S, NAVGPU_TP_STUCK_RIGHT_STRAFE, true);
          tpSet(S, NAVGPU_TP_STRAFE_RIGHT, true);
        } else if (best_yv < 0) {
          if (tpFlag(S, NAVGPU_TP_STRAFE_LEFT)) tpSet(S, NAVGPU_TP_STUCK_LEFT_STRAFE, true);
          tpSet(S, NAVGPU_TP_STRAFE_LEFT, true);
        }
        S.prev_x = x;
        S.prev_y = y;
      }
      resetOscillationIfMoved();
      resetEscapeIfMoved();
      finished = true;
    }
    if (!finished) {
      for (; q < P.size() && P[q].stage == 3; ++q) {
        made(q);
        const double vy_samp = P[q].vy;
        if (O[q].cost >= 0 && (O[q].cost <= best_cost || best_cost < 0)) {
          if (O[q].ahead_ok) {
            const double ahead_gdist = O[q].ahead;
            if (ahead_gdist < heading_dist) {
              if (vy_samp > 0 && !tpFlag(S, NAVGPU_TP_STUCK_LEFT_STRAFE)) {
                take(q);
                heading_dist = ahead_gdist;
              } else if (vy_samp < 0 && !tpFlag(S, NAVGPU_TP_STUCK_RIGHT_STRAFE)) {
                take(q);
                heading_dist = ahead_gdist;
              }
            }
          }
        }
      }
      if (best_cost >= 0) {
        if (!(best_xv > 0)) {
          if (best_thv < 0) {
            if (tpFlag(S, NAVGPU_TP_ROTATING_RIGHT)) tpSet(S, NAVGPU_TP_STUCK_RIGHT, true);
            tpSet(S, NAVGPU_TP_ROTATING_LEFT, true);
          } else if (best_thv > 0) {
            if (tpFlag(S, NAVGPU_TP_ROTATING_LEFT)) tpSet(S, NAVGPU_TP_STUCK_LEFT, true);
            tpSet(S, NAVGPU_TP_ROTATING_RIGHT, true);
          } else if (best_yv > 0) {
            if (tpFlag(S, NAVGPU_TP_STRAFE_RIGHT)) tpSet(S, NAVGPU_TP_STUCK_RIGHT_STRAFE, true);
            tpSet(S, NAVGPU_TP_STRAFE_LEFT, true);
          } else if (best_yv < 0) {
            if (tpFlag(S, NAVGPU_TP_STRAFE_LEFT)) tpSet(S, NAVGPU_TP_STUCK_LEFT_STRAFE, true);
            tpSet(S, NAVGPU_TP_STRAFE_RIGHT, true);
          }
          S.prev_x = x;
          S.prev_y = y;
        }
        resetOscillationIfMoved();
        resetEscapeIfMoved();
        finished = true;
      }
    }
    if (!finished) {
      while (q < P.size() && P[q].stage != 4) ++q;
      made(q);
      take(q);
      resetOscillationIfMoved();
      if (!tpFlag(S, NAVGPU_TP_ESCAPING) && best_cost > -2.0) {
        S.escape_x = x;
        S.escape_y = y;
        S.escape_theta = theta;
        tpSet(S, NAVGPU_TP_ESCAPING, true);
      }
      resetEscapeIfMoved();
      if (best_cost == -1.0) best_cost = 1.0;
    }
    navgpu_tp_result& r = results[k];
    r = navgpu_tp_result();
    r.n_samples = (int32_t)h.made.size();
    r.cost = best_cost;
    if (best >= 0) {
// ... 85 lines not shown
```

### navigation_amd/csrc/planner_samples.hip

```cpp
#include "planner_common.h"

namespace navgpu {

constexpr int kSamplesThreads = 128;
__global__ __launch_bounds__(kSamplesThreads) void k_samples(PlannerDev pl, uint32_t first, uint32_t count) {
  const uint32_t tid = threadIdx.x & 63u, wv = threadIdx.x >> 6;
  if (blockIdx.x >= 2 * count) {
    const uint32_t W = (pl.nx + 31) >> 5, words = pl.ny * W, per = (words + kSamplesThreads - 1) / kSamplesThreads;
    const uint32_t b = blockIdx.x - 2 * count, r = b / per, i = (b - r * per) * kSamplesThreads + threadIdx.x;
    if (i < words) {
      const uint32_t row = i / W, wi = i - row * W;
      pl.bfs_free[(size_t)(first + r) * words + i] = bfsFreeWord(pl.master + (size_t)(first + r) * pl.cells_padded, row, pl.nx, wi, pl.cfg.allow_unknown != 0 ? 0u : 1u);
    }
    return;
  }
  const navgpu_dwa_config& c = pl.cfg;
  if (blockIdx.x >= count) {
    const uint32_t robot = blockIdx.x - count, inst = first + robot;
    if (wv == 0) {
      const uint32_t total = 3 * count;
      uint32_t key[3], before[3] = {0, 0, 0};
#pragma unroll
      for (uint32_t g = 0; g < 3; ++g) key[g] = pl.bfs_levels[(size_t)inst * 3 + (2 - g)];
#pragma unroll 4
      for (uint32_t j = tid; j < total; j += 64) {
        const uint32_t gj = j / count, rj = j - gj * count;
        const uint32_t kj = pl.bfs_levels[(size_t)(first + rj) * 3 + (2 - gj)];
#pragma unroll
        for (uint32_t g = 0; g < 3; ++g) before[g] += (kj > key[g] || (kj == key[g] && j < g * count + robot)) ? 1u : 0u;
      }
#pragma unroll
      for (uint32_t g = 0; g < 3; ++g)
        for (int o = 32; o > 0; o >>= 1) before[g] += __shfl_xor(before[g], o);
      if (tid < 3) pl.bfs_order[(size_t)first * 3 + (tid == 0 ? before[0] : (tid == 1 ? before[1] : before[2]))] = tid * count + robot;
      if (robot == 0 && tid < 2) pl.bfs_next_item[tid] = 0;
      return;
    }
    const navgpu_robot_state st = pl.state[inst];
    int32_t* cnt = pl.axis_count + 4 * inst;
    int n = 0;
    if (tid < 3) {
      const int a = tid;
      const float vsamp = a == 0 ? (float)c.vx_samples : (a == 1 ? (float)c.vy_samples : (float)c.vth_samples);
      const double max_vel_th = c.max_rot_vel, min_vel_th = -1.0 * max_vel_th;
      double lim_min = a == 0 ? c.min_vel_x : (a == 1 ? c.min_vel_y : min_vel_th);
      double lim_max = a == 0 ? c.max_vel_x : (a == 1 ? c.max_vel_y : max_vel_th);
      const float acc = a == 0 ? (float)c.acc_lim_x : (a == 1 ? (float)c.acc_lim_y : (float)c.acc_lim_theta);
      const float v = st.vel[a];
      float maxv, minv;
      if (!c.use_dwa) {
        const double* P = pl.plan + (size_t)inst * pl.max_plan * 2;
        const uint32_t np = pl.plan_count[inst];
        const float gx = (float)P[2 * (np - 1)], gy = (float)P[2 * (np - 1) + 1];
        double dist = hyp2((double)(gx - st.pos[0]), (double)(gy - st.pos[1]));
        if (a < 2) lim_max = fmax(fmin(lim_max, dist / c.sim_time), lim_min);
        maxv = (float)fmin(lim_max, v + acc * c.sim_time);
        minv = (float)fmax(lim_min, v - acc * c.sim_time);
      } else {
        maxv = (float)fmin(lim_max, v + acc * c.sim_period);
        minv = (float)fmax(lim_min, v - acc * c.sim_period);
      }
      float* out = pl.axis_samples + ((size_t)inst * 3 + a) * pl.max_axis;
      const double mn = minv, mx = maxv;
      if (mn == mx) {
        out[n++] = (float)mn;
      } else {
        int num_samples = (int)vsamp;
        num_samples = num_samples > 2 ? num_samples : 2;
        double step_size = (mx - mn) / double(num_samples - 1 > 1 ? num_samples - 1 : 1);
        double current, next = mn;
        for (int j = 0; j < num_samples - 1; ++j) {
          current = next;
          next += step_size;
          if (n < (int)pl.max_axis) out[n] = (float)current;
          ++n;
          if ((current < 0) && (next > 0)) {
            if (n < (int)pl.max_axis) out[n] = 0.0f;
            ++n;
          }
        }
        if (n < (int)pl.max_axis) out[n] = (float)mx;
        ++n;
      }
      n = n < (int)pl.max_axis ? n : (int)pl.max_axis;
      cnt[a] = n;
    }
    const int n0 = __shfl(n, 0), n1 = __shfl(n, 1), n2 = __shfl(n, 2);
    if (tid == 0) {
      float prod = (float)c.vx_samples * (float)c.vy_samples * (float)c.vth_samples;
      cnt[3] = prod > 0 ? n0 * n1 * n2 : 0;
      pl.counters[2 * inst] = 0;
      pl.counters[2 * inst + 1] = 0;
    }
    return;
  }
  const uint32_t inst = first + blockIdx.x;
  const navgpu_robot_state st = pl.state[inst];
  __shared__ uint32_t s_pocket[2][2][kCareWords][64];
  __shared__ int s_ok[2];
  {
    int4 region = make_int4(0, -1, 0, -1);
    int care_ok = 0;
    const uint32_t reach = pl.bfs_reach[inst];
    const Geom g = geomOf(pl, inst);
    uint32_t mx = 0, my = 0;
    if (reach && worldToMap(g, (double)st.pos[0], (double)st.pos[1], mx, my)) {
      const int R = (int)reach + 2, nxi = (int)pl.nx, nyi = (int)pl.ny, Wm = (nxi + 31) >> 5;
      region.x = max((int)mx - R, 0);
      region.y = min((int)mx + R, nxi - 1);
      region.z = max((int)my - R, 0);
      region.w = min((int)my + R, nyi - 1);
      const int rows = region.w - region.z + 1, wx0 = region.x >> 5, nw = (region.y >> 5) - wx0 + 1;
      if (rows <= kCareRows && nw <= kCareWords) {
        const uint8_t* master = pl.master + (size_t)inst * pl.cells_padded;
        const uint32_t unknown_is_obstacle = pl.cfg.allow_unknown != 0 ? 0u : 1u;
        const int bx0 = max((int)mx - (int)reach, 0), bx1 = min((int)mx + (int)reach, nxi - 1);
        const int by0 = max((int)my - (int)reach, 0), by1 = min((int)my + (int)reach, nyi - 1);
        const int fy0 = max(min((int)my - kCareRows / 2, nyi - kCareRows), 0), fy1 = min(fy0 + kCareRows - 1, nyi - 1);
        const int fw0 = max(min(wx0 - (kCareWords - nw) / 2, Wm - kCareWords), 0), fw1 = min(fw0 + kCareWords - 1, Wm - 1);
        const int fx0 = fw0 * 32, fx1 = min(fw1 * 32 + 31, nxi - 1);
        auto colMask = [&](int w, int x0, int x1) -> uint32_t {
          const int lo = max(x0 - (fw0 + w) * 32, 0), hi = min(x1 - (fw0 + w) * 32, 31);
          return hi >= lo ? ((0xFFFFFFFFu >> (31 - hi)) & (0xFFFFFFFFu << lo)) : 0u;
        };
        const int ax0 = wv ? fx0 : region.x, ax1 = wv ? fx1 : region.y, ay0 = wv ? fy0 : region.z, ay1 = wv ? fy1 : region.w;
        uint32_t fm[2][kCareWords], F[2][kCareWords];
        uint32_t fword[2][kCareWords];
        if ((pl.nx & 15u) == 0 && (uint32_t)(fw1 * 32 + 31) < pl.nx) {
          uint4 ca[2][kCareWords], cb[2][kCareWords];
#pragma unroll
          for (int h = 0; h < 2; ++h)
#pragma unroll
            for (int w = 0; w < kCareWords; ++w) {
              const uint4* p = reinterpret_cast<const uint4*>(master + (size_t)min(fy0 + 2 * (int)tid + h, fy1) * pl.nx + (size_t)min(fw0 + w, fw1) * 32);
              ca[h][w] = p[0];
              cb[h][w] = p[1];
            }
#pragma unroll
          for (int h = 0; h < 2; ++h)
#pragma unroll
            for (int w = 0; w < kCareWords; ++w) {
              const uint4 a = ca[h][w], b = cb[h][w];
              fword[h][w] = ~(bfsObstacleNibble(a.x, unknown_is_obstacle) | (bfsObstacleNibble(a.y, unknown_is_obstacle) << 4) |
                              (bfsObstacleNibble(a.z, unknown_is_obstacle) << 8) | (bfsObstacleNibble(a.w, unknown_is_obstacle) << 12) |
                              (bfsObstacleNibble(b.x, unknown_is_obstacle) << 16) | (bfsObstacleNibble(b.y, unknown_is_obstacle) << 20) |
                              (bfsObstacleNibble(b.z, unknown_is_obstacle) << 24) | (bfsObstacleNibble(b.w, unknown_is_obstacle) << 28));
            }
        } else {
#pragma unroll
          for (int h = 0; h < 2; ++h)
#pragma unroll
            for (int w = 0; w < kCareWords; ++w) {
              const int row = fy0 + 2 * (int)tid + h;
              fword[h][w] = (row <= fy1 && fw0 + w <= fw1) ? bfsFreeWord(master, (uint32_t)row, pl.nx, (uint32_t)(fw0 + w), unknown_is_obstacle) : 0u;
            }
        }
#pragma unroll
        for (int h = 0; h < 2; ++h) {
          const int row = fy0 + 2 * (int)tid + h;
          const bool in_a = row >= ay0 && row <= ay1;
#pragma unroll
          for (int w = 0; w < kCareWords; ++w) {
            fm[h][w] = F[h][w] = 0;
            if (row <= fy1 && fw0 + w <= fw1) {
              const uint32_t cm = in_a ? colMask(w, ax0, ax1) : 0u;
              const uint32_t fw_ = fword[h][w];
              fm[h][w] = fw_ & cm;
              const uint32_t rim = (row == ay0 || row == ay1) ? cm : (colMask(w, ax0, ax0) | colMask(w, ax1, ax1));
              F[h][w] = fm[h][w] & rim;
            }
          }
        }
        bool ok = false;
        for (int it = 0; it < 256; ++it) {
          uint32_t changed = 0;
#pragma unroll
          for (int h = 0; h < 2; ++h) {
#pragma unroll
            for (int w = 0; w < kCareWords; ++w) {
              uint32_t up, dn;
              if (h == 0) {
                up = __shfl_up(F[1][w], 1);
                if (tid == 0) up = 0;
                dn = F[1][w];
              } else {
                up = F[0][w];
                dn = __shfl_down(F[0][w], 1);
                if (tid == 63) dn = 0;
              }
              const uint32_t cur = F[h][w], f = fm[h][w];
              uint32_t n = cur | up | dn | (cur << 1) | (cur >> 1);
              if (w > 0) n |= F[h][w - 1] >> 31;
              if (w + 1 < kCareWords) n |= F[h][w + 1] << 31;
              n &= f;
              n |= f & ~(f + n);
              const uint32_t fr_ = __brev(f), nr = __brev(n);
              n |= __brev(fr_ & ~(fr_ + nr));
              changed |= n ^ cur;
              F[h][w] = n;
            }
          }
          if (__builtin_amdgcn_ballot_w64(changed != 0) == 0) {
            ok = true;
            break;
          }
        }
#pragma unroll
        for (int h = 0; h < 2; ++h)
#pragma unroll
          for (int w = 0; w < kCareWords; ++w) s_pocket[wv][h][w][tid] = fm[h][w] & ~F[h][w];
        if (tid == 0) s_ok[wv] = ok ? 1 : 0;
        __syncthreads();
        const bool okR = s_ok[0] != 0, okL = s_ok[1] != 0;
        care_ok = okR ? 1 : 0;
        uint32_t extra = 0;
#pragma unroll
        for (int h = 0; h < 2; ++h) {
          const int row = fy0 + 2 * (int)tid + h;
#pragma unroll
          for (int w = 0; w < kCareWords; ++w)
            if (row >= by0 && row <= by1) extra |= (s_pocket[1][h][w][tid] ^ s_pocket[0][h][w][tid]) & colMask(w, bx0, bx1);
        }
        const bool large = okR && okL && __builtin_amdgcn_ballot_w64(extra != 0) != 0;
        if (large) region = make_int4(fx0, fx1, fy0, fy1);
        if (okR && wv == 0) {
          const int ry0 = region.z, rw0 = region.x >> 5;
          uint32_t* care = pl.bfs_care + (size_t)inst * kCareRows * kCareWords;
#pragma unroll
          for (int h = 0; h < 2; ++h) {
            const int row = fy0 + 2 * (int)tid + h, rr = row - ry0;
#pragma unroll
            for (int w = 0; w < kCareWords; ++w) {
              const int ww = fw0 + w - rw0;
              if (rr < 0 || rr >= kCareRows || row > region.w || ww < 0 || ww >= kCareWords) continue;
              const uint32_t pocket = s_pocket[large ? 1 : 0][h][w][tid];
              care[rr * kCareWords + ww] = (row >= by0 && row <= by1) ? (colMask(w, bx0, bx1) & ~pocket) : 0u;
            }
          }
        }
      }
    }
    if (threadIdx.x == 0) {
      int* b = pl.bfs_box + (size_t)inst * 8;
      b[0] = region.x;
      b[1] = region.y;
      b[2] = region.z;
      b[3] = region.w;
      b[4] = care_ok;
    }
  }
}
void launch_samples(const PlannerDev& pl, uint32_t first, uint32_t count, hipStream_t s) {
  const uint32_t words = pl.ny * ((pl.nx + 31) / 32);
  hipLaunchKernelGGL(k_samples, dim3(2 * count + count * ((words + kSamplesThreads - 1) / kSamplesThreads)), dim3(kSamplesThreads), 0, s, pl, first, count);
}

}
```

Baseline: 5.621 billion.

## Maintain BFS free-bit map incrementally inside inflation and row-tile merge

The inflation kernel now also updates the planner's packed free-cell bitmap for cells it touches inside the update box. The samples kernel can then skip its full-map bitmap rebuild when the bitmap is still valid. Every host path that changes the master grid clears a per-instance validity flag to force a rebuild. Separately, merge gets a row-aligned 3D grid variant so each 16-cell group stays within one row. In exchange, inflation reads the whole box, tracks ballots, and does extra read-modify-write stores, and correctness depends on every mutation path clearing the validity flag.

```diff
diff --git a/navigation_amd/csrc/costmap_kernels.hip b/navigation_amd/csrc/costmap_kernels.hip
--- a/navigation_amd/csrc/costmap_kernels.hip
+++ b/navigation_amd/csrc/costmap_kernels.hip
@@ -627,14 +627,16 @@
     hipLaunchKernelGGL(k_obstacle<false>, dim3(count), dim3(256), 0, s, cm, first, bounds_in, bounds_out, only_bounds);
 }
 
+template <bool ROWS>
 __global__ __launch_bounds__(256) void k_merge(CostmapDev cm, uint32_t first, const int32_t* boxes, int static_received, int layer_only) {
-  const uint32_t inst = first + blockIdx.y;
+  const uint32_t rb = ROWS ? blockIdx.z : blockIdx.y;
+  const uint32_t inst = first + rb;
   int x0, xn, y0, yn;
   if (boxes) {
-    x0 = boxes[4 * blockIdx.y + 0];
-    y0 = boxes[4 * blockIdx.y + 1];
-    xn = boxes[4 * blockIdx.y + 2];
-    yn = boxes[4 * blockIdx.y + 3];
+    x0 = boxes[4 * rb + 0];
+    y0 = boxes[4 * rb + 1];
+    xn = boxes[4 * rb + 2];
+    yn = boxes[4 * rb + 3];
   } else {
     const InstCostmapState* st = cm.state + inst;
     if (!st->box_valid) return;
@@ -643,10 +645,20 @@
     y0 = st->box[2];
     yn = st->box[3];
   }
-  const uint32_t q = blockIdx.x * blockDim.x + threadIdx.x;
-  const uint32_t base = q * 16;
-  if (base >= cm.cells) return;
-  const int row_first = base / cm.nx, row_last = (min(base + 15, cm.cells - 1)) / cm.nx;
+  uint32_t base;
+  int row_first, row_last;
+  if (ROWS) {
+    const uint32_t row = blockIdx.y * 16u + (threadIdx.x >> 4), gx = (blockIdx.x * 16u + (threadIdx.x & 15u)) * 16u;
+    if (row >= cm.ny || gx >= cm.nx) return;
+    row_first = row_last = (int)row;
+    base = row * cm.nx + gx;
+  } else {
+    const uint32_t q = blockIdx.x * blockDim.x + threadIdx.x;
+    base = q * 16;
+    if (base >= cm.cells) return;
+    row_first = base / cm.nx;
+    row_last = (min(base + 15, cm.cells - 1)) / cm.nx;
+  }
   if (row_last < y0 || row_first >= yn) return;
   bool inside = false;
   if (row_first == row_last) {
@@ -720,9 +732,14 @@
 }
 
 void launch_merge(const CostmapDev& cm, uint32_t first, uint32_t count, const int32_t* boxes, hipStream_t s, bool layer_only) {
+  if ((cm.nx & 15u) == 0 && count <= 65535u) {
+    dim3 grid((cm.nx / 16 + 15) / 16, (cm.ny + 15) / 16, count);
+    hipLaunchKernelGGL(k_merge<true>, grid, dim3(256), 0, s, cm, first, boxes, cm.static_received, layer_only ? 1 : 0);
+    return;
+  }
   uint32_t groups = (cm.cells + 15) / 16;
   dim3 grid((groups + 255) / 256, count);
-  hipLaunchKernelGGL(k_merge, grid, dim3(256), 0, s, cm, first, boxes, cm.static_received, layer_only ? 1 : 0);
+  hipLaunchKernelGGL(k_merge<false>, grid, dim3(256), 0, s, cm, first, boxes, cm.static_received, layer_only ? 1 : 0);
 }
 
 constexpr int kTile = 64;
@@ -809,7 +826,7 @@
 }
 
 constexpr int kBX = 64, kBY = 32;
-template <int RT>
+template <int RT, bool BITS>
 __global__ __launch_bounds__(256) void k_inflate_bits(CostmapDev cm, uint32_t first, uint32_t count, const int32_t* boxes) {
   const uint32_t tbx = blockIdx.x >> 3, tby = blockIdx.y, rz = blockIdx.z * 8u + (blockIdx.x & 7u);
   if (rz >= count) return;
@@ -829,12 +846,14 @@
     min_j = st->box[2];
     max_j = st->box[3];
   }
+  const int bx0 = max(min_i, 0), bxn = min(max_i, (int)cm.nx), by0 = max(min_j, 0), byn = min(max_j, (int)cm.ny);
   min_i = max(0, min_i - R);
   min_j = max(0, min_j - R);
   max_i = min((int)cm.nx, max_i + R);
   max_j = min((int)cm.ny, max_j + R);
   const int tx0 = (int)tbx * kBX, ty0 = (int)tby * kBY;
   if (tx0 - R >= max_i || tx0 + kBX + R <= min_i || ty0 - R >= max_j || ty0 + kBY + R <= min_j) return;
+  const bool tile_in_box = BITS && tx0 < bxn && tx0 + kBX > bx0 && ty0 < byn && ty0 + kBY > by0;
 
   constexpr int kMaxHR = kBY + 2 * 14;
   constexpr int kOct = (kMaxHR + 7) / 8;
@@ -895,9 +914,10 @@
     if (rows_hi) atomicOr(&s_rowany[1], rows_hi);
   }
   __syncthreads();
-  if (!s_any) return;
+  const bool seeds = s_any != 0;
+  if (!seeds && !tile_in_box) return;
   const uint32_t lowmask = (1u << R) - 1u;
-  for (int o = wave; o * 8 < HR; o += 4) {
+  for (int o = wave; seeds && o * 8 < HR; o += 4) {
     uint32_t packed = 0;
 #pragma unroll
     for (int k = 0; k < 8; ++k) {
@@ -922,12 +942,13 @@
   __syncthreads();
   uint32_t hw[5];
 #pragma unroll
-  for (int k = 0; k < 5; ++k) hw[k] = (wave + k) * 8 < (uint32_t)HR ? s_hd[wave + k][lane] : 0xFFFFFFFFu;
-  if (__ballot((hw[0] & hw[1] & hw[2] & hw[3] & hw[4]) != 0xFFFFFFFFu) == 0ull) return;
+  for (int k = 0; k < 5; ++k) hw[k] = (seeds && (wave + k) * 8 < (uint32_t)HR) ? s_hd[wave + k][lane] : 0xFFFFFFFFu;
+  const bool wave_cost = __ballot((hw[0] & hw[1] & hw[2] & hw[3] & hw[4]) != 0xFFFFFFFFu) != 0ull;
+  if (!wave_cost && !tile_in_box) return;
   const int gx = tx0 + (int)lane;
   const int R2 = R * R;
   uint32_t bestr[8] = {0xFFFFu, 0xFFFFu, 0xFFFFu, 0xFFFFu, 0xFFFFu, 0xFFFFu, 0xFFFFu, 0xFFFFu};
-  if (RT > 0) {
+  if (RT > 0 && wave_cost) {
     const unsigned long long rowany = (((unsigned long long)s_rowany[1] << 32) | s_rowany[0]) >> (8u * wave);
     const uint32_t ra_lo = __builtin_amdgcn_readfirstlane((uint32_t)rowany), ra_hi = __builtin_amdgcn_readfirstlane((uint32_t)(rowany >> 32));
 #pragma unroll
@@ -946,11 +967,17 @@
       }
     }
   }
+  uint8_t boxv[8];
+  if (BITS && tile_in_box) {
+#pragma unroll
+    for (int j = 0; j < 8; ++j) boxv[j] = master[min(ty0 + (int)wave * 8 + j, (int)cm.ny - 1) * cm.nx + min(gx, (int)cm.nx - 1)];
+  }
+  uint32_t my_touched = 0, my_free = 0;
 #pragma unroll
   for (int j = 0; j < 8; ++j) {
     const int gy = ty0 + (int)wave * 8 + j;
     uint32_t best = bestr[j];
-    if (RT == 0) {
+    if (RT == 0 && wave_cost) {
       for (int dy = -R; dy <= R; ++dy) {
         const int p = j + R + dy;
         const uint32_t wsel = p >> 3;
@@ -960,12 +987,46 @@
         best = d2 < best ? d2 : best;
       }
     }
-    if (best > (uint32_t)R2 || gx >= (int)cm.nx || gy >= (int)cm.ny) continue;
-    const uint8_t cost = s_lut2[best];
-    if (cost == 0) continue;
-    const uint8_t old = master[gy * cm.nx + gx];
-    const uint8_t nv = (old == kNoInfo && cost >= kInscribed) ? cost : (old > cost ? old : cost);
-    if (nv != old) master[gy * cm.nx + gx] = nv;
+    if (!BITS) {
+      if (best > (uint32_t)R2 || gx >= (int)cm.nx || gy >= (int)cm.ny) continue;
+      const uint8_t cost = s_lut2[best];
+      if (cost == 0) continue;
+      const uint8_t old = master[gy * cm.nx + gx];
+      const uint8_t nv = (old == kNoInfo && cost >= kInscribed) ? cost : (old > cost ? old : cost);
+      if (nv != old) master[gy * cm.nx + gx] = nv;
+    } else {
+      const bool on_map = gx < (int)cm.nx && gy < (int)cm.ny;
+      const uint8_t cost = best <= (uint32_t)R2 ? s_lut2[best] : (uint8_t)0;
+      const bool in_box = tile_in_box && on_map && gx >= bx0 && gx < bxn && gy >= by0 && gy < byn;
+      bool touched = in_box;
+      uint8_t nv = 0;
+      if (in_box || (on_map && cost != 0)) {
+        uint8_t old;
+        if (in_box)
+          old = boxv[j];
+        else
+          old = master[gy * cm.nx + gx];
+        nv = (old == kNoInfo && cost >= kInscribed) ? cost : (old > cost ? old : cost);
+        if (nv != old) {
+          master[gy * cm.nx + gx] = nv;
+          touched = true;
+        }
+      }
+      const unsigned long long tm = __ballot(touched);
+      if (tm != 0ull) {
+        const bool obstacle = nv == kLethal || nv == kInscribed || (nv == kNoInfo && cm.free_unknown_is_obstacle);
+        const unsigned long long fm = __ballot(touched && !obstacle);
+        if ((lane >> 1) == (uint32_t)j) {
+          my_touched = (lane & 1u) ? (uint32_t)(tm >> 32) : (uint32_t)tm;
+          my_free = (lane & 1u) ? (uint32_t)(fm >> 32) : (uint32_t)fm;
+        }
+      }
+    }
+  }
+  if (BITS && my_touched != 0u) {
+    const uint32_t W = (cm.nx + 31) >> 5;
+    uint32_t* p = cm.free_bits + (size_t)inst * cm.ny * W + (size_t)(ty0 + (int)wave * 8 + (int)(lane >> 1)) * W + 2u * tbx + (lane & 1u);
+    *p = (*p & ~my_touched) | (my_free & my_touched);
   }
 }
 
@@ -1152,10 +1213,17 @@
   }
   if (cm.lut2_ok && R >= 1 && R <= 14) {
     dim3 grid(8u * ((cm.nx + kBX - 1) / kBX), (cm.ny + kBY - 1) / kBY, (count + 7u) / 8u);
+    if (cm.free_bits && !boxes) {
+      if (R == 11)
+        hipLaunchKernelGGL((k_inflate_bits<11, true>), grid, dim3(256), 0, s, cm, first, count, boxes);
+      else
+        hipLaunchKernelGGL((k_inflate_bits<0, true>), grid, dim3(256), 0, s, cm, first, count, boxes);
+      return;
+    }
     if (R == 11)
-      hipLaunchKernelGGL(k_inflate_bits<11>, grid, dim3(256), 0, s, cm, first, count, boxes);
+      hipLaunchKernelGGL((k_inflate_bits<11, false>), grid, dim3(256), 0, s, cm, first, count, boxes);
     else
-      hipLaunchKernelGGL(k_inflate_bits<0>, grid, dim3(256), 0, s, cm, first, count, boxes);
+      hipLaunchKernelGGL((k_inflate_bits<0, false>), grid, dim3(256), 0, s, cm, first, count, boxes);
     return;
   }
   const int W = kTile + 2 * R, WS = (W + 3) & ~3;
@@ -1164,4 +1232,6 @@
   hipLaunchKernelGGL(k_inflate, grid, dim3(256), lds, s, cm, first, boxes);
 }
 
-}
+
+
+}
diff --git a/navigation_amd/csrc/navgpu_device.h b/navigation_amd/csrc/navgpu_device.h
--- a/navigation_amd/csrc/navgpu_device.h
+++ b/navigation_amd/csrc/navgpu_device.h
@@ -91,6 +91,8 @@
   uint8_t *master_alt, *obst_alt;
   uint32_t* voxel_alt;
   uint2* mark_seq;
+  uint32_t* free_bits;
+  uint32_t free_unknown_is_obstacle;
 };
 
 struct PlannerDev {
@@ -118,6 +120,7 @@
   uint32_t* bfs_care;
   uint32_t* bfs_reach;
   uint32_t bfs_bounded;
+  uint32_t bfs_free_current;
   unsigned long long* bfs_trace;
   uint32_t* bfs_next_item;
   uint32_t* bfs_free;
@@ -179,6 +182,9 @@
 void launch_reset_bounding_box(const CostmapDev& cm, uint32_t first, uint32_t count, const double* boxes_world, hipStream_t s);
 void launch_merge(const CostmapDev& cm, uint32_t first, uint32_t count, const int32_t* boxes, hipStream_t s, bool layer_only = false);
 void launch_inflate(const CostmapDev& cm, uint32_t first, uint32_t count, const int32_t* boxes, hipStream_t s);
+inline bool inflate_keeps_free_bits(const CostmapDev& cm) {
+  return (cm.layers & NAVGPU_LAYER_INFLATION) && cm.infl_enabled && !cm.infl_pq && cm.lut2_ok && cm.R >= 1 && cm.R <= 14;
+}
 void launch_static_interpret(uint8_t* dst, const int8_t* occ, uint32_t cells, uint32_t cells_padded, uint32_t count,
                              int track_unknown_space, int trinary, int lethal_threshold, int unknown_cost_value, hipStream_t s);
 void launch_export_window(const uint8_t* master, uint32_t nx, uint32_t x0, uint32_t y0, uint32_t w, uint32_t h, int8_t* out, hipStream_t s);
diff --git a/navigation_amd/csrc/navgpu_fleet.h b/navigation_amd/csrc/navgpu_fleet.h
--- a/navigation_amd/csrc/navgpu_fleet.h
+++ b/navigation_amd/csrc/navgpu_fleet.h
@@ -66,6 +66,10 @@
   std::vector<uint64_t> inputs_gen, cycle_gen;
   void touchInputs(uint32_t first, uint32_t count) {
     for (uint32_t i = first; i < first + count && i < inputs_gen.size(); ++i) ++inputs_gen[i];
+  }
+  std::vector<uint8_t> free_bits_valid;
+  void dropFreeBits(uint32_t first, uint32_t count) {
+    for (uint32_t i = first; i < first + count && i < free_bits_valid.size(); ++i) free_bits_valid[i] = 0;
   }
   navgpu_robot_state* hp_state = nullptr;
   navgpu_plan_result* hp_result = nullptr;
diff --git a/navigation_amd/csrc/navgpu_host.cpp b/navigation_amd/csrc/navgpu_host.cpp
--- a/navigation_amd/csrc/navgpu_host.cpp
+++ b/navigation_amd/csrc/navgpu_host.cpp
@@ -221,6 +221,7 @@
   f->bounded_grids = true;
   f->h_box.assign((size_t)n * 4, 0);
   f->inputs_gen.assign(n, 0);
+  f->free_bits_valid.assign(n, 0);
   f->cycle_gen.assign(n, 0);
   launch_fill_u8(cm.master, cm.master_default, (size_t)n * cm.cells_padded, f->stream);
   if (cm.obst) launch_fill_u8(cm.obst, cm.obstacle_default, (size_t)n * cm.cells_padded, f->stream);
@@ -317,6 +318,7 @@
   if (!f || !host || !f->rangeOk(first, count)) return NAVGPU_ERR_INVALID;
   FleetGuard guard_(f);
   f->touchInputs(first, count);
+  f->dropFreeBits(first, count);
   void* base;
   size_t elem, stride, used;
   int rc = gridInfo(f, grid, &base, &elem, &stride, &used);
@@ -349,6 +351,7 @@
   int rc = gridInfo(f, grid, &base, &elem, &stride, &used);
   if (rc) return rc;
   if (grid >= NAVGPU_GRID_PATH && (rc = ensureCompleteGrids(f, 0, f->desc.n_instances))) return rc;
+  if (grid == NAVGPU_GRID_MASTER) f->dropFreeBits(0, f->desc.n_instances);
   *ptr = base;
   if (stride_bytes) *stride_bytes = stride * elem;
   return NAVGPU_OK;
@@ -357,6 +360,7 @@
   if (!f || !f->rangeOk(first, count)) return NAVGPU_ERR_INVALID;
   FleetGuard guard_(f);
   f->touchInputs(first, count);
+  f->dropFreeBits(first, count);
   CostmapDev& cm = f->cm;
   switch (grid) {
     case NAVGPU_GRID_MASTER: launch_fill_u8(cm.master + (size_t)first * cm.cells_padded, cm.master_default, (size_t)count * cm.cells_padded, f->stream); break;
@@ -389,6 +393,7 @@
   }
   if (!base) return NAVGPU_ERR_STATE;
   f->touchInputs(first, count);
+  f->dropFreeBits(first, count);
   if (xn > x0 && yn > y0) launch_reset_window(base + (size_t)first * cm.cells_padded, cm.cells_padded, count, cm.nx, x0, y0, xn, yn, value, f->stream);
   return checkLaunch();
 }
@@ -404,6 +409,7 @@
     if (rc) return rc;
   }
   f->touchInputs(first, count);
+  f->dropFreeBits(first, count);
   HIP_TRY(hipMemcpyAsync(f->d_bounds_tmp, boxes, sizeof(double) * 4 * count, hipMemcpyHostToDevice, f->stream));
   launch_reset_bounding_box(cm, first, count, f->d_bounds_tmp, f->stream);
   HIP_TRY(waitStream(f->stream));
@@ -501,6 +507,7 @@
   FleetGuard guard_(f);
   CostmapDev& cm = f->cm;
   if (!cm.stat) return NAVGPU_ERR_STATE;
+  f->dropFreeBits(first, count);
   if (!f->d_occ) {
     int rc = f->alloc(&f->d_occ, cm.cells);
     if (rc) return rc;
@@ -563,6 +570,7 @@
   cm.static_use_maximum = use_maximum;
   cm.static_received = 1;
   f->touchInputs(0, f->desc.n_instances);
+  f->dropFreeBits(0, f->desc.n_instances);
   return checkLaunch();
 }
 
@@ -573,6 +581,7 @@
   HIP_TRY(hipMemcpyAsync(f->cm.stat_tf + (size_t)first * 12, m, sizeof(double) * 12 * count, hipMemcpyHostToDevice, f->stream));
   HIP_TRY(waitStream(f->stream));
   f->touchInputs(first, count);
+  f->dropFreeBits(first, count);
   return NAVGPU_OK;
 }
 
@@ -673,6 +682,7 @@
   HIP_TRY(waitStream(f->stream));
   cm.infl_pq = want_pq;
   cm.lut2_ok = lut2_ok ? 1 : 0;
+  f->dropFreeBits(0, f->desc.n_instances);
   const bool changed = !f->inflation_configured || f->infl.inflation_radius != p->inflation_radius ||
                        f->infl.cost_scaling_factor != p->cost_scaling_factor || f->infl.inscribed_radius != p->inscribed_radius ||
                        f->infl.enabled != p->enabled || f->infl.priority_queue_order != p->priority_queue_order;
@@ -786,6 +796,7 @@
   f->h_fp_n.swap(fp_n);
   f->h_fp_spec.swap(fp_spec);
   f->fp_radius = fp_radius;
+  f->dropFreeBits(first, count);
   if (f->planner_configured) {
     uint8_t* keep = fresh_prep ? fresh_prep : f->pl.prep;
     if (fresh_prep) f->release(f->pl.prep);
@@ -882,6 +893,7 @@
   launch_shift_u8(cm.master, cm.master_alt, cm, first, count, cm.master_default, f->stream);
   std::swap(cm.master, cm.master_alt);
   f->pl.master = cm.master;
+  f->dropFreeBits(first, count);
   if (cm.obst) {
     launch_shift_u8(cm.obst, cm.obst_alt, cm, first, count, cm.obstacle_default, f->stream);
     std::swap(cm.obst, cm.obst_alt);
@@ -906,6 +918,14 @@
   }
   PROFILED(f, NAVGPU_K_OBSTACLE, launch_obstacle(cm, first, count, nullptr, 0, f->stream));
   PROFILED(f, NAVGPU_K_MERGE, launch_merge(cm, first, count, nullptr, f->stream));
+  if (inflate_keeps_free_bits(cm)) {
+    CostmapDev keep = cm;
+    keep.free_bits = f->pl.bfs_free;
+    keep.free_unknown_is_obstacle = f->pl.cfg.allow_unknown != 0 ? 0u : 1u;
+    PROFILED(f, NAVGPU_K_INFLATE, launch_inflate(keep, first, count, nullptr, f->stream));
+    return checkLaunch();
+  }
+  f->dropFreeBits(first, count);
   if (cm.layers & NAVGPU_LAYER_INFLATION) PROFILED(f, NAVGPU_K_INFLATE, launch_inflate(cm, first, count, nullptr, f->stream));
   return checkLaunch();
 }
@@ -925,6 +945,7 @@
   if (!f || !f->rangeOk(first, count)) return NAVGPU_ERR_INVALID;
   FleetGuard guard_(f);
   f->touchInputs(first, count);
+  f->dropFreeBits(first, count);
   if (!f->inflation_configured) return NAVGPU_ERR_STATE;
   const int32_t* d_boxes = nullptr;
   if (boxes) {
@@ -955,6 +976,7 @@
   if (!f || !f->rangeOk(first, count)) return NAVGPU_ERR_INVALID;
   FleetGuard guard_(f);
   f->touchInputs(first, count);
+  f->dropFreeBits(first, count);
   const int32_t* d_boxes = nullptr;
   if (boxes) {
     HIP_TRY(hipMemcpyAsync(f->d_boxes_tmp, boxes, sizeof(int32_t) * 4 * count, hipMemcpyHostToDevice, f->stream));
@@ -1160,6 +1182,7 @@
   pl = np;
   f->planner_configured = true;
   f->touchInputs(0, nI);
+  f->dropFreeBits(0, nI);
   if ((rc = restageReach(f)) != NAVGPU_OK) return rc;
   HIP_TRY(waitStream(f->stream));
   return NAVGPU_OK;
@@ -1311,7 +1334,14 @@
     f->grid_partial[i] = robotBox(f, i, f->hp_state[i].pos, f->hp_reach[i], &f->h_box[(size_t)4 * i]) ? 1 : 0;
     f->cycle_gen[i] = f->inputs_gen[i];
   }
+  bool rebuild = NAVGPU_DEBUG_ENV("NAVGPU_DEBUG_REBUILD_FREE_BITS") != nullptr;
+  for (uint32_t i = first; i < first + count; ++i) {
+    if (!f->free_bits_valid[i]) rebuild = true;
+    f->free_bits_valid[i] = 1;
+  }
+  pl.bfs_free_current = rebuild ? 0u : 1u;
   launch_samples(pl, first, count, f->stream);
+  pl.bfs_free_current = 0;
 #ifdef NAVGPU_DEBUG_SWITCHES
   if (getenv("NAVGPU_DEBUG_BFS_TRACE") && !pl.bfs_trace) f->alloc(&pl.bfs_trace, (size_t)f->desc.n_instances * 3 * 8);
 #endif
diff --git a/navigation_amd/csrc/navgpu_tp.cpp b/navigation_amd/csrc/navgpu_tp.cpp
--- a/navigation_amd/csrc/navgpu_tp.cpp
+++ b/navigation_amd/csrc/navgpu_tp.cpp
@@ -181,6 +181,7 @@
   pl.cfg.allow_unknown = f->tp.cfg.allow_unknown;
   pl.bfs_bounded = 0;
   for (uint32_t i = first; i < first + count; ++i) f->grid_partial[i] = 0;
+  f->dropFreeBits(first, count);
   PROFILED(f, NAVGPU_K_BFS, launch_bfs(pl, first, count, f->stream));
   return NAVGPU_OK;
 }
diff --git a/navigation_amd/csrc/planner_samples.hip b/navigation_amd/csrc/planner_samples.hip
--- a/navigation_amd/csrc/planner_samples.hip
+++ b/navigation_amd/csrc/planner_samples.hip
@@ -252,7 +252,8 @@
 }
 void launch_samples(const PlannerDev& pl, uint32_t first, uint32_t count, hipStream_t s) {
   const uint32_t words = pl.ny * ((pl.nx + 31) / 32);
-  hipLaunchKernelGGL(k_samples, dim3(2 * count + count * ((words + kSamplesThreads - 1) / kSamplesThreads)), dim3(kSamplesThreads), 0, s, pl, first, count);
+  const uint32_t bitmap_blocks = pl.bfs_free_current ? 0u : count * ((words + kSamplesThreads - 1) / kSamplesThreads);
+  hipLaunchKernelGGL(k_samples, dim3(2 * count + bitmap_blocks), dim3(kSamplesThreads), 0, s, pl, first, count);
 }
 
 }
```

New measurement: 5.527 billion. 1.7% lower.
